# WU-CVGL/SIU3R

Measured on AMD Instinct MI355X. Metric: image-pairs/sec @2x512^2 (SIU3R network forward incl. panoptic post-process), higher is better.
Workload: dtype bf16x3 (fp32 activations, bf16 MFMA with hi/lo operand split; meets the 1e-3 parity bar)

## Files before the change

### include/siu3r_hip.h

```cpp
#ifndef SIU3R_HIP_H
#define SIU3R_HIP_H
#include <stdint.h>
#ifdef __cplusplus
extern "C" {
#endif

#define SIU3R_BF16 0
#define SIU3R_F32 1
#define SIU3R_F16 2
#define SIU3R_F64 3

const char* siu3r_last_error(void);
#define SIU3R_ABI_VERSION 12
int siu3r_abi_version(void);

int siu3r_rope2d(void* tokens, int dtype, int B, int N, int H, int D, int64_t stride_b,
                 int64_t stride_n, int64_t stride_h, const int64_t* positions, float base, float fwd,
                 void* stream);

typedef struct {
  const void* a;
  const void* w_hi;
  const void* w_lo;
  void* c;
  const float* bias;
  const void* residual;
  int32_t m, n, k, kpad;
  int64_t lda, ldc, ldr;
  int32_t a_dtype, c_dtype, r_dtype;
  int32_t act;
  int32_t relu_in;
  int32_t batch;
  int64_t sa, sw, sc, sr;
  int32_t a_mode;
  int32_t ih, iw, cin, kh, kw, stride, pad, oh, ow;
  int32_t out_mode, up, cout;
  const void* up_src;
  int32_t up_dtype;
  const float* rope_cos;
  const float* rope_sin;
  const int64_t* rope_pos;
  int32_t rope_ncols;
  int32_t map_gx, map_rm, map_rn;
  uint64_t* trace;
  const void* w_x3;
  int32_t bmod;
  int64_t sa_i, sc_i, sr_i, sbias;
  const float* ln_stats;
  const float* ln_c1;
  const float* ln_c2;
  int32_t ln_tiles;
  float ln_eps;
  int64_t ln_ldm, ln_sz, ln_sz_i;
  float* stats_out;
  int64_t st_ldm, st_sz, st_sz_i;
  void* c_aux;
  int32_t splitk;
  float* sk_ws;
  int32_t* sk_cnt;
  int64_t sk_ws_floats;
  int32_t sk_cnt_n;
  int32_t tile_cfg;
  int32_t m_main;
  int32_t sk_gx;
  void* c_x3;
  int32_t a_x3;
  int32_t c_x3_col0;
} siu3r_gemm_params;
#define SIU3R_TILE_AUTO 0
#define SIU3R_TILE_128x64 -1
#define SIU3R_TILE_PP_256x256 1
#define SIU3R_TILE_PP_256x128 2
#define SIU3R_TILE_PP_128x128 3
int siu3r_gemm(const siu3r_gemm_params* p, void* stream);
typedef struct {
  int32_t tile_cfg, bm, bn, splitk, skinny_rows, counters;
  int64_t ws_floats;
  char kernel[160];
  int32_t a_x3_ok, c_x3_ok;
  int32_t skinny_path;
} siu3r_gemm_plan_t;
int siu3r_gemm_plan(const siu3r_gemm_params* p, siu3r_gemm_plan_t* out);
int siu3r_gemm_tune(int key, int value);

int siu3r_layernorm(const float* x, void* y, int y_dtype, const float* gamma, const float* beta,
                    int64_t rows, int C, int64_t ldx, int64_t ldy, float eps, void* stream);
int siu3r_layernorm2(const float* x, void* y, int y_dtype, void* y2_bf16, const float* gamma, const float* beta, int64_t rows, int C,
                     int64_t ldx, int64_t ldy, int64_t ldy2, float eps, void* stream);

typedef struct {
  const void *q, *k, *v;
  void* out;
  int32_t dtype;
  int32_t B, H, Nq, Nk, D;
  int64_t q_sb, q_sn, q_sh, k_sb, k_sn, k_sh, v_sb, v_sn, v_sh;
  float scale;
  const float *rope_cos, *rope_sin;
  int32_t rope_max_pos;
  const int64_t *qpos, *kpos;
  const uint8_t* mask;
  int32_t split3;
  int64_t mask_ld;
  float* ws;
  int32_t splits;
  int32_t kv_bxor;
  int32_t kv_x3;
  int32_t out_x3;
} siu3r_attn_params;
int siu3r_attention(const siu3r_attn_params* p, void* stream);
int siu3r_attention_out_x3_ok(const siu3r_attn_params* p);
int siu3r_attention_kv_x3_ok(const siu3r_attn_params* p);
typedef struct {
  char kernel[160];
  int32_t queries_per_wg, key_ranges, combine, key_halves, side_path;
} siu3r_attn_plan_t;
int siu3r_attention_plan(const siu3r_attn_params* p, siu3r_attn_plan_t* out);

int siu3r_add(const float* a, const float* b, float* y, int64_t rows, int64_t b_rows, int C, void* stream);
int siu3r_pack_image_nhwc(const float* img, void* out, int out_dtype, int N, int H, int W, int cpad, void* stream);
int siu3r_resize_bilinear(const void* x, int x_dtype, void* y, int y_dtype, const void* addend, int add_dtype,
                          const float* ch_scale, const float* ch_shift, int N, int IH, int IW, int OH, int OW,
                          int C, int align_corners, void* stream);
int siu3r_resize_bilinear_strided(const void* x, int x_dtype, void* y, int y_dtype, const void* addend, int add_dtype,
                                  const float* ch_scale, const float* ch_shift, int N, int IH, int IW, int OH, int OW,
                                  int C, int align_corners, int64_t x_batch_stride, int64_t addend_batch_stride, void* stream);
int siu3r_resize_bilinear_planes(const void* x, int x_dtype, void* y_planes, int N, int IH, int IW, int OH, int OW, int C, int align_corners,
                                 int64_t x_batch_stride, void* stream);
int siu3r_affine_add(const void* x, int x_dtype, const void* addend, int add_dtype, void* y, int y_dtype,
                     const float* ch_scale, const float* ch_shift, int64_t rows, int C, void* stream);
int siu3r_affine_add_strided(const void* x, int x_dtype, const void* addend, int add_dtype, void* y, int y_dtype,
                             const float* ch_scale, const float* ch_shift, int64_t rows, int C, int64_t rows_per_batch,
                             int64_t x_batch_stride, int64_t addend_batch_stride, void* stream);
int siu3r_maxpool3x3s2(const void* x, void* y, int dtype, int N, int IH, int IW, int C, void* stream);
int siu3r_maxpool2x2s2(const void* x, void* y, int dtype, int N, int IH, int IW, int C, void* stream);
int siu3r_lpips_layer(const float* f0, const float* f1, const float* w, float* dist, int64_t npix, int C, float eps, void* stream);
int siu3r_stem7x7_x3(const float* img, const void* wfrag, const float* bias, const float* up_src, float* out, int B, int G, int H, int W,
                     int planes_out, void* stream);
int siu3r_proj_rows_x3(const float* x, const void* wfrag, const float* bias, float* out, int Z, int G, int64_t M, int K, int N, int ldc,
                       int64_t out_z_stride, void* stream);
int siu3r_rowchain_x3(const float* x, const float* res, const void* pack, float* out, int64_t M, int H, float eps1, float eps2, void* stream);
int siu3r_dwconv3x3_gelu(const void* x, void* y, int dtype, const float* w9c, const float* bias, int B, int H,
                         int W, int C, void* stream);
int siu3r_dwconv3x3_gelu_planes(const float* x, void* y_planes, const float* w9c, const float* bias, int B, int H, int W, int C, void* stream);
int siu3r_msdeform_sample(const void* value, int v_dtype, const float* offs_aw, const float* ref,
                          const int32_t* shapes_host, void* out, int out_dtype, int B, int S, int Q, int heads,
                          int d, int L, int P, void* stream);
int siu3r_msdeform_sample_planes(const void* value, int v_dtype, const float* offs_aw, const float* ref, const int32_t* shapes_host,
                                 void* out_planes, int B, int S, int Q, int heads, int d, int L, int P, void* stream);
int siu3r_groupnorm(const void* x, int x_dtype, void* y, int y_dtype, const float* gamma, const float* beta,
                    float* stats_ws, const void* addend, int add_dtype, int relu, int N, int HW, int C,
                    int groups, float eps, void* stream);
int siu3r_pts3d_exp(float* xyz, int64_t n, void* stream);
int siu3r_gaussian_adapter(const void* raw, int raw_dtype, float* opacities, float* scales, float* rotations,
                           float* harmonics, float* covariances, int64_t n, void* stream);
int siu3r_m2f_attn_mask(const float* mask_logits, uint8_t* out, int32_t* row_counts_ws, int B, int T, int IH,
                        int IW, int OH, int OW, int Q, int64_t out_ld, void* stream);

typedef struct {
  int32_t mode;
  int32_t width, height;
  float w2c[16];
  float proj[16];
  float tanfovx, tanfovy;
  float campos[3];
  float bg[3];
  int32_t sh_degree;
  int32_t sh_band4;
  float k2_znear_cull;
  float fx, fy, cx, cy;
  float near_plane, far_plane;
  float eps2d;
  float radius_clip;
  float extent_sigma;
  int32_t opacity_aware_extent;
  float alpha_min;
  float alpha_max;
  float t_min;
  float dilation;
  int32_t nt_post_blend;
  float k2_near, k2_far;
} siu3r_raster_cam;
int siu3r_raster_geometry(int width, int height, int64_t G, int32_t* out8);
int siu3r_raster_project(const siu3r_raster_cam* cams_host, int V, void* cams_dev, int64_t G, const float* means, const float* cov,
                         int cov_stride, const float* opacities, const float* colors, int channels, int sh_planar, float* rec,
                         int32_t* radii, int32_t* rect, int32_t* tiles_touched, uint32_t* keys, uint64_t* stats, void* stream);
int siu3r_raster_project_dp(const siu3r_raster_cam* cams_host, int V, void* cams_dev, const float* viewmats_dev, const float* Ks_dev, int64_t G,
                            const float* means, const float* cov, int cov_stride, const float* opacities, const float* colors, int channels,
                            int sh_planar, float* rec, int32_t* radii, int32_t* rect, int32_t* tiles_touched, uint32_t* keys, uint64_t* stats,
                            void* stream);
int siu3r_raster_project_c2w(const siu3r_raster_cam* cams_host, int V, void* cams_dev, const float* c2w_dev, const float* Kn_dev, float t_scale,
                             int64_t G, const float* means, const float* cov, int cov_stride, const float* opacities, const float* colors,
                             int channels, int sh_planar, float* rec, int32_t* radii, int32_t* rect, int32_t* tiles_touched, uint32_t* keys,
                             uint64_t* stats, void* stream);
int siu3r_raster_project_aa(const siu3r_raster_cam* cams_host, int V, void* cams_dev, int64_t G, const float* means, const float* cov,
                            int cov_stride, const float* opacities, const float* colors, int channels, int sh_planar, float* rec,
                            int32_t* radii, int32_t* rect, int32_t* tiles_touched, uint32_t* keys, uint64_t* stats, float* comp, void* stream);
int siu3r_raster_project_c2w_aa(const siu3r_raster_cam* cams_host, int V, void* cams_dev, const float* c2w_dev, const float* Kn_dev, float t_scale,
                                int64_t G, const float* means, const float* cov, int cov_stride, const float* opacities, const float* colors,
                                int channels, int sh_planar, float* rec, int32_t* radii, int32_t* rect, int32_t* tiles_touched, uint32_t* keys,
                                uint64_t* stats, float* comp, void* stream);
int siu3r_raster_sort(int V, int64_t G, uint32_t* keys_a, uint32_t* keys_b, int32_t* ids_a, int32_t* ids_b, int32_t* rs_hist,
                      int32_t* rs_tot, const uint64_t* stats, void* stream);
int siu3r_raster_bin(const siu3r_raster_cam* cams_host, int V, int64_t G, const uint32_t* keys, const int32_t* ids, const int32_t* rect,
                     int32_t* bin_hist, int32_t* bin_tot, int32_t* bin_start, void* entries, int64_t cap_e, uint64_t* stats, void* stream);
int siu3r_raster_composite_rgb(const siu3r_raster_cam* cams_host, int V, const void* cams_dev, int64_t G, const int32_t* bin_start,
                               const void* entries, int64_t cap_e, const float* rec, float* image, float* out_depth, float* out_alpha,
                               int32_t* n_touched, void* stream);
int siu3r_raster_tile_lists(const siu3r_raster_cam* cams_host, int V, const int32_t* bin_start, const void* entries, int64_t cap_e,
                            int32_t* tile_count, int32_t* tile_start, int32_t* ids, int64_t cap_d, uint64_t* stats, void* stream);
int siu3r_raster_composite_feat(const siu3r_raster_cam* cams_host, int V, const void* cams_dev, int64_t G, const int32_t* tile_start,
                                const int32_t* ids, int64_t cap_d, const float* rec, const float* feats, int channels, float* out,
                                float* out_alpha, void* stream);
int64_t siu3r_raster_composite_feat_ws_bytes(int width, int height, int V, int64_t cap_d);
int siu3r_raster_composite_feat_ws_lists(int width, int height, int V, int64_t G, const float* feats, int channels, const void* ws, int64_t ws_bytes,
                                         int64_t cap_d);
int siu3r_raster_composite_feat_ws(const siu3r_raster_cam* cams_host, int V, const void* cams_dev, int64_t G, const int32_t* tile_start,
                                   const int32_t* ids, int64_t cap_d, const float* rec, const float* feats, int channels, float* out,
                                   float* out_alpha, void* ws, int64_t ws_bytes, void* stream);
int siu3r_raster_tune(int key, int value);
int siu3r_raster_contrib(const siu3r_raster_cam* cams_host, int V, const void* cams_dev, int64_t G, const int32_t* bin_start, const void* entries,
                         int64_t cap_e, const float* rec, float* wmax, int32_t* count, uint64_t* wsum, void* stream);
int siu3r_raster_composite_rgb_bwd(const siu3r_raster_cam* cams_host, int V, const void* cams_dev, int64_t G, const int32_t* bin_start,
                                   const void* entries, int64_t cap_e, const float* rec, const float* image, const float* depth, const float* alpha,
                                   const float* g_image, const float* g_depth, const float* g_alpha, float* grad, void* stream);
int siu3r_raster_composite_rgb_bwd_abs(const siu3r_raster_cam* cams_host, int V, const void* cams_dev, int64_t G, const int32_t* bin_start,
                                       const void* entries, int64_t cap_e, const float* rec, const float* image, const float* depth,
                                       const float* alpha, const float* g_image, const float* g_depth, const float* g_alpha, float* grad,
                                       float* abs_mean2d, void* stream);
int siu3r_raster_project_bwd(const siu3r_raster_cam* cams_host, int V, const void* cams_dev, int64_t G, const float* means, const float* cov,
                             int cov_stride, const float* opacities, const float* colors, int channels, int sh_planar, const int32_t* rect,
                             const float* grad, float* g_means, float* g_cov, float* g_opacities, float* g_colors, float* g_mean2d,
                             float* pose_part, void* stream);
int siu3r_raster_project_bwd_aa(const siu3r_raster_cam* cams_host, int V, const void* cams_dev, int64_t G, const float* means, const float* cov,
                                int cov_stride, const float* opacities, const float* colors, int channels, int sh_planar, const int32_t* rect,
                                const float* grad, float* g_means, float* g_cov, float* g_opacities, float* g_colors, float* g_mean2d,
                                float* pose_part, void* stream);
int64_t siu3r_raster_pose_partial_rows(int64_t G);
int siu3r_raster_pose_reduce(int V, int64_t nrows, const float* pose_part, float* g_pose, void* stream);
int siu3r_raster_composite_rgb_bwd_k3(const siu3r_raster_cam* cams_host, int V, const void* cams_dev, int64_t G, const int32_t* bin_start,
                                      const void* entries, int64_t cap_e, const float* rec, const float* colors, const float* alphas,
                                      const float* g_colors, const float* g_alphas, float* grad, void* stream);
int siu3r_raster_quad_lists(const siu3r_raster_cam* cams_host, int V, const void* cams_dev, int64_t G, const int32_t* tile_start, const int32_t* ids,
                            int64_t cap_d, const float* rec, void* ws, int64_t ws_bytes, void* stream);
int siu3r_raster_composite_feat_bwd(const siu3r_raster_cam* cams_host, int V, const void* cams_dev, int64_t G, const int32_t* tile_start,
                                    const void* ws, int64_t cap_d, const float* rec, const float* feats, int channels, const float* out,
                                    const float* out_alpha, const float* g_out, const float* g_alpha, float* grad, float* g_feats, void* stream);
int siu3r_raster_project_bwd_k3(const siu3r_raster_cam* cams_host, int V, const void* cams_dev, int64_t G, const float* means, const float* cov,
                                int cov_stride, const int32_t* rect, const float* grad, float* g_means, float* g_cov, float* g_opacities,
                                float* g_colors, float* pose_part, void* stream);
int siu3r_raster_viewmat_reduce(int V, int64_t nrows, const float* pose_part, float* g_viewmats, void* stream);
int siu3r_scale_inplace(float* x, int64_t n, float s, void* stream);
int siu3r_lift_ids(const float* qc, int V, int H, int W, int q, int C, float sem_threshold, int num_queries,
                   uint32_t stuff_mask, int64_t* sem_id, int64_t* ins_id, int32_t* first_pix, int32_t* q_label,
                   void* stream);

int siu3r_split_bf16(const float* x, void* hi, void* lo, void* x3, int64_t rows, int k, int kpad, int64_t ldx, void* stream);

int siu3r_panoptic_stage1(const float* class_logits, const float* mask_logits_cl, float* probs, float* scores,
                          int32_t* labels, int32_t* kept_idx, int32_t* n_keep, float* p256, int32_t* lab_map,
                          int32_t* area, int32_t* orig, int32_t* seg_id, int32_t* seg_label, int32_t* seg_fused,
                          float* seg_score, int32_t* acc_list, int32_t* n_acc, int32_t* seg, int32_t* sem, int32_t* ins,
                          int B, int T, int Q, int C, int IH, int IW, int H, int W, int mask_size, float threshold,
                          float mask_threshold, float overlap, uint32_t fuse_mask, void* stream);
int siu3r_panoptic_qcl(const float* p256, const float* probs, const int32_t* kept_idx, const int32_t* acc_list, int nq,
                       float* out, int b, int T, int H, int W, int mask_size, int Q, int C, void* stream);

int siu3r_quat_scale_to_cov6(const float* quats_wxyz, const float* scales, float* cov6, int64_t G, void* stream);
int siu3r_sh_eval(const float* means, const float* campos3_host, const float* sh, int ncoef, int degree, float* rgb, int64_t G, void* stream);
int siu3r_blend_background(float* colors, const float* alpha, const float* bg_host, int channels, int64_t pixels, void* stream);
int siu3r_sh_eval_dp(const float* means, const float* campos3_dev, const float* sh, int ncoef, int degree, float* rgb, int64_t G, void* stream);
int siu3r_blend_background_dp(float* colors, const float* alpha, const float* bg_dev, int channels, int64_t pixels, void* stream);
int siu3r_quat_scale_to_cov6_bwd(const float* quats_wxyz, const float* scales, const float* g_cov6, float* g_quats, float* g_scales, int64_t G, void* stream);
int siu3r_sh_eval_bwd(const float* means, const float* campos3_dev, const float* sh, int ncoef, int degree, const float* g_rgb, float* g_sh, float* g_means,
                      float* g_campos3, int64_t G, void* stream);

int64_t siu3r_photo_loss_partials(int V, int C, int H, int W);
int siu3r_photo_loss(const float* pred, const float* target, int V, int C, int H, int W, const int64_t* pred_strides,
                     const int64_t* target_strides, float lambda, float data_range, float* grad_pred, float* partials, float* out,
                     void* stream);

int64_t siu3r_depth_loss_ws(int V, int H, int W);
int siu3r_depth_loss(const float* depth, const float* opacity, const float* target, const float* weight, int V, int H, int W, int mode, int space,
                     float min_opacity, float* g_depth, float* g_opacity, void* ws, float* out, float* per_view, int32_t* valid, void* stream);

int64_t siu3r_depth_smooth_ws(int V, int H, int W);
int siu3r_depth_smooth(const float* depth, const float* opacity, const int32_t* segments, int V, int H, int W, int order, int space,
                       float min_opacity, float* g_depth, float* g_opacity, void* ws, float* out, float* per_view, int32_t* active, void* stream);

int siu3r_density_accumulate(const float* g_mean2d, const int32_t* radii, int V, int64_t G, float sx, float sy, float* grad_accum,
                             int32_t* seen, int32_t* max_radius, void* stream);
int64_t siu3r_density_plan_ws(int64_t G);
int siu3r_density_plan(const float* grad_accum, const int32_t* seen, const int32_t* max_radius, const float* log_scales,
// ... 59 lines not shown
```

### siu3r_amd/_lib.py

```python
from __future__ import annotations

import ctypes as C
import os

_HERE = os.path.dirname(os.path.abspath(__file__))
LIB_PATH = os.environ.get("SIU3R_LIB_OVERRIDE") or os.path.join(_HERE, "libsiu3r_hip.so")

BF16, F32 = 0, 1


class GemmParams(C.Structure):
    _fields_ = [
        ("a", C.c_void_p), ("w_hi", C.c_void_p), ("w_lo", C.c_void_p), ("c", C.c_void_p),
        ("bias", C.c_void_p), ("residual", C.c_void_p),
        ("m", C.c_int32), ("n", C.c_int32), ("k", C.c_int32), ("kpad", C.c_int32),
        ("lda", C.c_int64), ("ldc", C.c_int64), ("ldr", C.c_int64),
        ("a_dtype", C.c_int32), ("c_dtype", C.c_int32), ("r_dtype", C.c_int32),
        ("act", C.c_int32), ("relu_in", C.c_int32),
        ("batch", C.c_int32),
        ("sa", C.c_int64), ("sw", C.c_int64), ("sc", C.c_int64), ("sr", C.c_int64),
        ("a_mode", C.c_int32),
        ("ih", C.c_int32), ("iw", C.c_int32), ("cin", C.c_int32), ("kh", C.c_int32), ("kw", C.c_int32),
        ("stride", C.c_int32), ("pad", C.c_int32), ("oh", C.c_int32), ("ow", C.c_int32),
        ("out_mode", C.c_int32), ("up", C.c_int32), ("cout", C.c_int32),
        ("up_src", C.c_void_p), ("up_dtype", C.c_int32),
        ("rope_cos", C.c_void_p), ("rope_sin", C.c_void_p), ("rope_pos", C.c_void_p), ("rope_ncols", C.c_int32),
        ("map_gx", C.c_int32), ("map_rm", C.c_int32), ("map_rn", C.c_int32),
        ("trace", C.c_void_p), ("w_x3", C.c_void_p),
        ("bmod", C.c_int32), ("sa_i", C.c_int64), ("sc_i", C.c_int64), ("sr_i", C.c_int64), ("sbias", C.c_int64),
        ("ln_stats", C.c_void_p), ("ln_c1", C.c_void_p), ("ln_c2", C.c_void_p), ("ln_tiles", C.c_int32), ("ln_eps", C.c_float),
        ("ln_ldm", C.c_int64), ("ln_sz", C.c_int64), ("ln_sz_i", C.c_int64),
        ("stats_out", C.c_void_p), ("st_ldm", C.c_int64), ("st_sz", C.c_int64), ("st_sz_i", C.c_int64),
        ("c_aux", C.c_void_p),
        ("splitk", C.c_int32), ("sk_ws", C.c_void_p), ("sk_cnt", C.c_void_p),
        ("sk_ws_floats", C.c_int64), ("sk_cnt_n", C.c_int32), ("tile_cfg", C.c_int32), ("m_main", C.c_int32), ("sk_gx", C.c_int32),
        ("c_x3", C.c_void_p), ("a_x3", C.c_int32), ("c_x3_col0", C.c_int32),
    ]


class GemmPlan(C.Structure):
    _fields_ = [
        ("tile_cfg", C.c_int32), ("bm", C.c_int32), ("bn", C.c_int32), ("splitk", C.c_int32), ("skinny_rows", C.c_int32),
        ("counters", C.c_int32), ("ws_floats", C.c_int64), ("kernel", C.c_char * 160), ("a_x3_ok", C.c_int32), ("c_x3_ok", C.c_int32), ("skinny_path", C.c_int32),
    ]


class AttnParams(C.Structure):
    _fields_ = [
        ("q", C.c_void_p), ("k", C.c_void_p), ("v", C.c_void_p), ("out", C.c_void_p),
        ("dtype", C.c_int32),
        ("B", C.c_int32), ("H", C.c_int32), ("Nq", C.c_int32), ("Nk", C.c_int32), ("D", C.c_int32),
        ("q_sb", C.c_int64), ("q_sn", C.c_int64), ("q_sh", C.c_int64),
        ("k_sb", C.c_int64), ("k_sn", C.c_int64), ("k_sh", C.c_int64),
        ("v_sb", C.c_int64), ("v_sn", C.c_int64), ("v_sh", C.c_int64),
        ("scale", C.c_float),
        ("rope_cos", C.c_void_p), ("rope_sin", C.c_void_p), ("rope_max_pos", C.c_int32),
        ("qpos", C.c_void_p), ("kpos", C.c_void_p), ("mask", C.c_void_p),
        ("split3", C.c_int32), ("mask_ld", C.c_int64),
        ("ws", C.c_void_p), ("splits", C.c_int32), ("kv_bxor", C.c_int32), ("kv_x3", C.c_int32), ("out_x3", C.c_int32),
    ]


class AttnPlan(C.Structure):
    _fields_ = [
        ("kernel", C.c_char * 160), ("queries_per_wg", C.c_int32), ("key_ranges", C.c_int32), ("combine", C.c_int32),
        ("key_halves", C.c_int32), ("side_path", C.c_int32),
    ]


class RasterCam(C.Structure):
    _fields_ = [
        ("mode", C.c_int32), ("width", C.c_int32), ("height", C.c_int32),
        ("w2c", C.c_float * 16), ("proj", C.c_float * 16),
        ("tanfovx", C.c_float), ("tanfovy", C.c_float), ("campos", C.c_float * 3), ("bg", C.c_float * 3),
        ("sh_degree", C.c_int32), ("sh_band4", C.c_int32), ("k2_znear_cull", C.c_float),
        ("fx", C.c_float), ("fy", C.c_float), ("cx", C.c_float), ("cy", C.c_float),
        ("near_plane", C.c_float), ("far_plane", C.c_float), ("eps2d", C.c_float), ("radius_clip", C.c_float),
        ("extent_sigma", C.c_float), ("opacity_aware_extent", C.c_int32),
        ("alpha_min", C.c_float), ("alpha_max", C.c_float), ("t_min", C.c_float), ("dilation", C.c_float),
        ("nt_post_blend", C.c_int32), ("k2_near", C.c_float), ("k2_far", C.c_float),
    ]


class AdamField(C.Structure):
    _fields_ = [
        ("param", C.c_void_p), ("grad", C.c_void_p), ("exp_avg", C.c_void_p), ("exp_avg_sq", C.c_void_p),
        ("width", C.c_int32), ("head_period", C.c_int32), ("lr", C.c_float), ("lr_tail", C.c_float),
    ]


_P, _I, _L, _F = C.c_void_p, C.c_int, C.c_int64, C.c_float
ABI_VERSION = 12

SIGNATURES = {
    "siu3r_last_error": [],
    "siu3r_abi_version": [],
    "siu3r_rope2d": [_P, _I, _I, _I, _I, _I, _L, _L, _L, _P, _F, _F, _P],
    "siu3r_gemm": [C.POINTER(GemmParams), _P],
    "siu3r_gemm_plan": [C.POINTER(GemmParams), C.POINTER(GemmPlan)],
    "siu3r_gemm_tune": [_I, _I],
    "siu3r_layernorm": [_P, _P, _I, _P, _P, _L, _I, _L, _L, _F, _P],
    "siu3r_layernorm2": [_P, _P, _I, _P, _P, _P, _L, _I, _L, _L, _L, _F, _P],
    "siu3r_attention": [C.POINTER(AttnParams), _P],
    "siu3r_attention_kv_x3_ok": [C.POINTER(AttnParams)],
    "siu3r_attention_out_x3_ok": [C.POINTER(AttnParams)],
    "siu3r_attention_plan": [C.POINTER(AttnParams), C.POINTER(AttnPlan)],
    "siu3r_add": [_P, _P, _P, _L, _L, _I, _P],
    "siu3r_pack_image_nhwc": [_P, _P, _I, _I, _I, _I, _I, _P],
    "siu3r_resize_bilinear": [_P, _I, _P, _I, _P, _I, _P, _P, _I, _I, _I, _I, _I, _I, _I, _P],
    "siu3r_affine_add": [_P, _I, _P, _I, _P, _I, _P, _P, _L, _I, _P],
    "siu3r_resize_bilinear_strided": [_P, _I, _P, _I, _P, _I, _P, _P, _I, _I, _I, _I, _I, _I, _I, _L, _L, _P],
    "siu3r_resize_bilinear_planes": [_P, _I, _P, _I, _I, _I, _I, _I, _I, _I, _L, _P],
    "siu3r_affine_add_strided": [_P, _I, _P, _I, _P, _I, _P, _P, _L, _I, _L, _L, _L, _P],
    "siu3r_maxpool3x3s2": [_P, _P, _I, _I, _I, _I, _I, _P],
    "siu3r_maxpool2x2s2": [_P, _P, _I, _I, _I, _I, _I, _P],
    "siu3r_lpips_layer": [_P, _P, _P, _P, _L, _I, _F, _P],
    "siu3r_stem7x7_x3": [_P, _P, _P, _P, _P, _I, _I, _I, _I, _I, _P],
    "siu3r_proj_rows_x3": [_P, _P, _P, _P, _I, _I, _L, _I, _I, _I, _L, _P],
    "siu3r_rowchain_x3": [_P, _P, _P, _P, _L, _I, _F, _F, _P],
    "siu3r_dwconv3x3_gelu": [_P, _P, _I, _P, _P, _I, _I, _I, _I, _P],
    "siu3r_dwconv3x3_gelu_planes": [_P, _P, _P, _P, _I, _I, _I, _I, _P],
    "siu3r_msdeform_sample_planes": [_P, _I, _P, _P, C.POINTER(C.c_int32), _P, _I, _I, _I, _I, _I, _I, _I, _P],
    "siu3r_msdeform_sample": [_P, _I, _P, _P, C.POINTER(C.c_int32), _P, _I, _I, _I, _I, _I, _I, _I, _I, _P],
    "siu3r_groupnorm": [_P, _I, _P, _I, _P, _P, _P, _P, _I, _I, _I, _I, _I, _I, _F, _P],
    "siu3r_pts3d_exp": [_P, _L, _P],
    "siu3r_gaussian_adapter": [_P, _I, _P, _P, _P, _P, _P, _L, _P],
    "siu3r_m2f_attn_mask": [_P, _P, _P, _I, _I, _I, _I, _I, _I, _I, _L, _P],
    "siu3r_split_bf16": [_P, _P, _P, _P, _L, _I, _I, _L, _P],
    "siu3r_raster_geometry": [_I, _I, _L, C.POINTER(C.c_int32)],
    "siu3r_raster_project": [C.POINTER(RasterCam), _I, _P, _L, _P, _P, _I, _P, _P, _I, _I, _P, _P, _P, _P, _P, _P, _P],
    "siu3r_raster_sort": [_I, _L, _P, _P, _P, _P, _P, _P, _P, _P],
    "siu3r_raster_bin": [C.POINTER(RasterCam), _I, _L, _P, _P, _P, _P, _P, _P, _P, _L, _P, _P],
    "siu3r_raster_composite_rgb": [C.POINTER(RasterCam), _I, _P, _L, _P, _P, _L, _P, _P, _P, _P, _P, _P],
    "siu3r_raster_tile_lists": [C.POINTER(RasterCam), _I, _P, _P, _L, _P, _P, _P, _L, _P, _P],
    "siu3r_raster_composite_feat": [C.POINTER(RasterCam), _I, _P, _L, _P, _P, _L, _P, _P, _I, _P, _P, _P],
    "siu3r_raster_composite_feat_ws_bytes": [_I, _I, _I, _L],
    "siu3r_raster_tune": [_I, _I],
    "siu3r_raster_composite_feat_ws": [C.POINTER(RasterCam), _I, _P, _L, _P, _P, _L, _P, _P, _I, _P, _P, _P, _L, _P],
    "siu3r_scale_inplace": [_P, _L, _F, _P],
    "siu3r_quat_scale_to_cov6": [_P, _P, _P, _L, _P],
    "siu3r_sh_eval": [_P, _P, _P, _I, _I, _P, _L, _P],
    "siu3r_blend_background": [_P, _P, _P, _I, _L, _P],
    "siu3r_sh_eval_dp": [_P, _P, _P, _I, _I, _P, _L, _P],
    "siu3r_blend_background_dp": [_P, _P, _P, _I, _L, _P],
    "siu3r_raster_project_dp": [C.POINTER(RasterCam), _I, _P, _P, _P, _L, _P, _P, _I, _P, _P, _I, _I, _P, _P, _P, _P, _P, _P, _P],
    "siu3r_raster_project_c2w": [C.POINTER(RasterCam), _I, _P, _P, _P, _F, _L, _P, _P, _I, _P, _P, _I, _I, _P, _P, _P, _P, _P, _P, _P],
    "siu3r_raster_project_aa": [C.POINTER(RasterCam), _I, _P, _L, _P, _P, _I, _P, _P, _I, _I, _P, _P, _P, _P, _P, _P, _P, _P],
    "siu3r_raster_project_c2w_aa": [C.POINTER(RasterCam), _I, _P, _P, _P, _F, _L, _P, _P, _I, _P, _P, _I, _I, _P, _P, _P, _P, _P, _P, _P, _P],
    "siu3r_raster_project_bwd_aa": [C.POINTER(RasterCam), _I, _P, _L, _P, _P, _I, _P, _P, _I, _I, _P, _P, _P, _P, _P, _P, _P, _P, _P],
    "siu3r_mip_filter3d_ws": [_I],
    "siu3r_mip_filter3d": [_P, _P, _I, _I, _I, _P, _L, _F, _F, _F, _P, _P, _P],
    "siu3r_mip_apply": [_P, _P, _P, _L, _P, _P, _P],
    "siu3r_mip_apply_bwd": [_P, _P, _P, _P, _P, _L, _P, _P, _P],
    "siu3r_raster_composite_rgb_bwd": [C.POINTER(RasterCam), _I, _P, _L, _P, _P, _L, _P, _P, _P, _P, _P, _P, _P, _P, _P],
    "siu3r_raster_composite_rgb_bwd_abs": [C.POINTER(RasterCam), _I, _P, _L, _P, _P, _L, _P, _P, _P, _P, _P, _P, _P, _P, _P, _P],
    "siu3r_raster_contrib": [C.POINTER(RasterCam), _I, _P, _L, _P, _P, _L, _P, _P, _P, _P, _P],
    "siu3r_raster_project_bwd": [C.POINTER(RasterCam), _I, _P, _L, _P, _P, _I, _P, _P, _I, _I, _P, _P, _P, _P, _P, _P, _P, _P, _P],
    "siu3r_raster_pose_partial_rows": [_L],
    "siu3r_raster_pose_reduce": [_I, _L, _P, _P, _P],
    "siu3r_raster_composite_rgb_bwd_k3": [C.POINTER(RasterCam), _I, _P, _L, _P, _P, _L, _P, _P, _P, _P, _P, _P, _P],
    "siu3r_raster_composite_feat_ws_lists": [_I, _I, _I, _L, _P, _I, _P, _L, _L],
    "siu3r_raster_quad_lists": [C.POINTER(RasterCam), _I, _P, _L, _P, _P, _L, _P, _P, _L, _P],
    "siu3r_raster_composite_feat_bwd": [C.POINTER(RasterCam), _I, _P, _L, _P, _P, _L, _P, _P, _I, _P, _P, _P, _P, _P, _P, _P],
    "siu3r_raster_project_bwd_k3": [C.POINTER(RasterCam), _I, _P, _L, _P, _P, _I, _P, _P, _P, _P, _P, _P, _P, _P],
    "siu3r_raster_viewmat_reduce": [_I, _L, _P, _P, _P],
    "siu3r_quat_scale_to_cov6_bwd": [_P, _P, _P, _P, _P, _L, _P],
    "siu3r_sh_eval_bwd": [_P, _P, _P, _I, _I, _P, _P, _P, _P, _L, _P],
    "siu3r_photo_loss_partials": [_I, _I, _I, _I],
    "siu3r_photo_loss": [_P, _P, _I, _I, _I, _I, C.POINTER(C.c_int64), C.POINTER(C.c_int64), _F, _F, _P, _P, _P, _P],
    "siu3r_depth_loss_ws": [_I, _I, _I],
    "siu3r_depth_loss": [_P, _P, _P, _P, _I, _I, _I, _I, _I, _F, _P, _P, _P, _P, _P, _P, _P],
    "siu3r_depth_smooth_ws": [_I, _I, _I],
    "siu3r_depth_smooth": [_P, _P, _P, _I, _I, _I, _I, _I, _F, _P, _P, _P, _P, _P, _P, _P],
    "siu3r_gaussian_adam_ws": [_L],
    "siu3r_gaussian_adam": [C.POINTER(AdamField), _I, _L, C.c_double, C.c_double, _F, _F, _F, _P, _I, _I, _P, _P, _P],
    "siu3r_density_accumulate": [_P, _P, _I, _L, _F, _F, _P, _P, _P, _P],
    "siu3r_density_plan_ws": [_L],
    "siu3r_density_plan": [_P, _P, _P, _P, _P, _L, _F, _F, _F, _I, _F, _I, _P, _P, _P, _P, _P],
    "siu3r_density_apply": [_I, _P, _P, _P, _I, _L, _P, _P, _P, _P, _P, _P, _P, _P, _P],
    "siu3r_mcmc_ws": [_L],
    "siu3r_mcmc_weights": [_P, _L, _F, _I, _P, _P, _P],
    "siu3r_mcmc_scan": [_P, _P, _L, _P, _P, _P, _P, _P],
    "siu3r_mcmc_sample": [_P, _L, _P, _L, _P, _P, _P],
    "siu3r_mcmc_relocate": [_P, _P, _P, _L, C.c_double, _P],
    "siu3r_mcmc_copy_rows": [_P, _P, _P, _I, _L, _P, _P, _L, _L, _P],
    "siu3r_mcmc_noise": [_P, _P, _P, _P, _P, _L, _F, _F, _P],
    "siu3r_mcmc_regularize": [_P, _P, _L, _F, _F, _P, _P, _P, _P, _P],
    "siu3r_exposure_ws": [_I, _I, _I],
    "siu3r_exposure_apply": [_P, C.POINTER(C.c_int64), _P, _I, _I, _I, _P, _P],
    "siu3r_exposure_apply_bwd": [_P, C.POINTER(C.c_int64), _P, _P, _I, _I, _I, _P, _P, _P, _P],
    "siu3r_camera_step": [_P, _P, _P, _P, _P, _P, _P, _I, _L] + [C.c_double] * 6 + [_P],
    "siu3r_bilagrid_apply": [_P, C.POINTER(C.c_int64), _P, _I, _I, _I, _I, _I, _I, _P, _P],
    "siu3r_bilagrid_apply_bwd": [_P, C.POINTER(C.c_int64), _P, _P, _I, _I, _I, _I, _I, _I, _P, _P, _P],
    "siu3r_bilagrid_tv_ws": [_I, _I, _I, _I],
    "siu3r_bilagrid_tv": [_P, _I, _I, _I, _I, _F, _P, _P, _P, _P],
    "siu3r_lift_ids":[_P, _I, _I, _I, _I, _I, _F, _I, C.c_uint32, _P, _P, _P, _P, _P],
    "siu3r_panoptic_stage1": [_P] * 20 + [_I] * 9 + [_F, _F, _F, C.c_uint32, _P],
    "siu3r_panoptic_qcl": [_P, _P, _P, _P, _I, _P, _I, _I, _I, _I, _I, _I, _I, _P],
}
_RESTYPES = {"siu3r_last_error": C.c_char_p, "siu3r_raster_composite_feat_ws_bytes": C.c_int64, "siu3r_raster_pose_partial_rows": C.c_int64}
_RESTYPES["siu3r_photo_loss_partials"] = C.c_int64
_RESTYPES["siu3r_density_plan_ws"] = C.c_int64
_RESTYPES["siu3r_depth_loss_ws"] = C.c_int64
_RESTYPES["siu3r_depth_smooth_ws"] = C.c_int64
_RESTYPES["siu3r_gaussian_adam_ws"] = C.c_int64
_RESTYPES["siu3r_mcmc_ws"] = C.c_int64
_RESTYPES["siu3r_exposure_ws"] = C.c_int64
_RESTYPES["siu3r_bilagrid_tv_ws"] = C.c_int64
_RESTYPES["siu3r_mip_filter3d_ws"] = C.c_int64

_lib = None


def lib():
    global _lib
    if _lib is not None:
        return _lib
    import torch
    if not os.path.exists(LIB_PATH):
        raise RuntimeError(
            f"{LIB_PATH} is missing: build it with `python -m siu3r_amd.build` "
            "(hipcc --offload-arch=gfx950).  There is no CPU fallback for the SIU3R hot path."
        )
    l = C.CDLL(LIB_PATH)
    for name, argtypes in SIGNATURES.items():
        fn = getattr(l, name)
        fn.argtypes = argtypes
        fn.restype = _RESTYPES.get(name, C.c_int)
    if l.siu3r_abi_version() != ABI_VERSION:
        raise RuntimeError(f"{LIB_PATH} has ABI version {l.siu3r_abi_version()}, these bindings expect {ABI_VERSION}: rebuild it "
                           f"(python -m siu3r_amd.build)")
    _lib = l
    return l


def check(rc: int, what: str = ""):
    if rc != 0:
        msg = lib().siu3r_last_error()
        raise RuntimeError((msg.decode() if msg else f"{what} failed") + f" [rc={rc}]")
```

### siu3r_amd/csrc/elementwise.hip

```cpp
#include "common.h"

namespace {

struct f32x4v {
  float v[4];
};
__device__ __forceinline__ f32x4v load4(const void* p, int dtype, int64_t i) {
  f32x4v r;
  if (dtype == SIU3R_F32) {
    float4 a = *(const float4*)((const float*)p + i);
    r.v[0] = a.x; r.v[1] = a.y; r.v[2] = a.z; r.v[3] = a.w;
  } else {
    uint2 a = *(const uint2*)((const u16*)p + i);
    r.v[0] = bf16_bits_to_f32((u16)(a.x & 0xffff));
    r.v[1] = bf16_bits_to_f32((u16)(a.x >> 16));
    r.v[2] = bf16_bits_to_f32((u16)(a.y & 0xffff));
    r.v[3] = bf16_bits_to_f32((u16)(a.y >> 16));
  }
  return r;
}
__device__ __forceinline__ void store4(void* p, int dtype, int64_t i, const f32x4v& r) {
  if (dtype == SIU3R_F32) {
    *(float4*)((float*)p + i) = make_float4(r.v[0], r.v[1], r.v[2], r.v[3]);
  } else {
    uint2 w;
    w.x = (uint32_t)f32_to_bf16_bits(r.v[0]) | ((uint32_t)f32_to_bf16_bits(r.v[1]) << 16);
    w.y = (uint32_t)f32_to_bf16_bits(r.v[2]) | ((uint32_t)f32_to_bf16_bits(r.v[3]) << 16);
    *(uint2*)((u16*)p + i) = w;
  }
}

__device__ __forceinline__ float wave_sum(float v) {
#pragma unroll
  for (int o = 32; o > 0; o >>= 1) v += __shfl_xor(v, o);
  return v;
}

template <int DT>
__global__ void rope2d_kernel(void* tokens, const int64_t* pos, int B, int N, int H, int D, int64_t sb, int64_t sn,
                              int64_t sh, float base, float fwd) {
  const int Q = D / 4, half = D / 2;
  const int64_t idx = (int64_t)blockIdx.x * blockDim.x + threadIdx.x;
  const int64_t total = (int64_t)B * N * half;
  if (idx >= total) return;
  const int pr = (int)(idx % half);
  const int64_t tok = idx / half;
  const int n = (int)(tok % N), b = (int)(tok / N);
  const int axis = pr / Q, q = pr - axis * Q;
  const float inv_freq = fwd / powf(base, q / float(Q));
  const float freq = pos[tok * 2 + axis] * inv_freq;
  const float c = cosf(freq), s = sinf(freq);
  const int64_t e0 = b * sb + n * sn + axis * 2 * Q + q;
  for (int h = 0; h < H; ++h) {
    const int64_t e = e0 + h * sh;
    if (DT == SIU3R_F32) {
      float* p = (float*)tokens + e;
      const float u = p[0], v = p[Q];
      p[0] = u * c - v * s;
      p[Q] = v * c + u * s;
    } else if (DT == SIU3R_F64) {
      double* p = (double*)tokens + e;
      const double u = p[0], v = p[Q];
      p[0] = u * (double)c - v * (double)s;
      p[Q] = v * (double)c + u * (double)s;
    } else if (DT == SIU3R_F16) {
      _Float16* p = (_Float16*)tokens + e;
      const float u = (float)p[0], v = (float)p[Q];
      p[0] = (_Float16)(u * c - v * s);
      p[Q] = (_Float16)(v * c + u * s);
    } else {
      u16* p = (u16*)tokens + e;
      const float u = bf16_bits_to_f32(p[0]), v = bf16_bits_to_f32(p[Q]);
      p[0] = f32_to_bf16_bits(u * c - v * s);
      p[Q] = f32_to_bf16_bits(v * c + u * s);
    }
  }
}

__global__ __launch_bounds__(256) void layernorm_kernel(const float* x, void* y, int y_dtype, void* y2, const float* gamma,
                                                        const float* beta, int64_t rows, int C, int64_t ldx,
                                                        int64_t ldy, int64_t ldy2, float eps) {
  const int lane = threadIdx.x & 63;
  const int64_t row = (int64_t)blockIdx.x * 4 + (threadIdx.x >> 6);
  if (row >= rows) return;
  const float* xr = x + row * ldx;
  float4 v[8];
  float sum = 0.f;
#pragma unroll
  for (int i = 0; i < 8; ++i) {
    const int c = lane * 4 + i * 256;
    if (c < C) {
      v[i] = *(const float4*)(xr + c);
      sum += v[i].x + v[i].y + v[i].z + v[i].w;
    }
  }
  const float mean = wave_sum(sum) / (float)C;
  float sq = 0.f;
#pragma unroll
  for (int i = 0; i < 8; ++i) {
    const int c = lane * 4 + i * 256;
    if (c < C) {
      const float a = v[i].x - mean, b = v[i].y - mean, cc = v[i].z - mean, d = v[i].w - mean;
      sq += a * a + b * b + cc * cc + d * d;
    }
  }
  const float rstd = rsqrtf(wave_sum(sq) / (float)C + eps);
#pragma unroll
  for (int i = 0; i < 8; ++i) {
    const int c = lane * 4 + i * 256;
    if (c < C) {
      const float4 g = *(const float4*)(gamma + c), bb = *(const float4*)(beta + c);
      f32x4v o;
      o.v[0] = (v[i].x - mean) * rstd * g.x + bb.x;
      o.v[1] = (v[i].y - mean) * rstd * g.y + bb.y;
      o.v[2] = (v[i].z - mean) * rstd * g.z + bb.z;
      o.v[3] = (v[i].w - mean) * rstd * g.w + bb.w;
      store4(y, y_dtype, row * ldy + c, o);
      if (y2) store4(y2, SIU3R_BF16, row * ldy2 + c, o);
    }
  }
}

__global__ void add_kernel(const float* a, const float* b, float* y, int64_t rows, int64_t b_rows, int C4) {
  const int64_t idx = (int64_t)blockIdx.x * blockDim.x + threadIdx.x;
  if (idx >= rows * C4) return;
  const int64_t r = idx / C4;
  const int c = (int)(idx - r * C4);
  const float4 x = ((const float4*)a)[idx];
  const float4 z = ((const float4*)b)[(r % b_rows) * C4 + c];
  ((float4*)y)[idx] = make_float4(x.x + z.x, x.y + z.y, x.z + z.z, x.w + z.w);
}

__global__ void pack_image_kernel(const float* img, void* out, int out_dtype, int N, int H, int W, int cpad) {
  const int64_t idx = (int64_t)blockIdx.x * blockDim.x + threadIdx.x;
  const int64_t hw = (int64_t)H * W;
  if (idx >= (int64_t)N * hw) return;
  const int64_t n = idx / hw, r = idx - n * hw;
  if (cpad == 4) {
    float4 o = {img[(n * 3 + 0) * hw + r], img[(n * 3 + 1) * hw + r], img[(n * 3 + 2) * hw + r], 0.f};
    ((float4*)out)[idx] = o;
    return;
  }
  f32x8 v;
#pragma unroll
  for (int j = 0; j < 8; ++j) v.v[j] = 0.f;
  for (int c = 0; c < 3; ++c) v.v[c] = img[(n * 3 + c) * hw + r];
  store8_from_f32(out, out_dtype, idx * 8, v);
}

__device__ __forceinline__ void src_index(int o, int in, int out, int align, int& i0, int& i1, float& l1) {
  float src;
  if (align) {
    const float scale = out > 1 ? (float)(in - 1) / (float)(out - 1) : 0.f;
// ... 263 lines not shown
        const float aw = expf(e4[pt] - mx) / den;
        const float locx = rx + o8[pt * 2 + 0] / (float)ww;
        const float locy = ry + o8[pt * 2 + 1] / (float)hh;
        const float gx = 2.f * locx - 1.f, gy = 2.f * locy - 1.f;
        const float fx = ((gx + 1.f) * ww - 1.f) * 0.5f, fy = ((gy + 1.f) * hh - 1.f) * 0.5f;
        const float x0f = floorf(fx), y0f = floorf(fy);
        const int x0 = (int)x0f, y0 = (int)y0f;
        const float lx = fx - x0f, ly = fy - y0f;
        const float wgt[4] = {(1.f - lx) * (1.f - ly), lx * (1.f - ly), (1.f - lx) * ly, lx * ly};
#pragma unroll
        for (int k = 0; k < 4; ++k) {
          const int xx = x0 + (k & 1), yy = y0 + (k >> 1);
          const bool ok = xx >= 0 && xx < ww && yy >= 0 && yy < hh;
          const int xc = min(max(xx, 0), ww - 1), yc = min(max(yy, 0), hh - 1);
          const int s_ = st0 + yc * ww + xc;
          v[pt][k] = load4(value, v_dtype, ((vb + s_) * heads + hd) * d + dc);
#pragma unroll
          for (int j = 0; j < 4; ++j) v[pt][k].v[j] = ok ? v[pt][k].v[j] : 0.f;
          wk[pt][k] = wgt[k] * aw;
        }
      }
#pragma unroll
      for (int pt = 0; pt < 4; ++pt)
#pragma unroll
        for (int k = 0; k < 4; ++k)
#pragma unroll
          for (int j = 0; j < 4; ++j) acc.v[j] += v[pt][k].v[j] * wk[pt][k];
    }
    if (out_x3) {
      store_planes4_pair((unsigned char*)out + ((int64_t)b * Q + q) * heads * d * 4, hd * d + dc, acc.v);
      return;
    }
    store4(out, out_dtype, (((int64_t)b * Q + q) * heads + hd) * d + dc, acc);
  } else {
    const int LP = L * P;
    const float* row = offs_aw + ((int64_t)b * Q + q) * (heads * LP * 3);
    const float* offs = row + hd * LP * 2;
    const float* logit = row + heads * LP * 2 + hd * LP;
    float mx = -INFINITY;
    for (int i = 0; i < LP; ++i) mx = fmaxf(mx, logit[i]);
    float den = 0.f;
    for (int i = 0; i < LP; ++i) den += expf(logit[i] - mx);
    f32x4v acc;
#pragma unroll
    for (int j = 0; j < 4; ++j) acc.v[j] = 0.f;
    for (int l = 0; l < L; ++l) {
      const int hh = sh.h[l], ww = sh.w[l];
      const float rx = ref[((int64_t)q * L + l) * 2 + 0], ry = ref[((int64_t)q * L + l) * 2 + 1];
      for (int pt = 0; pt < P; ++pt) {
        const int i = l * P + pt;
        const float aw = expf(logit[i] - mx) / den;
        const float locx = rx + offs[i * 2 + 0] / (float)ww;
        const float locy = ry + offs[i * 2 + 1] / (float)hh;
        const float gx = 2.f * locx - 1.f, gy = 2.f * locy - 1.f;
        const float fx = ((gx + 1.f) * ww - 1.f) * 0.5f, fy = ((gy + 1.f) * hh - 1.f) * 0.5f;
        const float x0f = floorf(fx), y0f = floorf(fy);
        const int x0 = (int)x0f, y0 = (int)y0f;
        const float lx = fx - x0f, ly = fy - y0f;
        const float wgt[4] = {(1.f - lx) * (1.f - ly), lx * (1.f - ly), (1.f - lx) * ly, lx * ly};
#pragma unroll
        for (int k = 0; k < 4; ++k) {
          const int xx = x0 + (k & 1), yy = y0 + (k >> 1);
          if (xx < 0 || xx >= ww || yy < 0 || yy >= hh) continue;
          const int64_t s = sh.start[l] + (int64_t)yy * ww + xx;
          const f32x4v v = load4(value, v_dtype, (((int64_t)b * S + s) * heads + hd) * d + dc);
          const float wk = wgt[k] * aw;
#pragma unroll
          for (int j = 0; j < 4; ++j) acc.v[j] += v.v[j] * wk;
        }
      }
    }
    store4(out, out_dtype, (((int64_t)b * Q + q) * heads + hd) * d + dc, acc);
  }
}

constexpr int GN_T = 1024;
__global__ __launch_bounds__(GN_T) void gn_stats_kernel(const void* x, int x_dtype, float* stats, int HW, int C,
                                                        int groups, float eps) {
  const int n = blockIdx.y, bx = blockIdx.x;
  const int g = groups % 8 == 0 ? (bx % 8) * (groups / 8) + bx / 8 : bx;
  const int cg = C / groups, cg4 = cg >> 2;
  const int64_t total = (int64_t)HW * cg4;
  double s = 0.0, ss = 0.0;
  auto acc = [&](const f32x4v& v) {
#pragma unroll
    for (int j = 0; j < 4; ++j) {
      s += v.v[j];
      ss += (double)v.v[j] * v.v[j];
    }
  };
  int64_t i = threadIdx.x;
  if (GN_T % cg4 == 0) {
    const int64_t step = (int64_t)(GN_T / cg4) * C;
    int64_t off = (int64_t)n * HW * C + g * cg + (int)(threadIdx.x % cg4) * 4 + (int64_t)(threadIdx.x / cg4) * C;
    for (; i + GN_T < total; i += 2 * GN_T, off += 2 * step) {
      const f32x4v v = load4(x, x_dtype, off), w = load4(x, x_dtype, off + step);
      acc(v);
      acc(w);
    }
    for (; i < total; i += GN_T, off += step) acc(load4(x, x_dtype, off));
  }
  for (; i < total; i += GN_T) {
    const int64_t px = i / cg4;
    acc(load4(x, x_dtype, ((int64_t)n * HW + px) * C + g * cg + (int)(i - px * cg4) * 4));
  }
  __shared__ double sh_s[GN_T], sh_ss[GN_T];
  sh_s[threadIdx.x] = s;
  sh_ss[threadIdx.x] = ss;
  __syncthreads();
  for (int o = GN_T / 2; o > 0; o >>= 1) {
    if (threadIdx.x < o) {
      sh_s[threadIdx.x] += sh_s[threadIdx.x + o];
      sh_ss[threadIdx.x] += sh_ss[threadIdx.x + o];
    }
    __syncthreads();
  }
  if (threadIdx.x == 0) {
    const double cnt = (double)HW * cg;
    const double mean = sh_s[0] / cnt;
    double var = sh_ss[0] / cnt - mean * mean;
    if (var < 0) var = 0;
    stats[((int64_t)n * groups + g) * 2 + 0] = (float)mean;
    stats[((int64_t)n * groups + g) * 2 + 1] = (float)(1.0 / sqrt(var + (double)eps));
  }
}
__global__ void gn_apply_kernel(const void* x, int x_dtype, void* y, int y_dtype, const float* gamma,
                                const float* beta, const float* stats, const void* addend, int add_dtype, int relu,
                                int N, int HW, int C, int groups) {
  const int C4 = C >> 2;
  const int64_t idx = (int64_t)blockIdx.x * blockDim.x + threadIdx.x;
  if (idx >= (int64_t)N * HW * C4) return;
  const int c = (int)(idx % C4) * 4;
  const int n = (int)(idx / ((int64_t)HW * C4));
  const int g = c / (C / groups);
  const float mean = stats[((int64_t)n * groups + g) * 2], rstd = stats[((int64_t)n * groups + g) * 2 + 1];
  f32x4v v = load4(x, x_dtype, idx * 4);
#pragma unroll
  for (int j = 0; j < 4; ++j) {
    float o = (v.v[j] - mean) * rstd * gamma[c + j] + beta[c + j];
    if (relu) o = fmaxf(o, 0.f);
    v.v[j] = o;
  }
  if (addend) {
    const f32x4v a = load4(addend, add_dtype, idx * 4);
#pragma unroll
    for (int j = 0; j < 4; ++j) v.v[j] += a.v[j];
  }
  store4(y, y_dtype, idx * 4, v);
}

__global__ void pts3d_kernel(float* xyz, int64_t n) {
  const int64_t i = (int64_t)blockIdx.x * blockDim.x + threadIdx.x;
  if (i >= n) return;
  const float x = xyz[i * 3], y = xyz[i * 3 + 1], z = xyz[i * 3 + 2];
  const float d = sqrtf(x * x + y * y + z * z);
  const float dc = fmaxf(d, 1e-8f);
  const float e = expm1f(d);
  xyz[i * 3] = x / dc * e;
  xyz[i * 3 + 1] = y / dc * e;
  xyz[i * 3 + 2] = z / dc * e;
}

constexpr int GA_ROWS = 128, GA_D = 83, GA_SH = 75;
__constant__ float c_sh_mask[25];
__global__ __launch_bounds__(256) void gaussian_adapter_kernel(const void* raw, int raw_dtype, float* opac,
                                                               float* scales, float* rots, float* sh, float* cov,
                                                               int64_t n) {
  __shared__ float s[GA_ROWS * GA_D];
  __shared__ float so[GA_ROWS * 17];
  const int64_t g0 = (int64_t)blockIdx.x * GA_ROWS;
  const int rows = (int)((n - g0) < GA_ROWS ? (n - g0) : GA_ROWS);
  const int nt = blockDim.x;
  if (raw_dtype == SIU3R_F32 && rows == GA_ROWS && ((uintptr_t)raw & 15) == 0) {
    const float4* src = (const float4*)((const float*)raw + g0 * GA_D);
    for (int i = threadIdx.x; i < GA_ROWS * GA_D / 4; i += nt) ((float4*)s)[i] = src[i];
  } else {
    for (int i = threadIdx.x; i < rows * GA_D; i += nt) s[i] = load_as_f32(raw, raw_dtype, g0 * GA_D + i);
  }
  __syncthreads();
  const int t = threadIdx.x;
  if (t < rows) {
    const float* r = s + t * GA_D;
    opac[g0 + t] = 1.f / (1.f + expf(-r[0]));
    float sc[3];
#pragma unroll
    for (int j = 0; j < 3; ++j) {
      const float x = r[1 + j];
      const float sp = x > 20.f ? x : log1pf(expf(x));
      sc[j] = fminf(0.001f * sp, 0.3f);
      so[t * 17 + j] = sc[j];
    }
    const float qi = r[4], qj = r[5], qk = r[6], qr = r[7];
    so[t * 17 + 3] = qi; so[t * 17 + 4] = qj; so[t * 17 + 5] = qk; so[t * 17 + 6] = qr;
    const float nrm = sqrtf(qi * qi + qj * qj + qk * qk + qr * qr) + 1e-8f;
    const float i_ = qi / nrm, j_ = qj / nrm, k_ = qk / nrm, r_ = qr / nrm;
    const float two_s = 2.f / ((i_ * i_ + j_ * j_ + k_ * k_ + r_ * r_) + 1e-8f);
    float R[9];
    R[0] = 1.f - two_s * (j_ * j_ + k_ * k_);
    R[1] = two_s * (i_ * j_ - k_ * r_);
    R[2] = two_s * (i_ * k_ + j_ * r_);
    R[3] = two_s * (i_ * j_ + k_ * r_);
    R[4] = 1.f - two_s * (i_ * i_ + k_ * k_);
    R[5] = two_s * (j_ * k_ - i_ * r_);
    R[6] = two_s * (i_ * k_ - j_ * r_);
    R[7] = two_s * (j_ * k_ + i_ * r_);
    R[8] = 1.f - two_s * (i_ * i_ + j_ * j_);
    float M[9];
#pragma unroll
    for (int a = 0; a < 3; ++a)
#pragma unroll
      for (int b = 0; b < 3; ++b) M[a * 3 + b] = R[a * 3 + b] * sc[b];
#pragma unroll
    for (int a = 0; a < 3; ++a)
#pragma unroll
      for (int b = 0; b < 3; ++b) {
        float v = 0.f;
#pragma unroll
        for (int k2 = 0; k2 < 3; ++k2) v += (M[a * 3 + k2] * sc[k2]) * R[b * 3 + k2];
        so[t * 17 + 7 + a * 3 + b] = v;
      }
  }
  __syncthreads();
  for (int i = threadIdx.x; i < rows * 3; i += nt) scales[g0 * 3 + i] = so[(i / 3) * 17 + i % 3];
  for (int i = threadIdx.x; i < rows * 4; i += nt) rots[g0 * 4 + i] = so[(i >> 2) * 17 + 3 + (i & 3)];
  for (int i = threadIdx.x; i < rows * 9; i += nt) cov[g0 * 9 + i] = so[(i / 9) * 17 + 7 + i % 9];
  if (rows == GA_ROWS && ((uintptr_t)sh & 15) == 0) {
    for (int i4 = threadIdx.x; i4 < GA_ROWS * GA_SH / 4; i4 += nt) {
      float v[4];
#pragma unroll
      for (int u = 0; u < 4; ++u) {
        const int i = i4 * 4 + u, rr = i / GA_SH, e = i - rr * GA_SH;
        v[u] = s[rr * GA_D + 8 + e] * c_sh_mask[e % 25];
      }
      ((float4*)(sh + g0 * GA_SH))[i4] = make_float4(v[0], v[1], v[2], v[3]);
    }
  } else {
    for (int i = threadIdx.x; i < rows * GA_SH; i += nt) {
      const int rr = i / GA_SH, e = i - rr * GA_SH;
      sh[g0 * GA_SH + i] = s[rr * GA_D + 8 + e] * c_sh_mask[e % 25];
    }
  }
}

__global__ void m2f_mask_kernel(const float* ml, uint8_t* out, int32_t* row_counts, int B, int T, int IH, int IW,
                                int OH, int OW, int Q, int64_t ld) {
  const int64_t idx = (int64_t)blockIdx.x * blockDim.x + threadIdx.x;
  const int64_t total = (int64_t)B * T * OH * OW * Q;
  if (idx >= total) return;
  const int q = (int)(idx % Q);
  int64_t r = idx / Q;
  const int ox = (int)(r % OW);
  r /= OW;
  const int oy = (int)(r % OH);
  r /= OH;
  const int t = (int)(r % T);
  const int b = (int)(r / T);
  int y0, y1, x0, x1;
  float ly, lx;
  src_index(oy, IH, OH, 0, y0, y1, ly);
  src_index(ox, IW, OW, 0, x0, x1, lx);
  const int64_t base = ((int64_t)b * T + t) * IH * IW;
  const float v00 = ml[(base + (int64_t)y0 * IW + x0) * Q + q], v01 = ml[(base + (int64_t)y0 * IW + x1) * Q + q];
  const float v10 = ml[(base + (int64_t)y1 * IW + x0) * Q + q], v11 = ml[(base + (int64_t)y1 * IW + x1) * Q + q];
  const float v = (1.f - ly) * ((1.f - lx) * v00 + lx * v01) + ly * ((1.f - lx) * v10 + lx * v11);
  const float sg = 1.f / (1.f + expf(-v));
  const uint8_t blocked = sg < 0.5f ? 1 : 0;
  const int64_t nk = (int64_t)T * OH * OW;
  out[((int64_t)b * Q + q) * ld + ((int64_t)t * OH + oy) * OW + ox] = blocked;
  if (!blocked) row_counts[b * Q + q] = 1;
}
__global__ void zero_i32_kernel(int32_t* p, int64_t n) {
  const int64_t idx = (int64_t)blockIdx.x * blockDim.x + threadIdx.x;
  if (idx < n) p[idx] = 0;
}
__global__ void m2f_mask_fix_kernel(uint8_t* out, const int32_t* row_counts, int64_t rows, int64_t nk, int64_t ld) {
  const int64_t idx = (int64_t)blockIdx.x * blockDim.x + threadIdx.x;
  if (idx >= rows * nk) return;
  const int64_t r = idx / nk;
  if (row_counts[r] == 0) out[r * ld + (idx - r * nk)] = 0;
}

__global__ void split_bf16_kernel(const float* x, u16* hi, u16* lo, u16* x3, int64_t rows, int k, int kpad, int64_t ldx) {
  const int64_t idx = (int64_t)blockIdx.x * blockDim.x + threadIdx.x;
  if (idx >= rows * kpad) return;
  const int64_t r = idx / kpad;
  const int c = (int)(idx - r * kpad);
  const float v = c < k ? x[r * ldx + c] : 0.f;
  const u16 h = f32_to_bf16_bits(v);
  const u16 l = f32_to_bf16_bits(v - bf16_bits_to_f32(h));
  if (hi) hi[idx] = h;
  if (lo) lo[idx] = l;
  if (x3) {
    const int64_t o = r * 2 * kpad + (c >> 5) * 64 + (c & 31);
    x3[o] = h;
    x3[o + 32] = l;
  }
}

inline dim3 grid1d(int64_t total, int block = 256) { return dim3((unsigned)cdiv64(total, block)); }

inline bool al4(const void* p, int dtype) { return ((uintptr_t)p & (dtype == SIU3R_F32 ? 15 : 7)) == 0; }
inline bool al16(const void* p) { return ((uintptr_t)p & 15) == 0; }

}

extern "C" int siu3r_rope2d(void* tokens, int dtype, int B, int N, int H, int D, int64_t sb, int64_t sn, int64_t sh,
                            const int64_t* positions, float base, float fwd, void* stream) {
  SIU3R_CHECK(D % 4 == 0, "token dim must be multiple of 4");
  SIU3R_CHECK(dtype == SIU3R_F32 || dtype == SIU3R_BF16 || dtype == SIU3R_F16 || dtype == SIU3R_F64, "rope_2d: unsupported dtype %d", dtype);
  SIU3R_CHECK(B >= 0 && N >= 0 && H >= 0, "rope_2d: negative size");
  const int64_t total = (int64_t)B * N * (D / 2);
  if (total == 0 || H == 0) return 0;
  SIU3R_CHECK(tokens && positions, "rope_2d: null pointer");
  hipStream_t s = (hipStream_t)stream;
  if (dtype == SIU3R_F32)
    hipLaunchKernelGGL(rope2d_kernel<SIU3R_F32>, grid1d(total), dim3(256), 0, s, tokens, positions, B, N, H, D, sb, sn, sh, base, fwd);
  else if (dtype == SIU3R_F64)
    hipLaunchKernelGGL(rope2d_kernel<SIU3R_F64>, grid1d(total), dim3(256), 0, s, tokens, positions, B, N, H, D, sb, sn, sh, base, fwd);
  else if (dtype == SIU3R_F16)
    hipLaunchKernelGGL(rope2d_kernel<SIU3R_F16>, grid1d(total), dim3(256), 0, s, tokens, positions, B, N, H, D, sb, sn, sh, base, fwd);
  else
    hipLaunchKernelGGL(rope2d_kernel<SIU3R_BF16>, grid1d(total), dim3(256), 0, s, tokens, positions, B, N, H, D, sb, sn, sh, base, fwd);
  SIU3R_LAUNCH_CHECK("siu3r_rope2d");
  return 0;
}

extern "C" int siu3r_layernorm(const float* x, void* y, int y_dtype, const float* gamma, const float* beta,
                               int64_t rows, int C, int64_t ldx, int64_t ldy, float eps, void* stream) {
  SIU3R_CHECK(C % 4 == 0 && C <= 2048 && ldx % 4 == 0 && ldy % 4 == 0, "layernorm: C=%d must be a multiple of 4 and <= 2048", C);
  if (rows == 0) return 0;
  SIU3R_CHECK(x && y && gamma && beta, "layernorm: null pointer");
  SIU3R_CHECK(al16(x) && al4(y, y_dtype) && al16(gamma) && al16(beta), "layernorm: x, gamma, beta must be 16-byte aligned, y 16 (fp32) / 8 (bf16)");
  hipLaunchKernelGGL(layernorm_kernel, dim3((unsigned)cdiv64(rows, 4)), dim3(256), 0, (hipStream_t)stream, x, y, y_dtype, (void*)nullptr, gamma, beta, rows, C, ldx, ldy, (int64_t)0, eps);
  SIU3R_LAUNCH_CHECK("siu3r_layernorm");
  return 0;
}

extern "C" int siu3r_layernorm2(const float* x, void* y, int y_dtype, void* y2_bf16, const float* gamma, const float* beta, int64_t rows,
                                int C, int64_t ldx, int64_t ldy, int64_t ldy2, float eps, void* stream) {
  SIU3R_CHECK(C % 4 == 0 && C <= 2048 && ldx % 4 == 0 && ldy % 4 == 0 && ldy2 % 4 == 0, "layernorm2: C=%d must be a multiple of 4 and <= 2048", C);
  if (rows == 0) return 0;
  SIU3R_CHECK(x && y && y2_bf16 && gamma && beta, "layernorm2: null pointer");
  SIU3R_CHECK(al16(x) && al4(y, y_dtype) && al4(y2_bf16, SIU3R_BF16) && al16(gamma) && al16(beta),
              "layernorm2: x, gamma, beta must be 16-byte aligned, y 16 (fp32) / 8 (bf16), y2 8");
  hipLaunchKernelGGL(layernorm_kernel, dim3((unsigned)cdiv64(rows, 4)), dim3(256), 0, (hipStream_t)stream, x, y, y_dtype, y2_bf16, gamma, beta, rows, C, ldx, ldy, ldy2, eps);
  SIU3R_LAUNCH_CHECK("siu3r_layernorm2");
  return 0;
}

extern "C" int siu3r_add(const float* a, const float* b, float* y, int64_t rows, int64_t b_rows, int C, void* stream) {
  SIU3R_CHECK(C % 4 == 0 && b_rows > 0, "add: bad arguments");
  if (rows == 0 || C == 0) return 0;
  SIU3R_CHECK(a && b && y, "add: null pointer");
  SIU3R_CHECK(al16(a) && al16(b) && al16(y), "add: a, b, y must be 16-byte aligned");
  hipLaunchKernelGGL(add_kernel, grid1d(rows * (C / 4)), dim3(256), 0, (hipStream_t)stream, a, b, y, rows, b_rows, C / 4);
  SIU3R_LAUNCH_CHECK("siu3r_add");
  return 0;
}

extern "C" int siu3r_pack_image_nhwc(const float* img, void* out, int out_dtype, int N, int H, int W, int cpad, void* stream) {
  SIU3R_CHECK(cpad == 8 || (cpad == 4 && out_dtype == SIU3R_F32), "pack_image: 8 channels (bf16 / fp32) or 4 channels (fp32) per pixel, got %d", cpad);
  if ((int64_t)N * H * W == 0) return 0;
  SIU3R_CHECK(img && out, "pack_image: null pointer");
  SIU3R_CHECK(al16(out), "pack_image: out must be 16-byte aligned");
  hipLaunchKernelGGL(pack_image_kernel, grid1d((int64_t)N * H * W), dim3(256), 0, (hipStream_t)stream, img, out, out_dtype, N, H, W, cpad);
  SIU3R_LAUNCH_CHECK("siu3r_pack_image_nhwc");
  return 0;
}

extern "C" int siu3r_resize_bilinear_strided(const void* x, int x_dtype, void* y, int y_dtype, const void* addend, int add_dtype,
                                             const float* ch_scale, const float* ch_shift, int N, int IH, int IW, int OH, int OW, int C,
                                             int align_corners, int64_t x_batch_stride, int64_t addend_batch_stride, void* stream) {
  SIU3R_CHECK(C % 4 == 0, "resize_bilinear: bad arguments (C=%d)", C);
  SIU3R_CHECK((ch_scale == nullptr) == (ch_shift == nullptr), "resize_bilinear: scale/shift must come together");
  if ((int64_t)N * OH * OW * C == 0) return 0;
  SIU3R_CHECK(x && y && IH > 0 && IW > 0, "resize_bilinear: null pointer or empty source");
  SIU3R_CHECK(al4(x, x_dtype) && al4(y, y_dtype) && al4(addend, add_dtype), "resize_bilinear: x, y, addend must be 16-byte (fp32) / 8-byte (bf16) aligned");
  SIU3R_CHECK(x_batch_stride >= (int64_t)IH * IW * C && x_batch_stride % 4 == 0 && (!addend || (addend_batch_stride >= (int64_t)OH * OW * C && addend_batch_stride % 4 == 0)),
              "resize_bilinear: batch strides must cover one map and keep 4-element alignment");
  hipLaunchKernelGGL(resize_kernel, grid1d((int64_t)N * OH * OW * (C / 4)), dim3(256), 0, (hipStream_t)stream, x, x_dtype, y, y_dtype, addend, add_dtype, ch_scale, ch_shift, N, IH, IW, OH, OW, C, align_corners, x_batch_stride, addend_batch_stride, 0);
  SIU3R_LAUNCH_CHECK("siu3r_resize_bilinear");
  return 0;
}

extern "C" int siu3r_resize_bilinear_planes(const void* x, int x_dtype, void* y_planes, int N, int IH, int IW, int OH, int OW, int C, int align_corners,
                                            int64_t x_batch_stride, void* stream) {
  SIU3R_CHECK(C % 32 == 0, "resize_bilinear_planes: planes need whole 32-column segments (C=%d)", C);
  if ((int64_t)N * OH * OW * C == 0) return 0;
  SIU3R_CHECK(x && y_planes && IH > 0 && IW > 0, "resize_bilinear_planes: null pointer or empty source");
  SIU3R_CHECK(al4(x, x_dtype) && ((uintptr_t)y_planes & 127) == 0, "resize_bilinear_planes: x must be 16-byte (fp32) / 8-byte (bf16) aligned, the planes 128-byte aligned");
  SIU3R_CHECK(x_batch_stride >= (int64_t)IH * IW * C && x_batch_stride % 4 == 0, "resize_bilinear_planes: the batch stride must cover one map and keep 4-element alignment");
  hipLaunchKernelGGL(resize_kernel, grid1d((int64_t)N * OH * OW * (C / 4)), dim3(256), 0, (hipStream_t)stream, x, x_dtype, y_planes, SIU3R_F32, nullptr, SIU3R_F32, nullptr, nullptr, N, IH, IW, OH, OW, C, align_corners, x_batch_stride, (int64_t)OH * OW * C, 1);
// ... 5 lines not shown
                                     int add_dtype, const float* ch_scale, const float* ch_shift, int N, int IH,
                                     int IW, int OH, int OW, int C, int align_corners, void* stream) {
  return siu3r_resize_bilinear_strided(x, x_dtype, y, y_dtype, addend, add_dtype, ch_scale, ch_shift, N, IH, IW, OH, OW, C, align_corners,
                                       (int64_t)IH * IW * C, (int64_t)OH * OW * C, stream);
}

extern "C" int siu3r_affine_add_strided(const void* x, int x_dtype, const void* addend, int add_dtype, void* y, int y_dtype, const float* ch_scale,
                                        const float* ch_shift, int64_t rows, int C, int64_t rows_per_batch, int64_t x_batch_stride,
                                        int64_t addend_batch_stride, void* stream) {
  SIU3R_CHECK(C % 4 == 0, "affine_add: bad arguments");
  if (rows == 0 || C == 0) return 0;
  SIU3R_CHECK(x && y && rows_per_batch > 0 && rows % rows_per_batch == 0, "affine_add: bad arguments");
  SIU3R_CHECK(al4(x, x_dtype) && al4(y, y_dtype) && al4(addend, add_dtype), "affine_add: x, y, addend must be 16-byte (fp32) / 8-byte (bf16) aligned");
  SIU3R_CHECK(x_batch_stride >= rows_per_batch * C && x_batch_stride % 4 == 0 && (!addend || (addend_batch_stride >= rows_per_batch * C && addend_batch_stride % 4 == 0)),
              "affine_add: batch strides must cover one batch item and keep 4-element alignment");
  hipLaunchKernelGGL(affine_add_kernel, grid1d(rows * (C / 4)), dim3(256), 0, (hipStream_t)stream, x, x_dtype, addend, add_dtype, y, y_dtype, ch_scale, ch_shift, rows, C,
                     rows_per_batch, x_batch_stride, addend_batch_stride);
  SIU3R_LAUNCH_CHECK("siu3r_affine_add");
  return 0;
}

extern "C" int siu3r_affine_add(const void* x, int x_dtype, const void* addend, int add_dtype, void* y, int y_dtype,
                                const float* ch_scale, const float* ch_shift, int64_t rows, int C, void* stream) {
  return siu3r_affine_add_strided(x, x_dtype, addend, add_dtype, y, y_dtype, ch_scale, ch_shift, rows, C, rows, rows * C, rows * C, stream);
}

extern "C" int siu3r_maxpool3x3s2(const void* x, void* y, int dtype, int N, int IH, int IW, int C, void* stream) {
  SIU3R_CHECK(C % 4 == 0, "maxpool: bad arguments");
  if ((int64_t)N * IH * IW * C == 0) return 0;
  SIU3R_CHECK(x && y, "maxpool: null pointer");
  SIU3R_CHECK(al4(x, dtype) && al4(y, dtype), "maxpool: x, y must be 16-byte (fp32) / 8-byte (bf16) aligned");
  const int OH = (IH + 2 - 3) / 2 + 1, OW = (IW + 2 - 3) / 2 + 1;
  hipLaunchKernelGGL(maxpool_kernel, grid1d((int64_t)N * OH * OW * (C / 4)), dim3(256), 0, (hipStream_t)stream, x, y, dtype, N, IH, IW, OH, OW, C);
  SIU3R_LAUNCH_CHECK("siu3r_maxpool3x3s2");
  return 0;
}

extern "C" int siu3r_maxpool2x2s2(const void* x, void* y, int dtype, int N, int IH, int IW, int C, void* stream) {
  SIU3R_CHECK(C % 4 == 0 && IH >= 2 && IW >= 2, "maxpool2x2s2: bad arguments");
  if ((int64_t)N * C == 0) return 0;
  SIU3R_CHECK(x && y, "maxpool2x2s2: null pointer");
  SIU3R_CHECK(al4(x, dtype) && al4(y, dtype), "maxpool2x2s2: x, y must be 16-byte (fp32) / 8-byte (bf16) aligned");
  const int OH = IH / 2, OW = IW / 2;
  hipLaunchKernelGGL(maxpool2x2_kernel, grid1d((int64_t)N * OH * OW * (C / 4)), dim3(256), 0, (hipStream_t)stream, x, y, dtype, N, IH, IW, OH, OW, C);
  SIU3R_LAUNCH_CHECK("siu3r_maxpool2x2s2");
  return 0;
}

extern "C" int siu3r_lpips_layer(const float* f0, const float* f1, const float* w, float* dist, int64_t npix, int C, float eps, void* stream) {
  SIU3R_CHECK(npix == 0 || (f0 && f1 && w && dist), "lpips_layer: null pointer");
  SIU3R_CHECK(C > 0 && C % 4 == 0 && (((uintptr_t)f0 | (uintptr_t)f1 | (uintptr_t)w) & 15) == 0, "lpips_layer: C = %d must be a multiple of 4, pointers 16-byte aligned", C);
  if (npix > 0) hipLaunchKernelGGL(lpips_layer_kernel, dim3((unsigned)cdiv64(npix, 4)), dim3(256), 0, (hipStream_t)stream, f0, f1, w, dist, npix, C, eps);
  SIU3R_LAUNCH_CHECK("siu3r_lpips_layer");
  return 0;
}

extern "C" int siu3r_dwconv3x3_gelu(const void* x, void* y, int dtype, const float* w9c, const float* bias, int B,
                                    int H, int W, int C, void* stream) {
  SIU3R_CHECK(C % 4 == 0 && H % 2 == 0 && W % 2 == 0, "dwconv3x3_gelu: bad arguments");
  const int64_t ntok = 21 * (int64_t)(H * W / 4);
  if ((int64_t)B * ntok * C == 0) return 0;
  SIU3R_CHECK(x && y && w9c && bias, "dwconv3x3_gelu: null pointer");
  SIU3R_CHECK(al4(x, dtype) && al4(y, dtype) && al16(w9c), "dwconv3x3_gelu: x, y must be 16-byte (fp32) / 8-byte (bf16) aligned, w9c 16");
  hipLaunchKernelGGL(dwconv_gelu_kernel, grid1d((int64_t)B * ntok * (C / 4)), dim3(256), 0, (hipStream_t)stream, x, y, dtype, w9c, bias, B, H, W, C, 0);
  SIU3R_LAUNCH_CHECK("siu3r_dwconv3x3_gelu");
  return 0;
}

extern "C" int siu3r_dwconv3x3_gelu_planes(const float* x, void* y_planes, const float* w9c, const float* bias, int B, int H, int W, int C, void* stream) {
  SIU3R_CHECK(C % 32 == 0 && H % 2 == 0 && W % 2 == 0, "dwconv3x3_gelu_planes: planes need whole 32-column segments (C=%d) and even H, W", C);
  const int64_t ntok = 21 * (int64_t)(H * W / 4);
  if ((int64_t)B * ntok * C == 0) return 0;
  SIU3R_CHECK(x && y_planes && w9c && bias, "dwconv3x3_gelu_planes: null pointer");
  SIU3R_CHECK(al16(x) && al16(w9c) && ((uintptr_t)y_planes & 127) == 0, "dwconv3x3_gelu_planes: x, w9c must be 16-byte aligned, the planes 128-byte aligned");
  hipLaunchKernelGGL(dwconv_gelu_kernel, grid1d((int64_t)B * ntok * (C / 4)), dim3(256), 0, (hipStream_t)stream, x, y_planes, SIU3R_F32, w9c, bias, B, H, W, C, 1);
  SIU3R_LAUNCH_CHECK("siu3r_dwconv3x3_gelu_planes");
  return 0;
}

static int msdeform_sample(const void* value, int v_dtype, const float* offs_aw, const float* ref, const int32_t* shapes_host, void* out, int out_dtype,
                           int B, int S, int Q, int heads, int d, int L, int P, int out_x3, void* stream) {
  SIU3R_CHECK(shapes_host, "msdeform_sample: null pointer");
  SIU3R_CHECK(L >= 1 && L <= 4 && d % 4 == 0, "msdeform_sample: L=%d (1..4), d=%d (%%4)", L, d);
  MsdShapes sh;
  int start = 0;
  for (int l = 0; l < L; ++l) {
    sh.h[l] = shapes_host[2 * l];
    sh.w[l] = shapes_host[2 * l + 1];
    sh.start[l] = start;
    start += sh.h[l] * sh.w[l];
  }
  SIU3R_CHECK(start == S, "msdeform_sample: spatial shapes sum %d != S=%d", start, S);
  if ((int64_t)B * Q * heads * d == 0) return 0;
  SIU3R_CHECK(value && offs_aw && ref && out, "msdeform_sample: null pointer");
  SIU3R_CHECK(al4(value, v_dtype) && al4(out, out_dtype), "msdeform_sample: value, out must be 16-byte (fp32) / 8-byte (bf16) aligned");
  const int D4 = d / 4;
  const int qb = (256 % D4 == 0 && !(out_x3 && d % 8 != 0)) ? 256 / D4 : 0;
  const dim3 grid = qb ? dim3((unsigned)((int64_t)B * ((Q + qb - 1) / qb) * heads)) : grid1d((int64_t)B * Q * heads * D4);
  const bool al = (((uintptr_t)offs_aw) & 15) == 0 && P == 4;
#define SIU3R_MSD(LT_, PT_) hipLaunchKernelGGL((msdeform_kernel<LT_, PT_>), grid, dim3(256), 0, (hipStream_t)stream, value, v_dtype, offs_aw, ref, sh, out, out_dtype, B, S, Q, heads, d, L, P, qb, out_x3)
  SIU3R_CHECK(!out_x3 || (al && (L == 1 || L == 3 || L == 4) && ((uintptr_t)out & 127) == 0),
              "msdeform_sample_planes: planes come from the <L, 4> kernels only (L = 1, 3, 4; P = 4; 16-byte aligned offs_aw) and need a 128-byte aligned destination");
  if (al && L == 1) SIU3R_MSD(1, 4);
  else if (al && L == 3) SIU3R_MSD(3, 4);
  else if (al && L == 4) SIU3R_MSD(4, 4);
  else SIU3R_MSD(0, 0);
#undef SIU3R_MSD
  SIU3R_LAUNCH_CHECK("siu3r_msdeform_sample");
  return 0;
}

extern "C" int siu3r_msdeform_sample(const void* value, int v_dtype, const float* offs_aw, const float* ref,
                                     const int32_t* shapes_host, void* out, int out_dtype, int B, int S, int Q,
                                     int heads, int d, int L, int P, void* stream) {
  return msdeform_sample(value, v_dtype, offs_aw, ref, shapes_host, out, out_dtype, B, S, Q, heads, d, L, P, 0, stream);
}

extern "C" int siu3r_msdeform_sample_planes(const void* value, int v_dtype, const float* offs_aw, const float* ref, const int32_t* shapes_host,
                                            void* out_planes, int B, int S, int Q, int heads, int d, int L, int P, void* stream) {
  SIU3R_CHECK(d % 4 == 0 && ((int64_t)heads * d) % 32 == 0, "msdeform_sample_planes: planes need rows of whole 32-column segments (heads=%d, d=%d)", heads, d);
  return msdeform_sample(value, v_dtype, offs_aw, ref, shapes_host, out_planes, SIU3R_F32, B, S, Q, heads, d, L, P, 1, stream);
}

extern "C" int siu3r_groupnorm(const void* x, int x_dtype, void* y, int y_dtype, const float* gamma,
                               const float* beta, float* stats_ws, const void* addend, int add_dtype, int relu, int N,
                               int HW, int C, int groups, float eps, void* stream) {
  SIU3R_CHECK(groups > 0 && C % groups == 0 && (C / groups) % 4 == 0, "groupnorm: C/groups must be a multiple of 4");
  if ((int64_t)N * HW * C == 0) return 0;
  SIU3R_CHECK(x && y && gamma && beta && stats_ws, "groupnorm: null pointer");
  SIU3R_CHECK(al4(x, x_dtype) && al4(y, y_dtype) && al4(addend, add_dtype), "groupnorm: x, y, addend must be 16-byte (fp32) / 8-byte (bf16) aligned");
  hipStream_t s = (hipStream_t)stream;
  hipLaunchKernelGGL(gn_stats_kernel, dim3(groups, N), dim3(GN_T), 0, s, x, x_dtype, stats_ws, HW, C, groups, eps);
  hipLaunchKernelGGL(gn_apply_kernel, grid1d((int64_t)N * HW * (C / 4)), dim3(256), 0, s, x, x_dtype, y, y_dtype, gamma, beta, stats_ws, addend, add_dtype, relu, N, HW, C, groups);
  SIU3R_LAUNCH_CHECK("siu3r_groupnorm");
  return 0;
}

extern "C" int siu3r_pts3d_exp(float* xyz, int64_t n, void* stream) {
  if (n == 0) return 0;
  SIU3R_CHECK(xyz, "pts3d_exp: null pointer");
  hipLaunchKernelGGL(pts3d_kernel, grid1d(n), dim3(256), 0, (hipStream_t)stream, xyz, n);
  SIU3R_LAUNCH_CHECK("siu3r_pts3d_exp");
  return 0;
}

extern "C" int siu3r_gaussian_adapter(const void* raw, int raw_dtype, float* opacities, float* scales,
                                      float* rotations, float* harmonics, float* covariances, int64_t n,
                                      void* stream) {
  if (n == 0) return 0;
  SIU3R_CHECK(raw && opacities && scales && rotations && harmonics && covariances, "gaussian_adapter: null pointer");
  static bool mask_set = false;
  if (!mask_set) {
    float m[25];
    m[0] = 1.f;
    for (int deg = 1; deg <= 4; ++deg) {
      float v = 0.1f;
      for (int i = 0; i < deg; ++i) v *= 0.25f;
      for (int i = deg * deg; i < (deg + 1) * (deg + 1); ++i) m[i] = v;
    }
    if (hipMemcpyToSymbol(HIP_SYMBOL(c_sh_mask), m, sizeof(m)) != hipSuccess) {
      siu3r_set_error("gaussian_adapter: cannot upload SH mask");
      return 2;
    }
    mask_set = true;
  }
  hipLaunchKernelGGL(gaussian_adapter_kernel, dim3((unsigned)cdiv64(n, GA_ROWS)), dim3(256), 0, (hipStream_t)stream, raw, raw_dtype, opacities, scales, rotations, harmonics, covariances, n);
  SIU3R_LAUNCH_CHECK("siu3r_gaussian_adapter");
  return 0;
}

extern "C" int siu3r_m2f_attn_mask(const float* mask_logits, uint8_t* out, int32_t* row_counts_ws, int B, int T,
                                   int IH, int IW, int OH, int OW, int Q, int64_t out_ld, void* stream) {
  SIU3R_CHECK(out_ld >= (int64_t)T * OH * OW, "m2f_attn_mask: out_ld too small");
  if ((int64_t)B * Q * T * OH * OW == 0) return 0;
  SIU3R_CHECK(mask_logits && out && row_counts_ws && IH > 0 && IW > 0, "m2f_attn_mask: null pointer or empty source");
  hipStream_t s = (hipStream_t)stream;
  hipLaunchKernelGGL(zero_i32_kernel, grid1d((int64_t)B * Q), dim3(256), 0, s, row_counts_ws, (int64_t)B * Q);
  const int64_t nk = (int64_t)T * OH * OW;
  hipLaunchKernelGGL(m2f_mask_kernel, grid1d((int64_t)B * nk * Q), dim3(256), 0, s, mask_logits, out, row_counts_ws, B, T, IH, IW, OH, OW, Q, out_ld);
  hipLaunchKernelGGL(m2f_mask_fix_kernel, grid1d((int64_t)B * Q * nk), dim3(256), 0, s, out, row_counts_ws, (int64_t)B * Q, nk, out_ld);
  SIU3R_LAUNCH_CHECK("siu3r_m2f_attn_mask");
  return 0;
}

extern "C" int siu3r_split_bf16(const float* x, void* hi, void* lo, void* x3, int64_t rows, int k, int kpad, int64_t ldx,
                                void* stream) {
  SIU3R_CHECK(kpad >= k && (!x3 || kpad % 32 == 0), "split_bf16: bad arguments");
  if (rows == 0 || kpad == 0) return 0;
  SIU3R_CHECK(x && (hi || x3), "split_bf16: null pointer");
  hipLaunchKernelGGL(split_bf16_kernel, grid1d(rows * kpad), dim3(256), 0, (hipStream_t)stream, x, (u16*)hi, (u16*)lo, (u16*)x3, rows, k, kpad, ldx);
  SIU3R_LAUNCH_CHECK("siu3r_split_bf16");
  return 0;
}
```

### siu3r_amd/csrc/proj.hip

```cpp
#include "common.h"

namespace {

struct ProjParams {
  const float* x;
  const uint4* wfrag;
  const float* bias;
  float* out;
  int64_t M, out_zs;
  int Z, G, N, ldc;
};

__device__ __forceinline__ void lds_barrier() { asm volatile("s_waitcnt lgkmcnt(0)\n\ts_barrier" ::: "memory"); }

template <int K, int NB, int RG>
__global__ __launch_bounds__(64 * NB * RG) void proj_rows_x3_kernel(const ProjParams p) {
#if __HIP_DEVICE_COMPILE__
  constexpr int NT = 64 * NB * RG, ROWS = 32 * RG, KS = K / 16;
  constexpr int LD = K + 8;
  constexpr int PIECES = ROWS * K / 4;
  constexpr int PPT = (PIECES + NT - 1) / NT;
  __shared__ __attribute__((aligned(16))) unsigned short s_hi[ROWS * LD], s_lo[ROWS * LD];
  const int t = threadIdx.x, lane = t & 63, wave = t >> 6;
  const int nb = wave % NB, rg = wave / NB;
  const int z = blockIdx.y, g = z % p.G;
  const int l31 = lane & 31, lh = lane >> 5;

  bf16x8 bh[KS], bl[KS];
  {
    const uint4* wf = p.wfrag + ((size_t)(g * NB + nb) * KS * 2) * 64 + lane;
#pragma unroll
    for (int s = 0; s < KS; ++s) {
      bh[s] = as_bf16x8(wf[(2 * s) * 64]);
      bl[s] = as_bf16x8(wf[(2 * s + 1) * 64]);
    }
  }
  const int col = nb * 32 + l31;
  const float bv = (p.bias && col < p.N) ? p.bias[g * NB * 32 + col] : 0.f;

  const int64_t ntiles = (p.M + ROWS - 1) / ROWS;
  const float* xz = p.x + (int64_t)z * p.M * K;
  float* oz = p.out + (int64_t)z * p.out_zs;
  float4 nx[PPT];
  auto fetch = [&](int64_t tile) {
#pragma unroll
    for (int i = 0; i < PPT; ++i) {
      const int pc = i * NT + t;
      const int64_t row = tile * ROWS + pc / (K / 4);
      nx[i] = (pc < PIECES && row < p.M) ? *(const float4*)(xz + row * K + 4 * (pc % (K / 4))) : make_float4(0.f, 0.f, 0.f, 0.f);
    }
  };
  int64_t tile = blockIdx.x;
  if (tile < ntiles) fetch(tile);
  for (; tile < ntiles; tile += gridDim.x) {
    lds_barrier();
#pragma unroll
    for (int i = 0; i < PPT; ++i) {
      const int pc = i * NT + t, r = pc / (K / 4), c = 4 * (pc % (K / 4));
      if (pc >= PIECES) break;
      const float4 v = nx[i];
      const uint32_t u0 = __float_as_uint(v.x), u1 = __float_as_uint(v.y), u2 = __float_as_uint(v.z), u3 = __float_as_uint(v.w);
      uint2 h, l;
      h.x = __builtin_amdgcn_perm(u1, u0, 0x07060302u);
      h.y = __builtin_amdgcn_perm(u3, u2, 0x07060302u);
      l.x = pack_bf16x2(v.x - __uint_as_float(u0 & 0xffff0000u), v.y - __uint_as_float(u1 & 0xffff0000u));
      l.y = pack_bf16x2(v.z - __uint_as_float(u2 & 0xffff0000u), v.w - __uint_as_float(u3 & 0xffff0000u));
      *(uint2*)(s_hi + r * LD + c) = h;
      *(uint2*)(s_lo + r * LD + c) = l;
    }
    lds_barrier();
    if (tile + gridDim.x < ntiles) fetch(tile + gridDim.x);

    f32x16 acc;
#pragma unroll
    for (int r = 0; r < 16; ++r) acc[r] = 0.f;
    const unsigned short *ah_p = s_hi + (rg * 32 + l31) * LD + 8 * lh, *al_p = s_lo + (rg * 32 + l31) * LD + 8 * lh;
#pragma unroll
    for (int s = 0; s < KS; ++s) {
      const bf16x8 ah = as_bf16x8(*(const uint4*)(ah_p + 16 * s)), al = as_bf16x8(*(const uint4*)(al_p + 16 * s));
      acc = __builtin_amdgcn_mfma_f32_32x32x16_bf16(ah, bh[s], acc, 0, 0, 0);
      acc = __builtin_amdgcn_mfma_f32_32x32x16_bf16(al, bh[s], acc, 0, 0, 0);
      acc = __builtin_amdgcn_mfma_f32_32x32x16_bf16(ah, bl[s], acc, 0, 0, 0);
    }
    if (col < p.N) {
      const int64_t row0 = tile * ROWS + rg * 32 + 4 * lh;
#pragma unroll
      for (int r = 0; r < 16; ++r) {
        const int64_t row = row0 + (r & 3) + 8 * (r >> 2);
        if (row < p.M) oz[row * p.ldc + col] = acc[r] + bv;
      }
    }
  }
#endif
}

}

extern "C" int siu3r_proj_rows_x3(const float* x, const void* wfrag, const float* bias, float* out, int Z, int G, int64_t M, int K, int N, int ldc,
                                  int64_t out_z_stride, void* stream) {
  SIU3R_CHECK(x && wfrag && out, "proj_rows_x3: null pointer");
  SIU3R_CHECK(Z > 0 && G > 0 && Z % G == 0 && M > 0 && N > 0 && ldc >= N, "proj_rows_x3: bad shape (Z=%d G=%d N=%d ldc=%d)", Z, G, N, ldc);
  ProjParams p{x, (const uint4*)wfrag, bias, out, M, out_z_stride > 0 ? out_z_stride : M * ldc, Z, G, N, ldc};
  const int nb = (N + 31) / 32;
  auto grid = [&](int rows) {
    const int64_t nt = (M + rows - 1) / rows;
    int64_t per = 256 / Z;
    if (per < 1) per = 1;
    return dim3((unsigned)(nt < per ? nt : per), Z);
  };
  hipStream_t s = (hipStream_t)stream;
  if (K == 256 && nb == 3)
    hipLaunchKernelGGL((proj_rows_x3_kernel<256, 3, 2>), grid(64), dim3(384), 0, s, p);
  else if (K == 128 && nb == 1)
    hipLaunchKernelGGL((proj_rows_x3_kernel<128, 1, 4>), grid(128), dim3(256), 0, s, p);
  else {
    siu3r_set_error("proj_rows_x3: no instantiation for K=%d N=%d (K 256 with N 65..96, K 128 with N <= 32)", K, N);
    return 1;
  }
  SIU3R_LAUNCH_CHECK("siu3r_proj_rows_x3");
  return 0;
}
```

### siu3r_amd/model.py

```python
from __future__ import annotations

import functools
import math
from typing import Dict, List, Optional, Sequence

import os

import torch
import torch.nn.functional as F

from . import ops
from .ops import ACT_GELU, ACT_NONE, ACT_RELU
from .gaussians_types import Gaussians
from . import postprocess as pp

ENC_HEADS, DEC_HEADS = 16, 12
ADAPTER_IDX = (5, 11, 17, 23)
DPT_HOOKS = (0, 6, 9, 12)


class _Weights:

    def __init__(self, sd: Dict[str, torch.Tensor], device, split: bool):
        self.sd, self.dev, self.split = sd, device, split
# ... 333 lines not shown
            other = {sides[0]: sides[1], sides[1]: sides[0]}
            build = lambda q: ops.cat_packed([W_.linear_ln_rows(q + ".attn.qkv", (0, 2 * Cc), q + ".norm1"),
                                              W_.linear_ln(other[q] + ".cross_attn.projk", other[q] + ".norm_y"),
                                              W_.linear_ln_rows(q + ".attn.qkv", (2 * Cc, 3 * Cc), q + ".norm1"),
                                              W_.linear_ln(other[q] + ".cross_attn.projv", other[q] + ".norm_y")])
            pj_buf = torch.empty((B, V, N + 1, 5 * Cc), dtype=ctx.act, device=x.device)
            pj = pj_buf.view(B * V, N + 1, 5, DEC_HEADS, hd)
            att = dict(heads=DEC_HEADS, head_dim=hd, scale=hd ** -0.5, split3=ctx.split)
            kvp = ops.Planes(pj_buf, storage=pj_buf) if (ctx.split and _KV_PLANES and ops.attention(pj[:, :, 0], pj[:, :, 1], pj[:, :, 3], dry_run=True, **att)) else None
            ops.linear_grouped(A(x, xb), grp("qkvx", build), ln=xs, rope=(rope[0], rope[1], pos, 3 * Cc), out=pj_buf, planes_out=kvp, planes_from_col=Cc)
            kvp = kvp is not None and kvp.valid
            self_qkv = (pj[:, :, 0], pj[:, :, 1], pj[:, :, 3])
        else:
            pj, kvp = None, False
            att = dict(heads=DEC_HEADS, head_dim=hd, scale=hd ** -0.5, split3=ctx.split)
            qkv = ops.linear_grouped(A(x, xb), grp("qkv", lambda q: W_.linear_ln(q + ".attn.qkv", q + ".norm1")), out_dtype=ctx.act, ln=xs,
                                     rope=(rope[0], rope[1], pos, 2 * Cc)).view(B * V, N + 1, 3, DEC_HEADS, hd)
            self_qkv = (qkv[:, :, 0], qkv[:, :, 1], qkv[:, :, 2])

        def attend(tag, wname, qkv_, res, S_out, **kw):
            xo, so, bo = S_out
            wp = grp(tag, lambda q: W_.linear(q + wname))
            a4 = torch.empty((B, V, N + 1, Cc), dtype=ctx.act, device=x.device)
            ap = _feeds_planes("dec_attn", ctx, a4, lambda t: ops.linear_grouped(t, wp, residual=res, out=xo, stats_out=so, aux_out=bo, dry_run=True))
            ops.attention(*qkv_, out=a4.view(B * V, N + 1, Cc), planes_out=ap, planes_only=True, **att, **kw)
            ops.linear_grouped(a4, wp, residual=res, out=xo, stats_out=so, aux_out=bo, a_planes=ap)

        S1 = x1, s1, b1 = self._new_stream(x)
        attend("proj", ".attn.proj", self_qkv, x, S1, kv_planes=kvp)
        qq = ops.linear_grouped(A(x1, b1), grp("projq", lambda q: W_.linear_ln(q + ".cross_attn.projq", q + ".norm2")), out_dtype=ctx.act, ln=s1,
                                rope=(rope[0], rope[1], pos, Cc)).view(B * V, N + 1, DEC_HEADS, hd)
        S2 = x2, s2, b2 = self._new_stream(x)
        if pj is not None:
            attend("xproj", ".cross_attn.proj", (qq, pj[:, :, 2], pj[:, :, 4]), x1, S2, kv_bxor=1, kv_planes=kvp)
        else:
            kv = ops.linear_grouped(A(x, xb), grp("projkv", lambda q: W_.linear_ln([q + ".cross_attn.projk", q + ".cross_attn.projv"], q + ".norm_y")),
                                    out_dtype=ctx.act, ln=xs, flip=True, rope=(rope[0], rope[1], pos, Cc)).view(B * V, N + 1, 2, DEC_HEADS, hd)
            attend("xproj", ".cross_attn.proj", (qq, kv[:, :, 0], kv[:, :, 1]), x1, S2)
        w1, w2 = grp("fc1", lambda q: W_.linear_ln(q + ".mlp.fc1", q + ".norm3")), grp("fc2", lambda q: W_.linear(q + ".mlp.fc2"))
        out2 = dict(residual=x2, out=d["g"][i + 1], stats_out=d["gstat"][i + 1], aux_out=d["gb16"][i + 1])
        h = torch.empty((B, V, N + 1, w1.n), dtype=ctx.act, device=x.device)
        hp = _feeds_planes("dec_fc", ctx, h, lambda t: ops.linear_grouped(t, w2, dry_run=True, **out2))
        ops.linear_grouped(A(x2, b2), w1, act=ACT_GELU, ln=s2, out=h, planes_out=hp, planes_only=True)
        ops.linear_grouped(h, w2, a_planes=hp, **out2)

    def decode_side(self, d, i, side):
        B, V, H, W, N = d["enc"]["dims"]
        g, g_next, rope = d["g"][i], d["g"][i + 1], d["rope"]
        if side == 0:
            mem0 = g[:, 1] if V == 2 else g[:, 1:].reshape(B, (V - 1) * (N + 1), -1)
            self._dec_block(f"backbone.dec_blocks.{i}", g[:, 0], mem0, d["pos0"], d["mem0_pos"], rope, out=g_next[:, 0])
            return
        if V == 2:
            xr, memr, outr = g[:, 1], g[:, 0], g_next[:, 1]
        else:
            xr = g[:, 1:].reshape(B * (V - 1), N + 1, -1)
            memr = torch.stack([torch.cat([g[:, j] for j in range(V) if j != v], dim=1) for v in range(1, V)], dim=1).flatten(0, 1)
            outr = g_next[0, 1:] if B == 1 else None
        r = self._dec_block(f"backbone.dec_blocks2.{i}", xr, memr, d["pos_rest"], d["memr_pos"], rope, out=outr)
        if outr is None:
            g_next[:, 1:].copy_(r.view(B, V - 1, N + 1, -1))

    def decode_end(self, d):
        B, V, H, W, N = d["enc"]["dims"]
        layers = [d["fv"]] + d["g"][1:]
        last = self.ctx.ln("backbone.dec_norm", layers[-1].reshape(B * V, N + 1, -1), 1e-6, out_dtype=torch.float32)
        layers[-1] = last.view(B, V, N + 1, -1)
        return dict(layers=layers, fv=d["fv"])

    def decode(self, enc):
        ctx = self.ctx
        d = self.decode_begin(enc)
        if d["merged"]:
            for i in range(self.dec_depth):
                self.decode_layer_merged(d, i)
            return self.decode_end(d)
        main = torch.cuda.current_stream()
        side = ctx.side_stream(0) if ctx.concurrent else main
        for i in range(self.dec_depth):
            if side is not main:
                side.wait_stream(main)
            self.decode_side(d, i, 0)
            with torch.cuda.stream(side):
                self.decode_side(d, i, 1)
            if side is not main:
                main.wait_stream(side)
        return self.decode_end(d)

    def _assemble(self, enc, dec):
        strip = lambda t: t[..., :-1, :]
        B, V, H, W, N = enc["dims"]
        feats = [strip(dec["fv"][:, v]) for v in range(V)]
        all_feats = [[strip(t[:, v]) for t in enc["av"]] for v in range(V)]
        decs = [[strip(t[:, v]) for t in dec["layers"]] for v in range(V)]
        return feats, all_feats, decs

    def forward(self, context: dict, symmetrize_batch=False, return_views=False):
        assert not symmetrize_batch, "symmetrize_batch is a training-time option"
        images, K = context["image"], context["intrinsics"]
        B, V, _, H, W = images.shape
        assert V == 2, "AsymmetricCroCo is the two-view backbone; use AsymmetricCroCoMulti for more views"
        enc = self.encode(images, K)
        dec = self.decode(enc)
        feats, all_feats, decs = self._assemble(enc, dec)
        shape = torch.tensor([[H, W]] * B)
        res = (feats[0], feats[1], all_feats[0], all_feats[1], decs[0], decs[1], shape, shape.clone())
        if return_views:
            res = res + ({"img": images[:, 0]}, {"img": images[:, 1]})
        return res

    __call__ = forward

    @property
    def patch_size(self):
        return 16

    @property
    def d_out(self):
        return 1024


class AsymmetricCroCoMulti(AsymmetricCroCo):

    def forward(self, context: dict, symmetrize_batch=False, return_views=False):
        assert not symmetrize_batch, "symmetrize_batch is a training-time option"
        images, K = context["image"], context["intrinsics"]
        B, V, _, H, W = images.shape
        enc = self.encode(images, K)
        dec = self.decode(enc)
        feats, all_feats, decs = self._assemble(enc, dec)
        shapes = [torch.tensor([[H, W]] * B) for _ in range(V)]
        res = (feats, all_feats, decs, shapes)
        if return_views:
            res = res + ([{"img": images[:, v]} for v in range(V)],)
        return res

    __call__ = forward


_PROJ_KERNEL = os.environ.get("SIU3R_NO_PROJ_KERNEL", "0") != "1"


def _head4(ctx, names, x, out=None):
    B, G, M, K = x.shape
    n = ctx.w.sd[names[0] + ".weight"].shape[0]
    if not (_PROJ_KERNEL and ctx.split and x.dtype == torch.float32 and x.is_contiguous() and ops.proj_rows_ok(K, n)):
        return None
    wf, wb, n = ctx.w.proj(tuple(names))
    if out is None:
        out = torch.empty((B, G, M, n), dtype=torch.float32, device=x.device)
    return ops.proj_rows_x3(x, wf, wb, n, out)


_STEM_KERNEL = os.environ.get("SIU3R_NO_STEM_KERNEL", "0") != "1"


def _stem_kernel_ok(ctx, img, path1, H, W) -> bool:
    return (_STEM_KERNEL and ctx.split and img.dtype == torch.float32 and img.shape[-1] == 4 and img.is_contiguous() and path1.dtype == torch.float32
            and path1.shape[-1] == 256 and path1.is_contiguous() and H % 16 == 0 and W % 16 == 0)


class _DPTHeads:

    def __init__(self, ctx: _Ctx, prefixes: Sequence[str], gs: bool):
        self.ctx, self.ps, self.gs = ctx, tuple(prefixes), gs
        self.grouped = len(self.ps) > 1

    def _w(self, kind: str, name: str):
        w = self.ctx.w
        if not self.grouped:
            return getattr(w, kind)(self.ps[0] + name)
        return w.group("pair:" + "|".join(self.ps) + ":" + name, lambda q: getattr(w, kind)(q + name), self.ps)

    def _rcu_planes(self) -> bool:
        return self.grouped and self.ctx.split and _CONV_PLANES

    def _stem_kernel_planes(self) -> bool:
        return _CONV_PLANES and not ops._NO_PRESPLIT

    def _stem_gemm_planes(self) -> bool:
        return self.grouped and self.ctx.split and _CONV_PLANES

    def _rcu(self, q, x, extra=None):
        ctx = self.ctx
        W = lambda name: self._w("conv", q + name)
        skip = lambda: x if extra is None else ops.affine_add(x.flatten(0, -4), extra.flatten(0, -4), None, None).view(x.shape)
        if self.grouped:
            W(".conv1"), W(".conv2")
            res = skip()
        if self._rcu_planes():
            o = torch.empty(x.shape[:-1] + (W(".conv1").n,), dtype=torch.float32, device=x.device)
            op = ops.Planes(o, storage=o)
            reads = bool(ops.conv2d(o, W(".conv2"), pad=1, residual=res, dry_run=True).a_x3_ok)
            ops.conv2d(x, W(".conv1"), pad=1, act=ACT_RELU, relu_in=True, out=o, planes_out=op if reads else None, planes_only=True)
            return ops.conv2d(o, W(".conv2"), pad=1, residual=res, a_planes=op if reads else None)
        o = ops.conv2d(x, W(".conv1"), pad=1, out_dtype=ctx.act, act=ACT_RELU, relu_in=True)
        if not self.grouped:
            res = skip()
        return ops.conv2d(o, W(".conv2"), pad=1, out_dtype=ctx.act, residual=res)

    def _fusion(self, q, x0, x1, reader=None):
        out = x0 if x1 is None else self._rcu(q + ".resConfUnit1", x1, extra=x0)
        out = self._rcu(q + ".resConfUnit2", out)
        lead, (hh, ww) = out.shape[:-3], out.shape[-3:-1]
        out = ops.linear(out.flatten(-3, -2), self._w("linear", q + ".out_conv"), out_dtype=self.ctx.act)
        up = torch.empty((*lead, 2 * hh, 2 * ww, out.shape[-1]), dtype=out.dtype, device=out.device)
        upp = _feeds_planes(reader[0], self.ctx, up, reader[1]) if reader is not None and _CONV_PLANES else None
        ops.resize_bilinear(out.view(-1, hh, ww, out.shape[-1]), (2 * hh, 2 * ww), True, out=up.view(-1, 2 * hh, 2 * ww, up.shape[-1]), planes_out=upp, planes_only=True)
        return up if reader is None else (up, upp)

    def trunk(self, tokens: Sequence[torch.Tensor], H, W, reader=None):
        ctx = self.ctx
        nh, nw = H // 16, W // 16
        layers = []
        for i, hk in enumerate(DPT_HOOKS):
            t = tokens[hk]
            a = f".dpt.act_postprocess.{i}"
            l = ops.linear(t, self._w("linear", a + ".0"), out_dtype=ctx.act).view(*t.shape[:-2], nh, nw, -1)
            if i in (0, 1):
                l = ops.conv_transpose2d(l, self._w("convT", a + ".1"), out_dtype=ctx.act)
            elif i == 3:
                l = ops.conv2d(l, self._w("conv", a + ".1"), stride=2, pad=1, out_dtype=ctx.act)
            layers.append(ops.conv2d(l, self._w("conv", f".dpt.scratch.layer_rn.{i}"), pad=1, out_dtype=ctx.act))
        s = ".dpt.scratch"
        path4 = self._fusion(s + ".refinenet4", layers[3], None)
        path3 = self._fusion(s + ".refinenet3", path4, layers[2])
        path2 = self._fusion(s + ".refinenet2", path3, layers[1])
        return self._fusion(s + ".refinenet1", path2, layers[0], reader)

    def _head4_names(self):
        return tuple(q + ".dpt.head.4" for q in self.ps)

    def forward_pts3d(self, tokens, H, W):
        ctx = self.ctx
        w0, w2 = self._w("conv", ".dpt.head.0"), self._w("conv", ".dpt.head.2")
        x, xp = self.trunk(tokens, H, W, reader=("pts_fusion", lambda t: ops.conv2d(t, w0, pad=1, dry_run=True)))
        x = ops.conv2d(x, w0, pad=1, out_dtype=ctx.act, a_planes=xp)
        lead = x.shape[:-3]
        up = torch.empty((*lead, H, W, x.shape[-1]), dtype=x.dtype, device=x.device)
        upp = _feeds_planes("pts_resize", ctx, up, lambda t: ops.conv2d(t, w2, pad=1, act=ACT_RELU, dry_run=True)) if _CONV_PLANES else None
        ops.resize_bilinear(x.flatten(0, -4), (H, W), True, out=up.view(-1, H, W, up.shape[-1]), planes_out=upp, planes_only=True)
        x = ops.conv2d(up, w2, pad=1, out_dtype=ctx.act, act=ACT_RELU, a_planes=upp)
        xyz = _head4(ctx, self._head4_names(), x.view(lead[0], len(self.ps), H * W, -1))
        if xyz is None:
            xyz = ops.linear(x.flatten(-3, -2), self._w("linear", ".dpt.head.4"), out_dtype=torch.float32)
        return ops.pts3d_exp_(xyz).view(*lead, H, W, 3)

    def forward_gs(self, tokens, img, H, W, out=None):
        ctx = self.ctx
        path1 = self.trunk(tokens, H, W)
        lead, G = path1.shape[:-3], len(self.ps)
        B = lead[0]
        assert B == 1 or G == 1
        x = torch.empty((*lead, H, W, path1.shape[-1]), dtype=ctx.act, device=ctx.dev)
        img5, up5, x5 = img.view(B, G, H, W, -1), path1.view(B, G, H // 2, W // 2, -1), x.view(B, G, H, W, -1)
        head0 = lambda: self._w("conv", ".dpt.head.0")
        stem = _stem_kernel_ok(ctx, img, path1, H, W)
        if self.grouped or stem:
            head0()
        xp = ops.Planes(x, storage=x) if (self._stem_gemm_planes() or (stem and self._stem_kernel_planes())) else None
        reads = xp is not None and bool(ops.conv2d(x, head0(), pad=1, act=ACT_RELU, dry_run=True).a_x3_ok)
        if stem:
            wf, wb = ctx.w.stem7(tuple(q + ".dpt.input_merger.0" for q in self.ps))
            reads = reads and self._stem_kernel_planes()
            ops.stem7x7_x3(img5, wf, wb, up5, x5, planes=reads)
        else:
            wrote = []
            for g, q in enumerate(self.ps):
                xg = ops.Planes(x5[:, g], storage=x5[:, g]) if reads else None
                ops.conv2d(img5[:, g], ctx.w.conv(q + ".dpt.input_merger.0", cin_pad=ops.image_channels(ctx.split)), pad=3, act=ACT_RELU,
                           up_src=up5[:, g], out=x5[:, g], planes_out=xg, planes_only=True)
                wrote.append(xg is not None and xg.valid)
            assert all(wrote) or not any(wrote), "the stems of a group run the same plan"
            reads = reads and all(wrote)
        if reads:
            xp.valid = xp.only = True
        x = ops.conv2d(x, head0(), pad=1, out_dtype=ctx.act, act=ACT_RELU, a_planes=xp if reads else None)
        if out is None:
            out = torch.empty((*lead, H * W, ctx.w.sd[self.ps[0] + ".dpt.head.4.weight"].shape[0]), dtype=torch.float32, device=ctx.dev)
        if _head4(ctx, self._head4_names(), x.view(B, G, H * W, -1), out=out if self.grouped else out.unsqueeze(1)) is None:
            ops.linear(x.flatten(-3, -2), self._w("linear", ".dpt.head.4"), out=out)
        return out


class UnifiedGaussianAdapter:

    def __init__(self, gaussian_scale_min=0.5, gaussian_scale_max=15.0, sh_degree=4):
        assert sh_degree == 4, "the HIP adapter kernel is specialised for sh_degree 4 (83 raw channels)"
        self.sh_degree = sh_degree

    @property
    def d_sh(self):
        return (self.sh_degree + 1) ** 2

    @property
    def d_in(self):
        return 7 + 3 * self.d_sh

    def forward(self, means, raw_gaussians, eps: float = 1e-8) -> Gaussians:
        g = ops.gaussian_adapter(raw_gaussians.contiguous())
        return Gaussians(means=means, **g)


class CroCoViTAdapter:
    def __init__(self, ctx: _Ctx, size):
        self.ctx = ctx
        self.H, self.W = size[0] // 16, size[1] // 16

    def _ref(self, Hi, Wi):
        key = ("adapter_ref", Hi, Wi)
        c = self.ctx.cache
        if key not in c:
            pts = []
            for (hh, ww) in ((Hi // 8, Wi // 8), (Hi // 16, Wi // 16), (Hi // 32, Wi // 32)):
                ry, rx = torch.meshgrid(torch.linspace(0.5, hh - 0.5, hh), torch.linspace(0.5, ww - 0.5, ww), indexing="ij")
                pts.append(torch.stack((rx.reshape(-1) / ww, ry.reshape(-1) / hh), -1))
            c[key] = torch.cat(pts, 0)[:, None, :].contiguous().to(self.ctx.dev)
        return c[key]

    def _extractor(self, p, c, ref, feat, h, w):
        ctx = self.ctx
        qn = ctx.ln(p + ".query_norm", c, 1e-6)
        fn = ctx.ln(p + ".feat_norm", feat, 1e-6)
        offs_aw = ops.linear(qn, ctx.w.merged(p + ".attn.offs_aw", [p + ".attn.sampling_offsets", p + ".attn.attention_weights"]), out_dtype=torch.float32)
        value = ops.linear(fn, ctx.w.linear(p + ".attn.value_proj"), out_dtype=ctx.act)
        wo = ctx.w.linear(p + ".attn.output_proj")
        samp = torch.empty((value.shape[0], offs_aw.shape[1], value.shape[2]), dtype=ctx.act, device=value.device)
        sp = _feeds_planes("ext_msd", ctx, samp, lambda t: ops.linear(t, wo, residual=c, dry_run=True))
        ops.msdeform_sample(value, offs_aw, ref, [(h, w)], 16, 4, ctx.act, out=samp, planes_out=sp, planes_only=True)
        c = ops.linear(samp, wo, out_dtype=torch.float32, residual=c, a_planes=sp)
        f1 = ops.linear(ctx.ln(p + ".ffn_norm", c, 1e-6), ctx.w.linear(p + ".ffn.fc1"), out_dtype=ctx.act)
        wk = p + ".ffn.dwconv.dwconv"
        if wk + "#w9c" not in ctx.w.vec:
            ctx.w.vec[wk + "#w9c"] = ctx.w.t(wk + ".weight").reshape(-1, 9).t().contiguous()
        w2 = ctx.w.linear(p + ".ffn.fc2")
        f2 = torch.empty_like(f1)
        fp = _feeds_planes("ext_dw", ctx, f2, lambda t: ops.linear(t, w2, residual=c, dry_run=True))
        ops.dwconv3x3_gelu(f1, ctx.w.vec[wk + "#w9c"], ctx.w.v(wk + ".bias"), h, w, out=f2, planes_out=fp, planes_only=True)
        return ops.linear(f2, w2, out_dtype=torch.float32, residual=c, a_planes=fp)

    def spm(self, img8: torch.Tensor):
        ctx = self.ctx
        Z, Hi, Wi, _ = img8.shape
        h, w = Hi // 16, Wi // 16
        sp = "adapter.spm"
        c = ops.conv2d(img8, ctx.w.conv(sp + ".stem.0", cin_pad=ops.image_channels(ctx.split), bn=sp + ".stem.1"), stride=2, pad=1, out_dtype=ctx.act, act=ACT_RELU)
        c = ops.conv2d(c, ctx.w.conv(sp + ".stem.3", bn=sp + ".stem.4"), pad=1, out_dtype=ctx.act, act=ACT_RELU)
        c = ops.conv2d(c, ctx.w.conv(sp + ".stem.6", bn=sp + ".stem.7"), pad=1, out_dtype=ctx.act, act=ACT_RELU)
        c1 = ops.maxpool3x3s2(c)
        c2 = ops.conv2d(c1, ctx.w.conv(sp + ".conv2.0", bn=sp + ".conv2.1"), stride=2, pad=1, out_dtype=ctx.act, act=ACT_RELU)
        c3 = ops.conv2d(c2, ctx.w.conv(sp + ".conv3.0", bn=sp + ".conv3.1"), stride=2, pad=1, out_dtype=ctx.act, act=ACT_RELU)
        c4 = ops.conv2d(c3, ctx.w.conv(sp + ".conv4.0", bn=sp + ".conv4.1"), stride=2, pad=1, out_dtype=ctx.act, act=ACT_RELU)
        le = ctx.w.v("adapter.level_embed")
        n2, n3, n4 = 4 * h * w, h * w, h * w // 4
        cc = torch.empty((Z, n2 + n3 + n4, 1024), dtype=torch.float32, device=ctx.dev)
        ops.linear(c2.view(Z, n2, -1), ctx.w.linear(sp + ".fc2", key=sp + ".fc2+le", extra_bias=le[0]), out=cc[:, :n2])
        ops.linear(c3.view(Z, n3, -1), ctx.w.linear(sp + ".fc3", key=sp + ".fc3+le", extra_bias=le[1]), out=cc[:, n2:n2 + n3])
        ops.linear(c4.view(Z, n4, -1), ctx.w.linear(sp + ".fc4", key=sp + ".fc4+le", extra_bias=le[2]), out=cc[:, n2 + n3:])
        return dict(c1_feat=c1, cc=cc, outs=[], dims=(Z, Hi, Wi, h, w, n2, n3, n4), ref=self._ref(Hi, Wi))

    def interact(self, a, i, x):
        Z, Hi, Wi, h, w, n2, n3, n4 = a["dims"]
        a["cc"] = self._extractor(f"adapter.interactions.{i}.extractor", a["cc"], a["ref"], x, h, w)
        if i == 3:
            for j in range(2):
                a["cc"] = self._extractor(f"adapter.interactions.3.extra_extractors.{j}", a["cc"], a["ref"], x, h, w)
        a["outs"].append(x.view(Z, h, w, -1))

    LATERAL = "mask2former.model.pixel_decoder.adapter_1.0"

    def _lateral_weights(self):
        W_ = self.ctx.w
        key = "adapter.lateral_fused"
        if key + ".y1" not in W_.lin:
            d = torch.float64
            w_lat = W_.t(self.LATERAL + ".weight").reshape(256, -1).to(d)
            b_lat = W_.t(self.LATERAL + ".bias").to(d) if (self.LATERAL + ".bias") in W_.sd else torch.zeros(256, dtype=d, device=W_.dev)
            s1, b1 = (t.to(d) for t in W_.bn_affine("adapter.norm1"))
            w_up, b_up = W_.t("adapter.up.weight").to(d), W_.t("adapter.up.bias").to(d)
            w_fc1 = W_.t("adapter.spm.fc1.weight").reshape(w_up.shape[1], -1).to(d)
            b_fc1 = W_.t("adapter.spm.fc1.bias").to(d)
            wa = w_lat * s1[None, :]
            W_.lin[key + ".y1"] = ops.pack_matrix(wa.float(), None, W_.split)
            W_.lin[key + ".up"] = ops.pack_conv_transpose(torch.einsum("pc,icyx->ipyx", wa, w_up).float(), None, W_.split)
            W_.lin[key + ".c1"] = ops.pack_matrix((wa @ w_fc1).float(), (w_lat @ b1 + wa @ (b_up + b_fc1) + b_lat).float(), W_.split)
        return W_.lin[key + ".y1"], W_.lin[key + ".up"], W_.lin[key + ".c1"]

    def finish(self, a, with_f1: bool = False):
        ctx = self.ctx
        Z, Hi, Wi, h, w, n2, n3, n4 = a["dims"]
        cc = a["cc"]
        c2 = (cc[:, :n2] if ctx.split else cc[:, :n2].to(ctx.act)).view(Z, 2 * h, 2 * w, -1)
        c3 = cc[:, n2:n2 + n3].view(Z, h, w, -1)
        c4 = cc[:, n2 + n3:].view(Z, h // 2, w // 2, -1)
        x1, x2, x3, x4 = a["outs"]
        pw_y1, pw_up, pw_c1 = self._lateral_weights()
        y1 = ops.linear(x1.view(Z, h * w, -1), pw_y1, out_dtype=torch.float32).view(Z, h, w, 256)
        t1 = ops.linear(a["c1_feat"].view(Z, 16 * h * w, -1), pw_c1, out_dtype=torch.float32).view(Z, 4 * h, 4 * w, 256)
        u1 = ops.resize_bilinear(y1, (4 * h, 4 * w), False, addend=t1, out_dtype=torch.float32)
        a["lat1"] = ops.conv_transpose2d(c2, pw_up, out_dtype=torch.float32, residual=u1)
        s2, b2 = ctx.w.bn_affine("adapter.norm2")
        s3, b3 = ctx.w.bn_affine("adapter.norm3")
        s4, b4 = ctx.w.bn_affine("adapter.norm4")
        f1 = None
        if with_f1:
            s1, b1 = ctx.w.bn_affine("adapter.norm1")
            c1 = ops.linear(a["c1_feat"], ctx.w.linear("adapter.spm.fc1"), out_dtype=torch.float32)
            c1 = ops.conv_transpose2d(c2, ctx.w.convT("adapter.up"), out_dtype=torch.float32, residual=c1)
            f1 = ops.resize_bilinear(x1, (4 * h, 4 * w), False, addend=c1, ch_scale=s1, ch_shift=b1, out_dtype=ctx.act)
        f2 = ops.resize_bilinear(x2, (2 * h, 2 * w), False, addend=c2, ch_scale=s2, ch_shift=b2, out_dtype=ctx.act)
        f3 = ops.affine_add(x3, c3, s3, b3, out_dtype=ctx.act)
        f4 = ops.resize_bilinear(x4, (h // 2, w // 2), False, addend=c4, ch_scale=s4, ch_shift=b4, out_dtype=ctx.act)
        return [f1, f2, f3, f4]

    def forward_nhwc(self, img: torch.Tensor, img8: torch.Tensor, all_feat: Sequence[torch.Tensor]):
        a = self.spm(img8)
        for i, idx in enumerate(ADAPTER_IDX):
            self.interact(a, i, all_feat[idx])
        return self.finish(a, with_f1=True)

    def forward(self, x, all_feat):
        img8 = ops.pack_image_nhwc(x.contiguous().float(), self.ctx.act, ops.image_channels(self.ctx.split))
        return [f.permute(0, 3, 1, 2) for f in self.forward_nhwc(x, img8, all_feat)]

    __call__ = forward


def _sine_pos_2d(h, w, npf=128):
    y = torch.arange(1, h + 1, dtype=torch.float32)[:, None].expand(h, w)
    x = torch.arange(1, w + 1, dtype=torch.float32)[None, :].expand(h, w)
    eps, scale = 1e-6, 2 * math.pi
    y = y / (y[-1:, :] + eps) * scale
    x = x / (x[:, -1:] + eps) * scale
# ... 146 lines not shown
            wkey, key = ("m2f_kvw", lvl), ("m2f_kv", T, sizes[lvl])
            if wkey not in ctx.cache:
                wk, wv, bk, bv = [], [], [], []
                for idx in (lvl, lvl + 3, lvl + 6):
                    wi, bi = ctx.w.t(f"{dp}.layers.{idx}.cross_attn.in_proj_weight"), ctx.w.t(f"{dp}.layers.{idx}.cross_attn.in_proj_bias")
                    wk.append(wi[256:512]); wv.append(wi[512:]); bk.append(bi[256:512]); bv.append(bi[512:])
                wkk = torch.cat(wk, 0)
                ctx.cache[wkey] = (ops.pack_matrix(torch.cat((wkk, torch.cat(wv, 0)), 0), None, ctx.split), wkk, torch.cat(bk, 0), torch.cat(bv, 0))
            pw, wkk, bkk, bvv = ctx.cache[wkey]
            if key not in ctx.cache:
                posk = pos3[lvl] @ wkk.t() + bkk
                ctx.cache[key] = torch.cat((posk, bvv[None].expand(posk.shape[0], -1)), 1).contiguous()
            res = ctx.cache[key]
            kv = ops.linear(feats[lvl], pw, out_dtype=ctx.act, residual=res if B == 1 else res[None].expand(B, -1, -1))
            kvs.append(kv.view(B, -1, 6, 8, 32))
        Q = self.num_queries
        qf = ctx.w.v(tm + ".queries_features.weight")
        qe = ctx.w.v(tm + ".queries_embedder.weight")
        hs = qf.unsqueeze(0).expand(B, -1, -1).contiguous()
        hsb = hs if ctx.split else hs.to(ctx.act)
        d = 32
        inter, interb = ctx.ln2(dp + ".layernorm", hs, 1e-5)
        masks, inters = [], [inter]
        m, am = self._mask_predictor(interb, mf_bt, sizes[0])
        masks.append(m)
        for idx in range(9):
            p = f"{dp}.layers.{idx}"
            lvl = idx % 3
            if p + ".cross_attn.q" not in ctx.w.lin:
                wi, bi = ctx.w.t(p + ".cross_attn.in_proj_weight"), ctx.w.t(p + ".cross_attn.in_proj_bias")
                ctx.w.lin[p + ".cross_attn.q"] = ops.pack_matrix(wi[:256], None, ctx.split)
                ctx.cache[p + ".cross_attn.qres"] = (qe @ wi[:256].t() + bi[:256]).contiguous()
                wq, wk_ = ctx.w.t(p + ".self_attn.q_proj.weight"), ctx.w.t(p + ".self_attn.k_proj.weight")
                bq, bk_ = ctx.w.t(p + ".self_attn.q_proj.bias"), ctx.w.t(p + ".self_attn.k_proj.bias")
                wqk = torch.cat((wq, wk_), 0)
                ctx.w.lin[p + ".self_attn.qk0"] = ops.pack_matrix(wqk, None, ctx.split)
                ctx.cache[p + ".self_attn.qkres"] = (qe @ wqk.t() + torch.cat((bq, bk_), 0)).contiguous()
            bres = (lambda r: r if B == 1 else r[None].expand(B, -1, -1))
            q = ops.linear(hsb, ctx.w.lin[p + ".cross_attn.q"], out_dtype=ctx.act, residual=bres(ctx.cache[p + ".cross_attn.qres"])).view(B, Q, 8, d)
            j = idx // 3
            k, v = kvs[lvl][:, :, j], kvs[lvl][:, :, 3 + j]
            if self.forced_attn_masks is not None:
                fm = self.forced_attn_masks[idx].to(ctx.dev, torch.uint8)
                am = torch.zeros((B, Q, ((fm.shape[-1] + 63) // 64) * 64), dtype=torch.uint8, device=ctx.dev)
                am[..., :fm.shape[-1]] = fm
            if self.record_attn_masks is not None:
                self.record_attn_masks.append(am.clone())
            a = ops.attention(q, k, v, heads=8, head_dim=d, scale=d ** -0.5, mask=am, split3=ctx.split)
            a = ops.linear(a, ctx.w.linear(p + ".cross_attn.out_proj"), out_dtype=torch.float32, residual=hs)
            hs, hsb = ctx.ln2(p + ".cross_attn_layer_norm", a, 1e-5)
            qk = ops.linear(hsb, ctx.w.lin[p + ".self_attn.qk0"], out_dtype=ctx.act, residual=bres(ctx.cache[p + ".self_attn.qkres"])).view(B, Q, 2, 8, d)
            v = ops.linear(hsb, ctx.w.linear(p + ".self_attn.v_proj"), out_dtype=ctx.act).view(B, Q, 8, d)
            a = ops.attention(qk[:, :, 0], qk[:, :, 1], v, heads=8, head_dim=d, scale=d ** -0.5, split3=ctx.split)
            a = ops.linear(a, ctx.w.linear(p + ".self_attn.out_proj"), out_dtype=torch.float32, residual=hs)
            hs, hsb = ctx.ln2(p + ".self_attn_layer_norm", a, 1e-5)
            f_ = ops.linear(hsb, ctx.w.linear(p + ".fc1"), out_dtype=ctx.act, act=ACT_RELU)
            f_ = ops.linear(f_, ctx.w.linear(p + ".fc2"), out_dtype=torch.float32, residual=hs)
            hs, hsb = ctx.ln2(p + ".final_layer_norm", f_, 1e-5)
            inter, interb = ctx.ln2(dp + ".layernorm", hs, 1e-5)
            m, am = self._mask_predictor(interb, mf_bt, sizes[(idx + 1) % 3])
            masks.append(m)
            inters.append(inter)
        class_logits = ops.linear(interb, ctx.w.linear("mask2former.class_predictor"), out_dtype=torch.float32)
        return class_logits, masks[-1], masks, inters

    def forward_nhwc(self, feats_nhwc: Sequence[torch.Tensor], B: int, T: int, lat1=None):
        mask_features, ms = self._pixel_decoder(feats_nhwc, lat1)
        class_logits, mask_cl, all_masks, inters = self._decoder(ms, mask_features, B, T)
        out = VideoMask2FormerForVideoSegmentationOutput(
            loss=None, class_queries_logits=class_logits,
            masks_queries_logits=mask_cl.permute(0, 4, 1, 2, 3),
            auxiliary_logits=None, attentions=None, word_embeddings=None,
        )
        out["_masks_channel_last"] = mask_cl
        out["_mask_features"], out["_ms"] = mask_features, ms
        return out

    def forward(self, multi_scale_feat: List[torch.Tensor], word_embeddings=None, mask_labels=None, class_labels=None, **kw):
        assert word_embeddings is None and mask_labels is None and class_labels is None, "inference path only"
        B, T = multi_scale_feat[0].shape[:2]
        feats = [f.flatten(0, 1).permute(0, 2, 3, 1).contiguous() for f in multi_scale_feat]
        return self.forward_nhwc(feats, B, T)

    __call__ = forward


_KV_PLANES = not os.environ.get("SIU3R_NO_KV_PLANES")
_CONV_PLANES = not os.environ.get("SIU3R_NO_CONV_PLANES")
_PRODUCER_PLANES_SITES = ("enc_attn", "dec_attn", "dec_fc", "pts_resize", "pts_fusion", "ext_msd", "ext_dw")
_PRODUCER_PLANES_DEFAULT = ("enc_attn", "pts_resize", "pts_fusion")
_PRODUCER_PLANES = frozenset(s_ for s_ in os.environ.get("SIU3R_PRODUCER_PLANES", ",".join(_PRODUCER_PLANES_DEFAULT)).split(",") if s_)
assert _PRODUCER_PLANES <= set(_PRODUCER_PLANES_SITES), _PRODUCER_PLANES


def _feeds_planes(site: str, ctx, like: torch.Tensor, plan) -> Optional[ops.Planes]:
    if site not in _PRODUCER_PLANES or ops._NO_PRESPLIT or not ctx.split or like.dtype != torch.float32:
        return None
    return ops.Planes(like, storage=like) if plan(like).a_x3_ok else None


_DEC_QKVX = not os.environ.get("SIU3R_NO_DEC_QKVX")
_HEAD_PAIRS = os.environ.get("SIU3R_NO_HEAD_PAIRS", "0") != "1"
_DEC_PER_LAYER = os.environ.get("SIU3R_DEC_PER_LAYER", "0") == "1"

_MAIN, _SEG, _DEC, _H0, _H1 = range(5)


@functools.lru_cache(maxsize=None)
def _schedule(paired: bool, merged: bool, dec_depth: int, pipelined: bool):
    steps = [("run", _MAIN, "enc_begin"), ("wait", _SEG, _MAIN), ("run", _SEG, "spm")]
    for k in range(len(ADAPTER_IDX)):
        steps += [("run", _MAIN, f"enc{k}"), ("wait", _SEG, _MAIN), ("run", _SEG, f"int{k}")]
    steps += [("run", _SEG, "seg"), ("after_seg", _SEG, None), ("run", _MAIN, "dec_pre")]
    if merged:
        steps += [("run", _MAIN, f"dec{i}") for i in range(dec_depth)] if _DEC_PER_LAYER else [("run", _MAIN, "dec_all")]
    for i in range(0 if merged else dec_depth):
        steps += [("wait", _DEC, _MAIN), ("run", _MAIN, f"decA{i}"), ("run", _DEC, f"decB{i}"), ("wait", _MAIN, _DEC)]
    steps += [("run", _MAIN, "dec_post"), ("wait", _H0, _MAIN), ("wait", _H1, _MAIN), ("wait", _SEG, _MAIN)]
    if paired:
        steps += [("run", _H0, "gs"), ("run", _H1 if pipelined else _MAIN, "pts")]
    else:
        steps += [("run", _H0, "gs0"), ("run", _H1, "gsr"), ("run", _H0 if pipelined else _MAIN, "ptsr"), ("run", _SEG, "pts0")]
    tail = _H1 if pipelined else _MAIN
    steps += [("wait", tail, _H0), ("wait", tail, _H1), ("wait", tail, _SEG), ("wait", tail, _SEG), ("run", tail, "tail")]
    return tuple(steps), tail


_PANOPTIC_TABLES = ("tab", "probs", "kept_idx", "acc_list", "p256", "seg", "sem", "ins")


class _PendingForward:

    def __init__(self, model, st, caller, host_slot, eager, replayed, lift, return_intermediates):
        self._model, self._out, self.done = model, None, False
        self.st, self.caller, self.host_slot, self.eager, self.replayed = st, caller, host_slot, eager, replayed
        self.lift, self.return_intermediates = lift, return_intermediates
        self.seg_out = self.pend = self.gaussians = None
        self.tail_stream = caller

    def result(self):
        if not self.done:
            self._out, self.done = self._model._finish(self), True
            self._model = self.st = self.seg_out = self.pend = self.gaussians = None
        return self._out


class _Run:

    def __init__(self, images, K):
        self.images, self.K = images, K
        self.img_bv = self.img8 = self.enc = self.adapter = self.dstate = self.dec = self.ms = self.seg = self.gaussians = None
        self.gs, self.pts, self.raw = [None, None], [None, None], None
        self.want_f1 = False


class SIU3RModel:
    def __init__(self, state_dict: Dict[str, torch.Tensor], image_size=(512, 512), precision="bf16", device="cuda",
                 num_queries=100, seg_threshold=0.5, label_ids_to_fuse=(0, 1), sh_degree=4):
        if not torch.cuda.is_available():
            raise RuntimeError("SIU3RModel (siu3r_amd) needs an MI355X GPU: there is no CPU fallback")
        self.image_size = tuple(image_size)
        self.precision = precision
        self.seg_threshold, self.label_ids_to_fuse = seg_threshold, set(label_ids_to_fuse)
        sd = {k[len("model."):] if k.startswith("model.") else k: v for k, v in state_dict.items()}
        self._w = _Weights(sd, torch.device(device), precision == "bf16x3")
        self._ctx = _Ctx(self._w, precision)
        self.backbone = AsymmetricCroCo(self._ctx)
        self.adapter = CroCoViTAdapter(self._ctx, image_size)
        self.mask2former = VideoMask2FormerForVideoSegmentation(self._ctx, num_queries)
        pts, gs = ("downstream_head1", "downstream_head2"), ("gaussian_param_head1", "gaussian_param_head2")
        self.downstream_head1, self.downstream_head2 = (_DPTHeads(self._ctx, (q,), gs=False) for q in pts)
        self.gaussian_param_head1, self.gaussian_param_head2 = (_DPTHeads(self._ctx, (q,), gs=True) for q in gs)
        self.gs_pair, self.pts_pair = _DPTHeads(self._ctx, gs, gs=True), _DPTHeads(self._ctx, pts, gs=False)
        self.gaussian_adapter = UnifiedGaussianAdapter(sh_degree=sh_degree)
        self.processor = pp.VideoMask2FormerImageProcessor()
        self.raw_gs_dim = (sh_degree + 1) ** 2 * 3 + 3 + 4 + 1
        self.use_graph = os.environ.get("SIU3R_NO_GRAPH", "0") != "1"
        self._graphs: Dict = {}
        self.pipeline_depth = max(1, int(os.environ.get("SIU3R_PIPELINE_DEPTH", "2")))
        self._next_slot = 0
        self._inflight: Dict = {}
        self._timeline = None

    def eval(self):
        return self

    def release_source_weights(self):
        self._w.sd = {k: v for k, v in self._w.sd.items() if v.numel() <= 65536}

    def forward(self, context_views_images, context_views_intrinsics, mask_labels=None, class_labels=None,
                enable_query_class_logit_lift=False, return_intermediates=False):
        if self._inflight.get(0) is not None and not self._inflight[0].done:
            raise RuntimeError("SIU3RModel.forward: a forward_async() of slot 0 is still pending; call its result() first")
        return self._submit(context_views_images, context_views_intrinsics, mask_labels, class_labels, enable_query_class_logit_lift,
                            return_intermediates, slot=None).result()

    def forward_async(self, context_views_images, context_views_intrinsics, mask_labels=None, class_labels=None,
                      enable_query_class_logit_lift=False):
        slot = self._next_slot
        prev = self._inflight.get(slot)
        if prev is not None and not prev.done:
            raise RuntimeError(f"SIU3RModel.forward_async: {self.pipeline_depth} steps are already pending; call result() on the oldest first")
        self._next_slot = (slot + 1) % self.pipeline_depth
        h = self._submit(context_views_images, context_views_intrinsics, mask_labels, class_labels, enable_query_class_logit_lift, False, slot=slot)
        self._inflight[slot] = h
        return h

    def _submit(self, context_views_images, context_views_intrinsics, mask_labels, class_labels, enable_query_class_logit_lift,
                return_intermediates, slot):
        assert mask_labels is None and class_labels is None, "inference path only (training losses are out of scope)"
        ctx = self._ctx
        images = context_views_images.to(ctx.dev)
        K = context_views_intrinsics.to(ctx.dev)
        B, V, _, H, W = images.shape
        key = (B, V, H, W, images.dtype, K.dtype)
        eager = (not self.use_graph) or return_intermediates or ops.kernel_timer_active() or torch.cuda.is_current_stream_capturing()
        ent = None if eager else self._graphs.get(key)
        replayed = ent is not None
        caller = torch.cuda.current_stream()
        sidx = 0 if slot is None else slot
        pipelined = slot is not None and ctx.concurrent
        if replayed:
            sl = ent["slots"].get(sidx)
            if sl is None:
                sl = ent["slots"][sidx] = self._capture_slot(ent, key, images, K)
                if sidx == 0:
                    ent["graphs"], ent["st"] = sl["graphs"], sl["st"]
            st = sl["st"]
        else:
            st = _Run(images, K)
            st.want_f1 = bool(return_intermediates)
        h = _PendingForward(self, st, caller, sidx, eager, replayed, enable_query_class_logit_lift, return_intermediates)
        after_seg = functools.partial(self._after_seg, h)
        if replayed:
            if sl.get("done") is not None:
                caller.wait_event(sl["done"])
            st.images.copy_(images, non_blocking=True)
            st.K.copy_(K, non_blocking=True)
            h.tail_stream = self._run_stages(st, functools.partial(self._replay_stage, sl), after_seg, pipelined=pipelined)
            if pipelined:
                sl["done"] = torch.cuda.Event()
                sl["done"].record(h.tail_stream)
        elif eager:
            self._run_stages(st, lambda name, fn: fn(), after_seg)
        else:
            ent = self._graphs[key] = {"graphs": None, "st": None, "slots": {}, "need": {}}
            self._run_stages(st, functools.partial(self._meter_stage, ent["need"]), after_seg)
        h.gaussians = st.gaussians
        return h

    @staticmethod
    def _meter_stage(need, name, fn):
        with ops.splitk_meter() as m:
            fn()
        need[name] = m

    def _replay_stage(self, sl, name, fn):
        tl = self._timeline
        if tl is not None:
            e0, e1 = torch.cuda.Event(enable_timing=True), torch.cuda.Event(enable_timing=True)
            e0.record()
        fn() if name == "tail" else sl["graphs"][name].replay()
        if tl is not None:
            e1.record()
            tl.append((name, e0, e1))

    def _after_seg(self, h):
        st = h.st
        B, _, _, H, W = st.images.shape
        seg_o = st.seg
        if h.replayed:
            seg_o = VideoMask2FormerForVideoSegmentationOutput(st.seg)
            for k_ in ("class_queries_logits", "masks_queries_logits"):
                seg_o[k_] = seg_o[k_].clone()
                seg_o[k_].record_stream(h.caller)
        pend = self.processor.begin_panoptic(seg_o, threshold=self.seg_threshold, target_sizes=[(H, W)] * B,
                                             label_ids_to_fuse=self.label_ids_to_fuse, host_slot=h.host_slot)
        for k_ in _PANOPTIC_TABLES:
            pend[k_].record_stream(h.caller)
        h.seg_out, h.pend = seg_o, pend

    def _finish(self, h):
        st, seg_out, gaussians = h.st, h.seg_out, h.gaussians
        B, V, _, H, W = st.images.shape
        cur = torch.cuda.current_stream()
        if h.tail_stream is not cur:
            cur.wait_stream(h.tail_stream)
            for _, v_ in gaussians.items():
                if isinstance(v_, torch.Tensor):
                    v_.record_stream(cur)
        if cur is not h.caller:
            for k_ in _PANOPTIC_TABLES:
                h.pend[k_].record_stream(cur)
        results = self.processor.finish_panoptic(h.pend)
        if not h.eager:
            for k_ in ("_masks_channel_last", "_mask_features", "_ms"):
                seg_out.pop(k_, None)
        g_, masks, infos, qcl, qscores = pp.post_process_gaussians(gaussians, results, B, V, H, W, h.lift)
        if h.return_intermediates:
            _, _, decs = self.backbone._assemble(st.enc, st.dec)
            all1 = [t[:, 0, :-1] for t in st.enc["av"]]
            all2 = [t[:, 1, :-1] for t in st.enc["av"]]
            self._last = dict(dec1=decs[0], dec2=decs[1], decs=decs, all_feat1=all1, all_feat2=all2, ms=st.ms, lat1=st.adapter["lat1"], pts1=st.pts[0],
                              pts2=st.pts[1], gs_raw1=st.gs[0].reshape(B, H, W, -1), gs_raw2=st.gs[1].reshape(-1, H, W, st.gs[1].shape[-1]), seg_out=st.seg)
        if h.lift:
            return g_, seg_out, masks, infos, qscores
        return g_, seg_out, masks, infos

    def _capture_slot(self, ent, key, images, K):
        ctx = self._ctx
        sl = {"st": _Run(images.clone(), K.clone()), "graphs": {}, "ws": {}}
        st = sl["st"]
        torch.cuda.synchronize()
        conc, ctx.concurrent = ctx.concurrent, False
        try:
            for name, fn in self._stages(st):
                if name == "tail":
                    continue
                m = ent["need"].get(name)
                ws = sl["ws"][name] = m.workspace(ctx.dev) if m is not None else None
                g = torch.cuda.CUDAGraph()
                with ops.splitk_scope(ws):
                    with torch.cuda.graph(g, capture_error_mode="thread_local"):
                        fn()
                sl["graphs"][name] = g
        finally:
            ctx.concurrent = conc
        torch.cuda.synchronize()
        return sl

    def _stages(self, st):
        bb = self.backbone

        def dec_pre():
            st.dstate = bb.decode_begin(st.enc)
            B, V, _, H, W = st.images.shape
            st.raw = torch.empty((B, V, H * W, self.raw_gs_dim), dtype=torch.float32, device=self._ctx.dev)

        def dec_post():
            st.dec = bb.decode_end(st.dstate)

        dec = [("dec_pre", dec_pre)]
        if self._merged_decoder(st) and not _DEC_PER_LAYER:
            dec += [("dec_all", lambda: [bb.decode_layer_merged(st.dstate, i) for i in range(bb.dec_depth)])]
        for i in range(bb.dec_depth):
            if self._merged_decoder(st):
                if _DEC_PER_LAYER:
                    dec += [(f"dec{i}", lambda i=i: bb.decode_layer_merged(st.dstate, i))]
            else:
                dec += [(f"decA{i}", lambda i=i: bb.decode_side(st.dstate, i, 0)), (f"decB{i}", lambda i=i: bb.decode_side(st.dstate, i, 1))]
        dec += [("dec_post", dec_post)]
        ad = self.adapter
        bounds = [0] + [i + 1 for i in ADAPTER_IDX]

        def enc_seg(k):
            bb.encode_blocks(st.enc, bounds[k], bounds[k + 1])
            if k == len(ADAPTER_IDX) - 1:
                if bounds[-1] < bb.enc_depth:
                    bb.encode_blocks(st.enc, bounds[-1], bb.enc_depth)
                bb.encode_end(st.enc)

        def interact(k):
            B, V, _, H, W = st.images.shape
            t = st.enc["all_feat"][ADAPTER_IDX[k]].view(B * V, -1, bb.enc_embed_dim)[:, :-1]
            ad.interact(st.adapter, k, t)

        enc = [("enc_begin", lambda: self._s_encode_begin(st)), ("spm", lambda: setattr(st, "adapter", ad.spm(st.img8)))]
        for k in range(len(ADAPTER_IDX)):
            enc += [(f"enc{k}", lambda k=k: enc_seg(k)), (f"int{k}", lambda k=k: interact(k))]
        if self._paired_heads(st):
            heads = [("gs", lambda: self._s_head(st, True)), ("pts", lambda: self._s_head(st, False))]
        else:
            heads = [("gs0", lambda: self._s_head(st, True, 0)), ("gsr", lambda: self._s_head(st, True, 1)), ("pts0", lambda: self._s_head(st, False, 0)),
                     ("ptsr", lambda: self._s_head(st, False, 1))]
        return enc + [("seg", lambda: self._s_seg(st))] + dec + heads + [("tail", lambda: self._s_tail(st))]

    def _paired_heads(self, st) -> bool:
        B, V = st.images.shape[:2]
        return _HEAD_PAIRS and V == 2 and B == 1

    def _merged_decoder(self, st) -> bool:
        return self._ctx.fold and st.images.shape[1] == 2

    def _run_stages(self, st, run, after_seg=None, pipelined=False):
        ctx = self._ctx
        stages = dict(self._stages(st))
        main = torch.cuda.current_stream()
        streams = (main, ctx.side_stream(1), ctx.side_stream(0), ctx.side_stream(2), ctx.side_stream(3)) if ctx.concurrent else (main,) * 5
        steps, tail = _schedule(self._paired_heads(st), self._merged_decoder(st), self.backbone.dec_depth, bool(pipelined))
        for op, x, arg in steps:
            x = streams[x]
            if op == "wait":
                if x is not streams[arg]:
                    x.wait_stream(streams[arg])
            elif op == "after_seg" and after_seg is None:
                pass
            elif x is main:
                run(arg, stages[arg]) if op == "run" else after_seg()
            else:
                with torch.cuda.stream(x):
                    run(arg, stages[arg]) if op == "run" else after_seg()
        return streams[tail]

    def _s_encode_begin(self, st):
        ctx = self._ctx
        B, V, _, H, W = st.images.shape
        st.img_bv = st.images.reshape(B * V, 3, H, W).contiguous().float()
        st.img8 = ops.pack_image_nhwc(st.img_bv, ctx.act, ops.image_channels(ctx.split))
        st.enc = self.backbone.encode_begin(st.images, st.K)

    def _s_seg(self, st):
        B, V, _, H, W = st.images.shape
        st.ms = self.adapter.finish(st.adapter, with_f1=st.want_f1)
        st.seg = self.mask2former.forward_nhwc(st.ms, B, V, lat1=st.adapter["lat1"])

    @staticmethod
    def _rest_views(t):
        r = t[:, 1:]
        return r[0] if t.shape[0] == 1 else (r[:, 0] if t.shape[1] == 2 else r.reshape(-1, *t.shape[2:]))

    def _s_head(self, st, gs: bool, side=None):
        B, V, _, H, W = st.images.shape
        views = (lambda t: t) if side is None else (lambda t: t[:, 0]) if side == 0 else self._rest_views
        toks = [views(t)[..., :-1, :] for t in st.dec["layers"]]
        heads = (self.gs_pair, self.gaussian_param_head1, self.gaussian_param_head2) if gs else (self.pts_pair, self.downstream_head1, self.downstream_head2)
        head = heads[0 if side is None else 1 + side]
        if gs:
            dst = st.raw if side is None else st.raw[:, side] if (side == 0 or V == 2) else (st.raw[0, 1:] if B == 1 else None)
            r = head.forward_gs(toks, views(st.img8.view(B, V, H, W, -1)).contiguous(), H, W, out=dst)
        else:
            r = head.forward_pts3d(toks, H, W)
        res = st.gs if gs else st.pts
        if side is None:
            res[:] = [r[:, 0], r[:, 1]]
        else:
            res[side] = r

    def _s_tail(self, st):
        B, V, _, H, W = st.images.shape
        cat = lambda a, b_: torch.cat((a.reshape(B, 1, H * W, -1), b_.reshape(B, V - 1, H * W, -1)), dim=1)
        raw = st.raw if (V == 2 or B == 1) else cat(st.gs[0], st.gs[1])
        st.gaussians = self.gaussian_adapter.forward(cat(st.pts[0], st.pts[1]), raw)

    __call__ = forward


class SIU3RMultiViewModel(SIU3RModel):

    def __init__(self, *args, **kw):
        super().__init__(*args, **kw)
        self.backbone = AsymmetricCroCoMulti(self._ctx)
```

### siu3r_amd/ops.py

```python
from __future__ import annotations

import ctypes as C
import math
import os
from dataclasses import dataclass
from typing import Optional, Sequence

import torch

from . import _lib
from ._lib import BF16, F32, AttnParams, GemmParams, check

ACT_NONE, ACT_GELU, ACT_RELU = 0, 1, 2


def _dt(t: torch.Tensor) -> int:
    if t.dtype == torch.float32:
        return F32
    if t.dtype == torch.bfloat16:
        return BF16
    raise RuntimeError(f"unsupported dtype {t.dtype} (float32 or bfloat16 expected)")


def torch_dtype(code: int):
# ... 612 lines not shown
        if splits > 1:
            p.splits = splits
            ws = torch.empty((B, heads, splits, qt * 128, head_dim + 4), dtype=torch.float32, device=q.device)
            p.ws = _p(ws)
    if dry_run:
        return bool(_lib.lib().siu3r_attention_kv_x3_ok(C.byref(p))) and not _NO_PRESPLIT
    if plan:
        pl = _lib.AttnPlan()
        check(_lib.lib().siu3r_attention_plan(C.byref(p), C.byref(pl)))
        return pl

    def planes_ok():
        p.out = _p(planes_out.t)
        ok = bool(_lib.lib().siu3r_attention_out_x3_ok(C.byref(p)))
        p.out = _p(out)
        return ok

    if _producer_planes(planes_out, planes_only, out, planes_ok):
        p.out, p.out_x3 = _p(planes_out.t), 1
    check(_lib.lib().siu3r_attention(C.byref(p), _stream()))
    return out


def attention_plan(q, k, v, **kw):
    return attention(q, k, v, plan=True, **kw)


def layernorm2(x: torch.Tensor, gamma, beta, eps: float):
    _gpu(x)
    assert x.dtype == torch.float32 and x.is_contiguous()
    Cc = x.shape[-1]
    rows = x.numel() // Cc
    out = torch.empty(x.shape, dtype=torch.float32, device=x.device)
    out2 = torch.empty(x.shape, dtype=torch.bfloat16, device=x.device)
    check(_lib.lib().siu3r_layernorm2(_p(x), _p(out), F32, _p(out2), _p(gamma), _p(beta), rows, Cc, Cc, Cc, Cc, eps, _stream()))
    return out, out2


def layernorm(x: torch.Tensor, gamma, beta, eps: float, out_dtype=torch.float32):
    _gpu(x)
    assert x.dtype == torch.float32 and x.stride(-1) == 1
    Cc = x.shape[-1]
    rows = x.numel() // Cc
    x2 = x.reshape(rows, Cc) if x.is_contiguous() else x
    out = torch.empty(x.shape, dtype=out_dtype, device=x.device)
    if x.is_contiguous():
        ldx = Cc
    else:
        assert x.dim() == 3
        for b in range(x.shape[0]):
            check(_lib.lib().siu3r_layernorm(_p(x[b]), _p(out[b]), _dt(out), _p(gamma), _p(beta), x.shape[1], Cc,
                                             x.stride(1), Cc, eps, _stream()))
        return out
    check(_lib.lib().siu3r_layernorm(_p(x2), _p(out), _dt(out), _p(gamma), _p(beta), rows, Cc, ldx, Cc, eps, _stream()))
    return out


def add(a: torch.Tensor, b: torch.Tensor):
    _gpu(a, b)
    assert a.is_contiguous() and b.is_contiguous() and a.dtype == torch.float32 and b.dtype == torch.float32
    Cc = a.shape[-1]
    y = torch.empty_like(a)
    check(_lib.lib().siu3r_add(_p(a), _p(b), _p(y), a.numel() // Cc, b.numel() // Cc, Cc, _stream()))
    return y


def pack_image_nhwc(img: torch.Tensor, out_dtype, cpad: int = 8):
    _gpu(img)
    assert img.dtype == torch.float32 and img.is_contiguous() and img.shape[1] == 3
    N, _, H, W = img.shape
    out = torch.empty((N, H, W, cpad), dtype=out_dtype, device=img.device)
    check(_lib.lib().siu3r_pack_image_nhwc(_p(img), _p(out), _dt(out), N, H, W, cpad, _stream()))
    return out


def pack_image_nhwc8(img: torch.Tensor, out_dtype):
    return pack_image_nhwc(img, out_dtype, 8)


def pack_stem7(weights: Sequence[torch.Tensor], biases: Sequence[Optional[torch.Tensor]]):
    frs = []
    for w in weights:
        _gpu(w)
        assert tuple(w.shape) == (256, 3, 7, 7), w.shape
        wk = torch.zeros((256, 7, 8, 4), dtype=torch.float32, device=w.device)
        wk[:, :, :7, :3] = w.detach().float().permute(0, 2, 3, 1)
        wk = wk.reshape(256, 14, 2, 8)
        fr = wk.reshape(8, 32, 14, 2, 8).permute(0, 2, 3, 1, 4)
        fr = fr.reshape(8, 14, 64, 8)
        hi = fr.to(torch.bfloat16)
        lo = (fr - hi.float()).to(torch.bfloat16)
        frs.append(torch.stack([hi, lo], dim=2))
    b = None
    if any(x is not None for x in biases):
        b = torch.stack([torch.zeros(256, device=weights[0].device) if x is None else x.detach().float() for x in biases]).contiguous()
    return torch.stack(frs).contiguous(), b


def stem7x7_x3(img: torch.Tensor, wfrag: torch.Tensor, bias: Optional[torch.Tensor], up_src: Optional[torch.Tensor], out: torch.Tensor, planes: bool = False):
    _gpu(img, wfrag, bias, up_src, out)
    B, G, H, W, c = img.shape
    assert c == 4 and img.dtype == torch.float32 and img.is_contiguous() and tuple(wfrag.shape) == (G, 8, 14, 2, 64, 8) and wfrag.dtype == torch.bfloat16
    assert out.shape == (B, G, H, W, 256) and out.dtype == torch.float32 and out.is_contiguous()
    assert bias is None or (tuple(bias.shape) == (G, 256) and bias.is_contiguous())
    assert up_src is None or (up_src.shape == (B, G, H // 2, W // 2, 256) and up_src.dtype == torch.float32 and up_src.is_contiguous())
    check(_lib.lib().siu3r_stem7x7_x3(_p(img), _p(wfrag), _p(bias), _p(up_src), _p(out), B, G, H, W, 1 if planes else 0, _stream()))
    return out


def _proj_fragments(w: torch.Tensor) -> torch.Tensor:
    w = w.detach().float().reshape(w.shape[0], -1)
    N, K = w.shape
    NB = (N + 31) // 32
    assert K % 16 == 0
    wp = torch.zeros((NB * 32, K), dtype=torch.float32, device=w.device)
    wp[:N] = w
    fr = wp.reshape(NB, 32, K // 16, 2, 8).permute(0, 2, 3, 1, 4).reshape(NB, K // 16, 64, 8)
    hi = fr.to(torch.bfloat16)
    lo = (fr - hi.float()).to(torch.bfloat16)
    return torch.stack([hi, lo], dim=2)


def pack_proj(weights: Sequence[torch.Tensor], biases: Sequence[Optional[torch.Tensor]]):
    frs, N = [], None
    for w in weights:
        _gpu(w)
        N = w.shape[0]
        frs.append(_proj_fragments(w))
    b = None
    if any(x is not None for x in biases):
        NB = frs[0].shape[0]
        b = torch.zeros((len(weights), NB * 32), dtype=torch.float32, device=frs[0].device)
        for i, x in enumerate(biases):
            if x is not None:
                b[i, :N] = x.detach().float()
    return torch.stack(frs).contiguous(), b, N


def proj_rows_x3(x: torch.Tensor, wfrag: torch.Tensor, bias: Optional[torch.Tensor], n: int, out: torch.Tensor):
    _gpu(x, wfrag, bias, out)
    B, G, M, K = x.shape
    assert x.dtype == torch.float32 and x.is_contiguous() and wfrag.shape[0] == G and wfrag.dtype == torch.bfloat16
    assert out.shape == (B, G, M, n) and out.dtype == torch.float32 and out.stride(3) == 1 and out.stride(2) >= n
    zs = out.stride(1) if G > 1 else out.stride(0)
    assert zs >= M * out.stride(2) and (B == 1 or G == 1 or out.stride(0) == G * zs), (out.shape, out.stride())
    check(_lib.lib().siu3r_proj_rows_x3(_p(x), _p(wfrag), _p(bias), _p(out), B * G, G, M, K, n, out.stride(2), zs, _stream()))
    return out


def proj_rows_ok(K: int, n: int) -> bool:
    return (K == 256 and 65 <= n <= 96) or (K == 128 and n <= 32)


def pack_rowchain(wo, bo, g1, b1, w1, c1, w2, c2, g2, b2) -> torch.Tensor:
    H = w1.shape[0]
    assert tuple(wo.shape) == (256, 256) and tuple(w1.shape) == (H, 256) and tuple(w2.shape) == (256, H) and H > 0 and H % 256 == 0
    vec = [bo, g1, b1, c2, g2, b2, c1]
    assert all(v.numel() == (H if v is c1 else 256) for v in vec)
    parts = [_proj_fragments(w).contiguous().view(torch.uint8).reshape(-1) for w in (wo, w1, w2)]
    parts.append(torch.cat([v.detach().float().reshape(-1) for v in vec]).contiguous().view(torch.uint8))
    return torch.cat(parts).contiguous()


def unpack_rowchain(pack: torch.Tensor, H: int) -> dict:
    def mat(buf, N, K):
        fr = buf.view(torch.bfloat16).reshape(N // 32, K // 16, 2, 2, 32, 8).double()
        return (fr[:, :, 0] + fr[:, :, 1]).permute(0, 3, 1, 2, 4).reshape(N, K)
    pack = pack.cpu()
    o1, o2, o3 = 256 * 256 * 4, 256 * 256 * 4 + H * 256 * 4, 256 * 256 * 4 + 2 * H * 256 * 4
    assert pack.dtype == torch.uint8 and pack.numel() == o3 + (6 * 256 + H) * 4
    vec = pack[o3:].view(torch.float32)
    out = {"wo": mat(pack[:o1], 256, 256), "w1": mat(pack[o1:o2], H, 256), "w2": mat(pack[o2:o3], 256, H)}
    for i, k in enumerate(("bo", "g1", "b1", "c2", "g2", "b2")):
        out[k] = vec[256 * i:256 * (i + 1)].clone()
    out["c1"] = vec[6 * 256:].clone()
    return out


def rowchain_ok(x: torch.Tensor, res: torch.Tensor, split: bool) -> bool:
    return bool(split) and all(t.dtype == torch.float32 and t.is_contiguous() and t.dim() >= 2 and t.shape[-1] == 256 for t in (x, res)) \
        and x.shape == res.shape


def rowchain_x3(x: torch.Tensor, res: torch.Tensor, pack: torch.Tensor, H: int, eps1: float, eps2: float, out: Optional[torch.Tensor] = None):
    _gpu(x, res, pack, out)
    assert rowchain_ok(x, res, True), (x.shape, x.dtype, res.shape, res.dtype)
    assert pack.dtype == torch.uint8 and pack.numel() == (256 * 256 + 2 * H * 256) * 4 + (6 * 256 + H) * 4
    if out is None:
        out = torch.empty_like(x)
    assert out.shape == x.shape and out.dtype == torch.float32 and out.is_contiguous()
    M = x.numel() // 256
    if M:
        check(_lib.lib().siu3r_rowchain_x3(_p(x), _p(res), _p(pack), _p(out), M, H, eps1, eps2, _stream()))
    return out


def image_channels(split: bool) -> int:
    return 4 if split else 8


def _batch_strided(t: torch.Tensor, inner: int) -> int:
    dense = list(torch.empty(t.shape[1:], device="meta").stride())
    assert list(t.stride()[1:]) == dense and (t.shape[0] == 1 or t.stride(0) >= inner), (t.shape, t.stride())
    return t.stride(0) if t.shape[0] > 1 else inner


def resize_bilinear(x: torch.Tensor, size, align_corners: bool, *, addend=None, ch_scale=None, ch_shift=None,
                    out_dtype=None, out: Optional[torch.Tensor] = None, planes_out: Optional[Planes] = None, planes_only: bool = False):
    _gpu(x, addend, out)
    N, IH, IW, Cc = x.shape
    OH, OW = size
    if out is None:
        out = torch.empty((N, OH, OW, Cc), dtype=out_dtype or x.dtype, device=x.device)
    assert out.shape == (N, OH, OW, Cc) and out.is_contiguous()
    x_bs = _batch_strided(x, IH * IW * Cc)
    if _producer_planes(planes_out, planes_only, out, lambda: addend is None and ch_scale is None and Cc % 32 == 0 and planes_out.t.data_ptr() % 128 == 0):
        check(_lib.lib().siu3r_resize_bilinear_planes(_p(x), _dt(x), _p(planes_out.t), N, IH, IW, OH, OW, Cc, int(align_corners), x_bs, _stream()))
        return out
    a_bs = OH * OW * Cc
    if addend is not None:
        assert addend.shape == out.shape
        a_bs = _batch_strided(addend, OH * OW * Cc)
    check(_lib.lib().siu3r_resize_bilinear_strided(_p(x), _dt(x), _p(out), _dt(out), _p(addend), _dt(addend) if addend is not None else F32,
                                                   _p(ch_scale), _p(ch_shift), N, IH, IW, OH, OW, Cc, int(align_corners), x_bs, a_bs, _stream()))
    return out


def affine_add(x: torch.Tensor, addend, ch_scale, ch_shift, out_dtype=None):
    _gpu(x, addend)
    Cc = x.shape[-1]
    rows_pb = math.prod(x.shape[1:-1])
    x_bs = _batch_strided(x, rows_pb * Cc)
    a_bs = rows_pb * Cc
    if addend is not None:
        assert addend.numel() == x.numel()
        a_bs = _batch_strided(addend.view(x.shape) if addend.is_contiguous() else addend, rows_pb * Cc)
    out = torch.empty(x.shape, dtype=out_dtype or x.dtype, device=x.device)
    check(_lib.lib().siu3r_affine_add_strided(_p(x), _dt(x), _p(addend), _dt(addend) if addend is not None else F32, _p(out), _dt(out), _p(ch_scale),
                                              _p(ch_shift), x.shape[0] * rows_pb, Cc, rows_pb, x_bs, a_bs, _stream()))
    return out


def maxpool3x3s2(x: torch.Tensor):
    _gpu(x)
    assert x.is_contiguous()
    N, IH, IW, Cc = x.shape
    out = torch.empty((N, (IH - 1) // 2 + 1, (IW - 1) // 2 + 1, Cc), dtype=x.dtype, device=x.device)
    check(_lib.lib().siu3r_maxpool3x3s2(_p(x), _p(out), _dt(x), N, IH, IW, Cc, _stream()))
    return out


def maxpool2x2s2(x: torch.Tensor):
    _gpu(x)
    assert x.is_contiguous()
    N, IH, IW, Cc = x.shape
    out = torch.empty((N, IH // 2, IW // 2, Cc), dtype=x.dtype, device=x.device)
    check(_lib.lib().siu3r_maxpool2x2s2(_p(x), _p(out), _dt(x), N, IH, IW, Cc, _stream()))
    return out


def lpips_layer(f0: torch.Tensor, f1: torch.Tensor, w: torch.Tensor, eps: float) -> torch.Tensor:
    _gpu(f0, f1, w)
    assert f0.shape == f1.shape and f0.is_contiguous() and f1.is_contiguous() and w.is_contiguous()
    assert f0.dtype == f1.dtype == w.dtype == torch.float32 and w.numel() == f0.shape[-1]
    dist = torch.empty(f0.shape[:-1], dtype=torch.float32, device=f0.device)
    check(_lib.lib().siu3r_lpips_layer(_p(f0), _p(f1), _p(w), _p(dist), dist.numel(), f0.shape[-1], float(eps), _stream()))
    return dist


def dwconv3x3_gelu(x: torch.Tensor, w9c: torch.Tensor, bias: torch.Tensor, H: int, W: int, *, out: Optional[torch.Tensor] = None,
                   planes_out: Optional[Planes] = None, planes_only: bool = False):
    _gpu(x, out)
    assert x.is_contiguous()
    B, N, Cc = x.shape
    assert N == 21 * (H * W // 4)
    if out is None:
        out = torch.empty_like(x)
    assert out.shape == x.shape and out.dtype == x.dtype and out.is_contiguous()
    if _producer_planes(planes_out, planes_only, out, lambda: x.dtype == torch.float32 and Cc % 32 == 0 and planes_out.t.data_ptr() % 128 == 0):
        check(_lib.lib().siu3r_dwconv3x3_gelu_planes(_p(x), _p(planes_out.t), _p(w9c), _p(bias), B, H, W, Cc, _stream()))
        return out
    check(_lib.lib().siu3r_dwconv3x3_gelu(_p(x), _p(out), _dt(x), _p(w9c), _p(bias), B, H, W, Cc, _stream()))
    return out


def msdeform_sample(value: torch.Tensor, offs_aw: torch.Tensor, ref: torch.Tensor, shapes: Sequence[Sequence[int]],
                    heads: int, points: int, out_dtype, *, out: Optional[torch.Tensor] = None, planes_out: Optional[Planes] = None,
                    planes_only: bool = False):
    _gpu(value, offs_aw, ref, out)
    assert value.is_contiguous() and offs_aw.is_contiguous() and ref.is_contiguous() and offs_aw.dtype == torch.float32
    B, S, Cc = value.shape
    Q = offs_aw.shape[1]
    L = len(shapes)
    d = Cc // heads
    assert offs_aw.shape[2] == heads * L * points * 3 and ref.shape == (Q, L, 2)
    if out is None:
        out = torch.empty((B, Q, Cc), dtype=out_dtype, device=value.device)
    assert out.shape == (B, Q, Cc) and out.is_contiguous()
    arr = (C.c_int32 * (2 * L))(*[int(v) for s in shapes for v in s])
    if _producer_planes(planes_out, planes_only, out, lambda: L in (1, 3, 4) and points == 4 and Cc % 32 == 0 and offs_aw.data_ptr() % 16 == 0
                        and planes_out.t.data_ptr() % 128 == 0):
        check(_lib.lib().siu3r_msdeform_sample_planes(_p(value), _dt(value), _p(offs_aw), _p(ref), arr, _p(planes_out.t), B, S, Q, heads, d, L, points, _stream()))
        return out
    check(_lib.lib().siu3r_msdeform_sample(_p(value), _dt(value), _p(offs_aw), _p(ref), arr, _p(out), _dt(out), B, S, Q,
                                           heads, d, L, points, _stream()))
    return out
# ... 72 lines not shown
```

Baseline: 57.55.

## Fuse gaussian adapter and pts3d exp into head projection epilogues

After: 57.69, median of 6. Within noise of the previous version (+0.2%).

```diff
diff --git a/include/siu3r_hip.h b/include/siu3r_hip.h
--- a/include/siu3r_hip.h
+++ b/include/siu3r_hip.h
@@ -138,6 +138,10 @@
                      int planes_out, void* stream);
 int siu3r_proj_rows_x3(const float* x, const void* wfrag, const float* bias, float* out, int Z, int G, int64_t M, int K, int N, int ldc,
                        int64_t out_z_stride, void* stream);
+int siu3r_proj_rows_x3_gaussians(const float* x, const void* wfrag, const float* bias, float* raw_or_null, float* opacities, float* scales,
+                                 float* rotations, float* harmonics, float* covariances, int Z, int G, int64_t M, int K, int N, void* stream);
+int siu3r_proj_rows_x3_pts3d(const float* x, const void* wfrag, const float* bias, float* out, int Z, int G, int64_t M, int K, int N, int ldc,
+                             int64_t out_z_stride, void* stream);
 int siu3r_rowchain_x3(const float* x, const float* res, const void* pack, float* out, int64_t M, int H, float eps1, float eps2, void* stream);
 int siu3r_dwconv3x3_gelu(const void* x, void* y, int dtype, const float* w9c, const float* bias, int B, int H,
                          int W, int C, void* stream);
diff --git a/siu3r_amd/_lib.py b/siu3r_amd/_lib.py
--- a/siu3r_amd/_lib.py
+++ b/siu3r_amd/_lib.py
@@ -117,6 +117,8 @@
     "siu3r_lpips_layer": [_P, _P, _P, _P, _L, _I, _F, _P],
     "siu3r_stem7x7_x3": [_P, _P, _P, _P, _P, _I, _I, _I, _I, _I, _P],
     "siu3r_proj_rows_x3": [_P, _P, _P, _P, _I, _I, _L, _I, _I, _I, _L, _P],
+    "siu3r_proj_rows_x3_gaussians": [_P, _P, _P, _P, _P, _P, _P, _P, _P, _I, _I, _L, _I, _I, _P],
+    "siu3r_proj_rows_x3_pts3d": [_P, _P, _P, _P, _I, _I, _L, _I, _I, _I, _L, _P],
     "siu3r_rowchain_x3": [_P, _P, _P, _P, _L, _I, _F, _F, _P],
     "siu3r_dwconv3x3_gelu": [_P, _P, _I, _P, _P, _I, _I, _I, _I, _P],
     "siu3r_dwconv3x3_gelu_planes": [_P, _P, _P, _P, _I, _I, _I, _I, _P],
diff --git a/siu3r_amd/csrc/elementwise.hip b/siu3r_amd/csrc/elementwise.hip
--- a/siu3r_amd/csrc/elementwise.hip
+++ b/siu3r_amd/csrc/elementwise.hip
@@ -1,4 +1,5 @@
 #include "common.h"
+#include "gaussian_rows.h"
 
 namespace {
 
@@ -568,13 +569,11 @@
 __global__ void pts3d_kernel(float* xyz, int64_t n) {
   const int64_t i = (int64_t)blockIdx.x * blockDim.x + threadIdx.x;
   if (i >= n) return;
-  const float x = xyz[i * 3], y = xyz[i * 3 + 1], z = xyz[i * 3 + 2];
-  const float d = sqrtf(x * x + y * y + z * z);
-  const float dc = fmaxf(d, 1e-8f);
-  const float e = expm1f(d);
-  xyz[i * 3] = x / dc * e;
-  xyz[i * 3 + 1] = y / dc * e;
-  xyz[i * 3 + 2] = z / dc * e;
+  float x = xyz[i * 3], y = xyz[i * 3 + 1], z = xyz[i * 3 + 2];
+  pts3d_row(x, y, z);
+  xyz[i * 3] = x;
+  xyz[i * 3 + 1] = y;
+  xyz[i * 3 + 2] = z;
 }
 
 constexpr int GA_ROWS = 128, GA_D = 83, GA_SH = 75;
@@ -596,45 +595,7 @@
   __syncthreads();
   const int t = threadIdx.x;
   if (t < rows) {
-    const float* r = s + t * GA_D;
-    opac[g0 + t] = 1.f / (1.f + expf(-r[0]));
-    float sc[3];
-#pragma unroll
-    for (int j = 0; j < 3; ++j) {
-      const float x = r[1 + j];
-      const float sp = x > 20.f ? x : log1pf(expf(x));
-      sc[j] = fminf(0.001f * sp, 0.3f);
-      so[t * 17 + j] = sc[j];
-    }
-    const float qi = r[4], qj = r[5], qk = r[6], qr = r[7];
-    so[t * 17 + 3] = qi; so[t * 17 + 4] = qj; so[t * 17 + 5] = qk; so[t * 17 + 6] = qr;
-    const float nrm = sqrtf(qi * qi + qj * qj + qk * qk + qr * qr) + 1e-8f;
-    const float i_ = qi / nrm, j_ = qj / nrm, k_ = qk / nrm, r_ = qr / nrm;
-    const float two_s = 2.f / ((i_ * i_ + j_ * j_ + k_ * k_ + r_ * r_) + 1e-8f);
-    float R[9];
-    R[0] = 1.f - two_s * (j_ * j_ + k_ * k_);
-    R[1] = two_s * (i_ * j_ - k_ * r_);
-    R[2] = two_s * (i_ * k_ + j_ * r_);
-    R[3] = two_s * (i_ * j_ + k_ * r_);
-    R[4] = 1.f - two_s * (i_ * i_ + k_ * k_);
-    R[5] = two_s * (j_ * k_ - i_ * r_);
-    R[6] = two_s * (i_ * k_ - j_ * r_);
-    R[7] = two_s * (j_ * k_ + i_ * r_);
-    R[8] = 1.f - two_s * (i_ * i_ + j_ * j_);
-    float M[9];
-#pragma unroll
-    for (int a = 0; a < 3; ++a)
-#pragma unroll
-      for (int b = 0; b < 3; ++b) M[a * 3 + b] = R[a * 3 + b] * sc[b];
-#pragma unroll
-    for (int a = 0; a < 3; ++a)
-#pragma unroll
-      for (int b = 0; b < 3; ++b) {
-        float v = 0.f;
-#pragma unroll
-        for (int k2 = 0; k2 < 3; ++k2) v += (M[a * 3 + k2] * sc[k2]) * R[b * 3 + k2];
-        so[t * 17 + 7 + a * 3 + b] = v;
-      }
+    opac[g0 + t] = gaussian_row(s + t * GA_D, so + t * 17);
   }
   __syncthreads();
   for (int i = threadIdx.x; i < rows * 3; i += nt) scales[g0 * 3 + i] = so[(i / 3) * 17 + i % 3];
@@ -646,14 +607,14 @@
 #pragma unroll
       for (int u = 0; u < 4; ++u) {
         const int i = i4 * 4 + u, rr = i / GA_SH, e = i - rr * GA_SH;
-        v[u] = s[rr * GA_D + 8 + e] * c_sh_mask[e % 25];
+        v[u] = gaussian_sh(s[rr * GA_D + 8 + e], c_sh_mask[e % 25]);
       }
       ((float4*)(sh + g0 * GA_SH))[i4] = make_float4(v[0], v[1], v[2], v[3]);
     }
   } else {
     for (int i = threadIdx.x; i < rows * GA_SH; i += nt) {
       const int rr = i / GA_SH, e = i - rr * GA_SH;
-      sh[g0 * GA_SH + i] = s[rr * GA_D + 8 + e] * c_sh_mask[e % 25];
+      sh[g0 * GA_SH + i] = gaussian_sh(s[rr * GA_D + 8 + e], c_sh_mask[e % 25]);
     }
   }
 }
@@ -965,12 +926,7 @@
   static bool mask_set = false;
   if (!mask_set) {
     float m[25];
-    m[0] = 1.f;
-    for (int deg = 1; deg <= 4; ++deg) {
-      float v = 0.1f;
-      for (int i = 0; i < deg; ++i) v *= 0.25f;
-      for (int i = deg * deg; i < (deg + 1) * (deg + 1); ++i) m[i] = v;
-    }
+    gaussian_sh_mask(m);
     if (hipMemcpyToSymbol(HIP_SYMBOL(c_sh_mask), m, sizeof(m)) != hipSuccess) {
       siu3r_set_error("gaussian_adapter: cannot upload SH mask");
       return 2;
diff --git a/siu3r_amd/csrc/gaussian_rows.h b/siu3r_amd/csrc/gaussian_rows.h
--- /dev/null
+++ b/siu3r_amd/csrc/gaussian_rows.h
@@ -0,0 +1,64 @@
+#pragma once
+#include <hip/hip_runtime.h>
+
+static inline void gaussian_sh_mask(float m[25]) {
+  m[0] = 1.f;
+  for (int deg = 1; deg <= 4; ++deg) {
+    float v = 0.1f;
+    for (int i = 0; i < deg; ++i) v *= 0.25f;
+    for (int i = deg * deg; i < (deg + 1) * (deg + 1); ++i) m[i] = v;
+  }
+}
+
+__device__ __forceinline__ float gaussian_row(const float* r, float* so) {
+  const float opac = 1.f / (1.f + expf(-r[0]));
+  float sc[3];
+#pragma unroll
+  for (int j = 0; j < 3; ++j) {
+    const float x = r[1 + j];
+    const float sp = x > 20.f ? x : log1pf(expf(x));
+    sc[j] = fminf(0.001f * sp, 0.3f);
+    so[j] = sc[j];
+  }
+  const float qi = r[4], qj = r[5], qk = r[6], qr = r[7];
+  so[3] = qi; so[4] = qj; so[5] = qk; so[6] = qr;
+  const float nrm = sqrtf(qi * qi + qj * qj + qk * qk + qr * qr) + 1e-8f;
+  const float i_ = qi / nrm, j_ = qj / nrm, k_ = qk / nrm, r_ = qr / nrm;
+  const float two_s = 2.f / ((i_ * i_ + j_ * j_ + k_ * k_ + r_ * r_) + 1e-8f);
+  float R[9];
+  R[0] = 1.f - two_s * (j_ * j_ + k_ * k_);
+  R[1] = two_s * (i_ * j_ - k_ * r_);
+  R[2] = two_s * (i_ * k_ + j_ * r_);
+  R[3] = two_s * (i_ * j_ + k_ * r_);
+  R[4] = 1.f - two_s * (i_ * i_ + k_ * k_);
+  R[5] = two_s * (j_ * k_ - i_ * r_);
+  R[6] = two_s * (i_ * k_ - j_ * r_);
+  R[7] = two_s * (j_ * k_ + i_ * r_);
+  R[8] = 1.f - two_s * (i_ * i_ + j_ * j_);
+  float M[9];
+#pragma unroll
+  for (int a = 0; a < 3; ++a)
+#pragma unroll
+    for (int b = 0; b < 3; ++b) M[a * 3 + b] = R[a * 3 + b] * sc[b];
+#pragma unroll
+  for (int a = 0; a < 3; ++a)
+#pragma unroll
+    for (int b = 0; b < 3; ++b) {
+      float v = 0.f;
+#pragma unroll
+      for (int k2 = 0; k2 < 3; ++k2) v += (M[a * 3 + k2] * sc[k2]) * R[b * 3 + k2];
+      so[7 + a * 3 + b] = v;
+    }
+  return opac;
+}
+
+__device__ __forceinline__ float gaussian_sh(float raw, float mask) { return raw * mask; }
+
+__device__ __forceinline__ void pts3d_row(float& x, float& y, float& z) {
+  const float d = sqrtf(x * x + y * y + z * z);
+  const float dc = fmaxf(d, 1e-8f);
+  const float e = expm1f(d);
+  x = x / dc * e;
+  y = y / dc * e;
+  z = z / dc * e;
+}
diff --git a/siu3r_amd/csrc/proj.hip b/siu3r_amd/csrc/proj.hip
--- a/siu3r_amd/csrc/proj.hip
+++ b/siu3r_amd/csrc/proj.hip
@@ -1,4 +1,5 @@
 #include "common.h"
+#include "gaussian_rows.h"
 
 namespace {
 
@@ -9,18 +10,40 @@
   float* out;
   int64_t M, out_zs;
   int Z, G, N, ldc;
+  float *opac, *scales, *rots, *sh, *cov;
+  float sh_mask[25];
 };
 
 __device__ __forceinline__ void lds_barrier() { asm volatile("s_waitcnt lgkmcnt(0)\n\ts_barrier" ::: "memory"); }
 
-template <int K, int NB, int RG>
+template <class F>
+__device__ __forceinline__ void store_span(float* dst, int n, int tid, int nthreads, F get) {
+  int head = (int)((16u - ((uint32_t)(uintptr_t)dst & 15u)) >> 2) & 3;
+  if (head > n) head = n;
+  const int n4 = (n - head) >> 2, tail0 = head + 4 * n4;
+  for (int i = tid; i < n4; i += nthreads) {
+    const int b = head + 4 * i;
+    *(float4*)(dst + b) = make_float4(get(b), get(b + 1), get(b + 2), get(b + 3));
+  }
+  for (int i = tid; i < head + (n - tail0); i += nthreads) {
+    const int j = i < head ? i : tail0 + (i - head);
+    dst[j] = get(j);
+  }
+}
+
+constexpr int FIN_LD = 97;
+
+template <int K, int NB, int RG, int FIN>
 __global__ __launch_bounds__(64 * NB * RG) void proj_rows_x3_kernel(const ProjParams p) {
+  static_assert(FIN == 0 || (FIN == 1 && K == 256 && NB == 3 && RG == 2) || (FIN == 2 && K == 128 && NB == 1 && RG == 4), "no such finishing epilogue");
 #if __HIP_DEVICE_COMPILE__
   constexpr int NT = 64 * NB * RG, ROWS = 32 * RG, KS = K / 16;
   constexpr int LD = K + 8;
   constexpr int PIECES = ROWS * K / 4;
   constexpr int PPT = (PIECES + NT - 1) / NT;
   __shared__ __attribute__((aligned(16))) unsigned short s_hi[ROWS * LD], s_lo[ROWS * LD];
+  __shared__ float s_row[FIN == 1 ? ROWS * FIN_LD : 1], s_so[FIN == 1 ? ROWS * 17 : 1], s_mask[FIN == 1 ? 32 : 1];
+  __shared__ float s_xyz[FIN == 2 ? RG * 96 : 1];
   const int t = threadIdx.x, lane = t & 63, wave = t >> 6;
   const int nb = wave % NB, rg = wave / NB;
   const int z = blockIdx.y, g = z % p.G;
@@ -41,6 +64,11 @@
   const int64_t ntiles = (p.M + ROWS - 1) / ROWS;
   const float* xz = p.x + (int64_t)z * p.M * K;
   float* oz = p.out + (int64_t)z * p.out_zs;
+  if constexpr (FIN == 1) {
+#pragma unroll
+    for (int i = 0; i < 25; ++i)
+      if (t == i) s_mask[i] = p.sh_mask[i];
+  }
   float4 nx[PPT];
   auto fetch = [&](int64_t tile) {
 #pragma unroll
@@ -82,18 +110,64 @@
       acc = __builtin_amdgcn_mfma_f32_32x32x16_bf16(al, bh[s], acc, 0, 0, 0);
       acc = __builtin_amdgcn_mfma_f32_32x32x16_bf16(ah, bl[s], acc, 0, 0, 0);
     }
-    if (col < p.N) {
-      const int64_t row0 = tile * ROWS + rg * 32 + 4 * lh;
-#pragma unroll
-      for (int r = 0; r < 16; ++r) {
-        const int64_t row = row0 + (r & 3) + 8 * (r >> 2);
-        if (row < p.M) oz[row * p.ldc + col] = acc[r] + bv;
-      }
+    if constexpr (FIN == 2) {
+      float* sx = s_xyz + rg * 96;
+      if (l31 < 3) {
+#pragma unroll
+        for (int r = 0; r < 16; ++r) sx[(4 * lh + (r & 3) + 8 * (r >> 2)) * 3 + l31] = acc[r] + bv;
+      }
+      asm volatile("s_waitcnt lgkmcnt(0)" ::: "memory");
+      const int64_t row = tile * ROWS + rg * 32 + l31;
+      if (lh == 0 && row < p.M) {
+        float x = sx[l31 * 3], y = sx[l31 * 3 + 1], zc = sx[l31 * 3 + 2];
+        pts3d_row(x, y, zc);
+        float* o = oz + row * p.ldc;
+        o[0] = x;
+        o[1] = y;
+        o[2] = zc;
+      }
+    } else {
+      if (FIN == 0 || p.out) {
+        if (col < p.N) {
+          const int64_t row0 = tile * ROWS + rg * 32 + 4 * lh;
+#pragma unroll
+          for (int r = 0; r < 16; ++r) {
+            const int64_t row = row0 + (r & 3) + 8 * (r >> 2);
+            if (row < p.M) oz[row * p.ldc + col] = acc[r] + bv;
+          }
+        }
+      }
+    }
+    if constexpr (FIN == 1) {
+#pragma unroll
+      for (int r = 0; r < 16; ++r) s_row[(rg * 32 + 4 * lh + (r & 3) + 8 * (r >> 2)) * FIN_LD + col] = acc[r] + bv;
+      lds_barrier();
+      const int64_t g0 = (int64_t)z * p.M + tile * ROWS;
+      const int rows = (int)(p.M - tile * ROWS < ROWS ? p.M - tile * ROWS : ROWS);
+      if (wave == 0) {
+        if (lane < rows) p.opac[g0 + lane] = gaussian_row(s_row + lane * FIN_LD, s_so + lane * 17);
+      } else {
+        store_span(p.sh + g0 * 75, rows * 75, t - 64, NT - 64, [&](int i) {
+          const int rr = i / 75, e = i - rr * 75;
+          return gaussian_sh(s_row[rr * FIN_LD + 8 + e], s_mask[e % 25]);
+        });
+      }
+      lds_barrier();
+      store_span(p.scales + g0 * 3, rows * 3, t, NT, [&](int i) { return s_so[(i / 3) * 17 + i % 3]; });
+      store_span(p.rots + g0 * 4, rows * 4, t, NT, [&](int i) { return s_so[(i >> 2) * 17 + 3 + (i & 3)]; });
+      store_span(p.cov + g0 * 9, rows * 9, t, NT, [&](int i) { return s_so[(i / 9) * 17 + 7 + i % 9]; });
     }
   }
 #endif
 }
 
+}
+
+static dim3 proj_grid(int64_t M, int Z, int rows) {
+  const int64_t nt = (M + rows - 1) / rows;
+  int64_t per = 256 / Z;
+  if (per < 1) per = 1;
+  return dim3((unsigned)(nt < per ? nt : per), Z);
 }
 
 extern "C" int siu3r_proj_rows_x3(const float* x, const void* wfrag, const float* bias, float* out, int Z, int G, int64_t M, int K, int N, int ldc,
@@ -102,17 +176,11 @@
   SIU3R_CHECK(Z > 0 && G > 0 && Z % G == 0 && M > 0 && N > 0 && ldc >= N, "proj_rows_x3: bad shape (Z=%d G=%d N=%d ldc=%d)", Z, G, N, ldc);
   ProjParams p{x, (const uint4*)wfrag, bias, out, M, out_z_stride > 0 ? out_z_stride : M * ldc, Z, G, N, ldc};
   const int nb = (N + 31) / 32;
-  auto grid = [&](int rows) {
-    const int64_t nt = (M + rows - 1) / rows;
-    int64_t per = 256 / Z;
-    if (per < 1) per = 1;
-    return dim3((unsigned)(nt < per ? nt : per), Z);
-  };
   hipStream_t s = (hipStream_t)stream;
   if (K == 256 && nb == 3)
-    hipLaunchKernelGGL((proj_rows_x3_kernel<256, 3, 2>), grid(64), dim3(384), 0, s, p);
+    hipLaunchKernelGGL((proj_rows_x3_kernel<256, 3, 2, 0>), proj_grid(M, Z, 64), dim3(384), 0, s, p);
   else if (K == 128 && nb == 1)
-    hipLaunchKernelGGL((proj_rows_x3_kernel<128, 1, 4>), grid(128), dim3(256), 0, s, p);
+    hipLaunchKernelGGL((proj_rows_x3_kernel<128, 1, 4, 0>), proj_grid(M, Z, 128), dim3(256), 0, s, p);
   else {
     siu3r_set_error("proj_rows_x3: no instantiation for K=%d N=%d (K 256 with N 65..96, K 128 with N <= 32)", K, N);
     return 1;
@@ -120,3 +188,26 @@
   SIU3R_LAUNCH_CHECK("siu3r_proj_rows_x3");
   return 0;
 }
+
+extern "C" int siu3r_proj_rows_x3_gaussians(const float* x, const void* wfrag, const float* bias, float* raw_or_null, float* opacities, float* scales,
+                                            float* rotations, float* harmonics, float* covariances, int Z, int G, int64_t M, int K, int N, void* stream) {
+  SIU3R_CHECK(x && wfrag && opacities && scales && rotations && harmonics && covariances, "proj_rows_x3_gaussians: null pointer");
+  SIU3R_CHECK(Z > 0 && G > 0 && Z % G == 0 && M > 0, "proj_rows_x3_gaussians: bad shape (Z=%d G=%d M=%lld)", Z, G, (long long)M);
+  SIU3R_CHECK(K == 256 && N == 83, "proj_rows_x3_gaussians: no instantiation for K=%d N=%d (K 256 with N 83)", K, N);
+  ProjParams p{x, (const uint4*)wfrag, bias, raw_or_null, M, M * N, Z, G, N, N, opacities, scales, rotations, harmonics, covariances, {}};
+  gaussian_sh_mask(p.sh_mask);
+  hipLaunchKernelGGL((proj_rows_x3_kernel<256, 3, 2, 1>), proj_grid(M, Z, 64), dim3(384), 0, (hipStream_t)stream, p);
+  SIU3R_LAUNCH_CHECK("siu3r_proj_rows_x3_gaussians");
+  return 0;
+}
+
+extern "C" int siu3r_proj_rows_x3_pts3d(const float* x, const void* wfrag, const float* bias, float* out, int Z, int G, int64_t M, int K, int N, int ldc,
+                                        int64_t out_z_stride, void* stream) {
+  SIU3R_CHECK(x && wfrag && out, "proj_rows_x3_pts3d: null pointer");
+  SIU3R_CHECK(Z > 0 && G > 0 && Z % G == 0 && M > 0 && ldc >= 3, "proj_rows_x3_pts3d: bad shape (Z=%d G=%d M=%lld ldc=%d)", Z, G, (long long)M, ldc);
+  SIU3R_CHECK(K == 128 && N == 3, "proj_rows_x3_pts3d: no instantiation for K=%d N=%d (K 128 with N 3)", K, N);
+  ProjParams p{x, (const uint4*)wfrag, bias, out, M, out_z_stride > 0 ? out_z_stride : M * ldc, Z, G, N, ldc};
+  hipLaunchKernelGGL((proj_rows_x3_kernel<128, 1, 4, 2>), proj_grid(M, Z, 128), dim3(256), 0, (hipStream_t)stream, p);
+  SIU3R_LAUNCH_CHECK("siu3r_proj_rows_x3_pts3d");
+  return 0;
+}
diff --git a/siu3r_amd/model.py b/siu3r_amd/model.py
--- a/siu3r_amd/model.py
+++ b/siu3r_amd/model.py
@@ -509,6 +509,16 @@
     return ops.proj_rows_x3(x, wf, wb, n, out)
 
 
+_HEAD_FINISH = os.environ.get("SIU3R_NO_HEAD_FINISH", "0") != "1"
+_SKIP_ADD = _HEAD_FINISH
+
+
+def _head4_finish_ok(ctx, names, x, gs: bool) -> bool:
+    K, n = x.shape[-1], ctx.w.sd[names[0] + ".weight"].shape[0]
+    ok = ops.proj_rows_gaussians_ok if gs else ops.proj_rows_pts3d_ok
+    return bool(_HEAD_FINISH and _PROJ_KERNEL and ctx.split and x.dtype == torch.float32 and x.is_contiguous() and ok(K, n))
+
+
 _STEM_KERNEL = os.environ.get("SIU3R_NO_STEM_KERNEL", "0") != "1"
 
 
@@ -538,10 +548,10 @@
     def _stem_gemm_planes(self) -> bool:
         return self.grouped and self.ctx.split and _CONV_PLANES
 
-    def _rcu(self, q, x, extra=None):
+    def _rcu(self, q, x, extra=None, summed=False):
         ctx = self.ctx
         W = lambda name: self._w("conv", q + name)
-        skip = lambda: x if extra is None else ops.affine_add(x.flatten(0, -4), extra.flatten(0, -4), None, None).view(x.shape)
+        skip = lambda: x if extra is None else extra if summed else ops.affine_add(x.flatten(0, -4), extra.flatten(0, -4), None, None).view(x.shape)
         if self.grouped:
             W(".conv1"), W(".conv2")
             res = skip()
@@ -556,14 +566,15 @@
             res = skip()
         return ops.conv2d(o, W(".conv2"), pad=1, out_dtype=ctx.act, residual=res)
 
-    def _fusion(self, q, x0, x1, reader=None):
-        out = x0 if x1 is None else self._rcu(q + ".resConfUnit1", x1, extra=x0)
+    def _fusion(self, q, x0, x1, reader=None, skip=None, summed=False):
+        out = x0 if x1 is None else self._rcu(q + ".resConfUnit1", x1, extra=x0, summed=summed)
         out = self._rcu(q + ".resConfUnit2", out)
         lead, (hh, ww) = out.shape[:-3], out.shape[-3:-1]
         out = ops.linear(out.flatten(-3, -2), self._w("linear", q + ".out_conv"), out_dtype=self.ctx.act)
         up = torch.empty((*lead, 2 * hh, 2 * ww, out.shape[-1]), dtype=out.dtype, device=out.device)
         upp = _feeds_planes(reader[0], self.ctx, up, reader[1]) if reader is not None and _CONV_PLANES else None
-        ops.resize_bilinear(out.view(-1, hh, ww, out.shape[-1]), (2 * hh, 2 * ww), True, out=up.view(-1, 2 * hh, 2 * ww, up.shape[-1]), planes_out=upp, planes_only=True)
+        ops.resize_bilinear(out.view(-1, hh, ww, out.shape[-1]), (2 * hh, 2 * ww), True, out=up.view(-1, 2 * hh, 2 * ww, up.shape[-1]), planes_out=upp, planes_only=True,
+                            addend=None if skip is None else skip.flatten(0, -4))
         return up if reader is None else (up, upp)
 
     def trunk(self, tokens: Sequence[torch.Tensor], H, W, reader=None):
@@ -580,10 +591,12 @@
                 l = ops.conv2d(l, self._w("conv", a + ".1"), stride=2, pad=1, out_dtype=ctx.act)
             layers.append(ops.conv2d(l, self._w("conv", f".dpt.scratch.layer_rn.{i}"), pad=1, out_dtype=ctx.act))
         s = ".dpt.scratch"
-        path4 = self._fusion(s + ".refinenet4", layers[3], None)
-        path3 = self._fusion(s + ".refinenet3", path4, layers[2])
-        path2 = self._fusion(s + ".refinenet2", path3, layers[1])
-        return self._fusion(s + ".refinenet1", path2, layers[0], reader)
+        fuse = _SKIP_ADD and ctx.act == torch.float32 and all(l.dtype == torch.float32 and l.is_contiguous() for l in layers)
+        nxt = lambda i: layers[i] if fuse else None
+        path4 = self._fusion(s + ".refinenet4", layers[3], None, skip=nxt(2))
+        path3 = self._fusion(s + ".refinenet3", path4, layers[2], skip=nxt(1), summed=fuse)
+        path2 = self._fusion(s + ".refinenet2", path3, layers[1], skip=nxt(0), summed=fuse)
+        return self._fusion(s + ".refinenet1", path2, layers[0], reader, summed=fuse)
 
     def _head4_names(self):
         return tuple(q + ".dpt.head.4" for q in self.ps)
@@ -598,12 +611,17 @@
         upp = _feeds_planes("pts_resize", ctx, up, lambda t: ops.conv2d(t, w2, pad=1, act=ACT_RELU, dry_run=True)) if _CONV_PLANES else None
         ops.resize_bilinear(x.flatten(0, -4), (H, W), True, out=up.view(-1, H, W, up.shape[-1]), planes_out=upp, planes_only=True)
         x = ops.conv2d(up, w2, pad=1, out_dtype=ctx.act, act=ACT_RELU, a_planes=upp)
-        xyz = _head4(ctx, self._head4_names(), x.view(lead[0], len(self.ps), H * W, -1))
+        x4 = x.view(lead[0], len(self.ps), H * W, -1)
+        if _head4_finish_ok(ctx, self._head4_names(), x4, gs=False):
+            wf, wb, n = ctx.w.proj(self._head4_names())
+            xyz = torch.empty((*x4.shape[:3], n), dtype=torch.float32, device=x.device)
+            return ops.proj_rows_x3_pts3d(x4, wf, wb, n, xyz).view(*lead, H, W, 3)
+        xyz = _head4(ctx, self._head4_names(), x4)
         if xyz is None:
             xyz = ops.linear(x.flatten(-3, -2), self._w("linear", ".dpt.head.4"), out_dtype=torch.float32)
         return ops.pts3d_exp_(xyz).view(*lead, H, W, 3)
 
-    def forward_gs(self, tokens, img, H, W, out=None):
+    def forward_gs(self, tokens, img, H, W, out=None, fields=None, want_raw=True):
         ctx = self.ctx
         path1 = self.trunk(tokens, H, W)
         lead, G = path1.shape[:-3], len(self.ps)
@@ -633,9 +651,17 @@
         if reads:
             xp.valid = xp.only = True
         x = ops.conv2d(x, head0(), pad=1, out_dtype=ctx.act, act=ACT_RELU, a_planes=xp if reads else None)
+        x4 = x.view(B, G, H * W, -1)
+        if fields is not None and _head4_finish_ok(ctx, self._head4_names(), x4, gs=True) and (not want_raw or out is None or out.is_contiguous()):
+            wf, wb, n = ctx.w.proj(self._head4_names())
+            if want_raw and out is None:
+                out = torch.empty((*lead, H * W, n), dtype=torch.float32, device=ctx.dev)
+            ops.proj_rows_x3_gaussians(x4, wf, wb, n, raw=out.view(B, G, H * W, n) if want_raw else None, out=fields)
+            fields["done"] = True
+            return out if want_raw else None
         if out is None:
             out = torch.empty((*lead, H * W, ctx.w.sd[self.ps[0] + ".dpt.head.4.weight"].shape[0]), dtype=torch.float32, device=ctx.dev)
-        if _head4(ctx, self._head4_names(), x.view(B, G, H * W, -1), out=out if self.grouped else out.unsqueeze(1)) is None:
+        if _head4(ctx, self._head4_names(), x4, out=out if self.grouped else out.unsqueeze(1)) is None:
             ops.linear(x.flatten(-3, -2), self._w("linear", ".dpt.head.4"), out=out)
         return out
 
@@ -1088,6 +1114,7 @@
         self.img_bv = self.img8 = self.enc = self.adapter = self.dstate = self.dec = self.ms = self.seg = self.gaussians = None
         self.gs, self.pts, self.raw = [None, None], [None, None], None
         self.want_f1 = False
+        self.fresh, self.want_raw, self.fields, self.pts_all = False, False, None, None
 
 
 class SIU3RModel:
@@ -1165,7 +1192,8 @@
             st = sl["st"]
         else:
             st = _Run(images, K)
-            st.want_f1 = bool(return_intermediates)
+            st.want_f1 = st.want_raw = bool(return_intermediates)
+            st.fresh = True
         h = _PendingForward(self, st, caller, sidx, eager, replayed, enable_query_class_logit_lift, return_intermediates)
         after_seg = functools.partial(self._after_seg, h)
         if replayed:
@@ -1271,7 +1299,12 @@
         def dec_pre():
             st.dstate = bb.decode_begin(st.enc)
             B, V, _, H, W = st.images.shape
-            st.raw = torch.empty((B, V, H * W, self.raw_gs_dim), dtype=torch.float32, device=self._ctx.dev)
+            dev = self._ctx.dev
+            if self._finish_gs(st):
+                f = lambda *s_: torch.empty((B, V, H * W, *s_), dtype=torch.float32, device=dev)
+                st.fields = dict(opacities=f(), scales=f(3), rotations=f(4), harmonics=f(3, 25), covariances=f(3, 3))
+            if st.fields is None or st.want_raw:
+                st.raw = torch.empty((B, V, H * W, self.raw_gs_dim), dtype=torch.float32, device=dev)
 
         def dec_post():
             st.dec = bb.decode_end(st.dstate)
@@ -1314,6 +1347,9 @@
     def _paired_heads(self, st) -> bool:
         B, V = st.images.shape[:2]
         return _HEAD_PAIRS and V == 2 and B == 1
+
+    def _finish_gs(self, st) -> bool:
+        return bool(_HEAD_FINISH and _PROJ_KERNEL and self._ctx.split and st.fresh and self._paired_heads(st))
 
     def _merged_decoder(self, st) -> bool:
         return self._ctx.fold and st.images.shape[1] == 2
@@ -1363,19 +1399,29 @@
         head = heads[0 if side is None else 1 + side]
         if gs:
             dst = st.raw if side is None else st.raw[:, side] if (side == 0 or V == 2) else (st.raw[0, 1:] if B == 1 else None)
-            r = head.forward_gs(toks, views(st.img8.view(B, V, H, W, -1)).contiguous(), H, W, out=dst)
+            r = head.forward_gs(toks, views(st.img8.view(B, V, H, W, -1)).contiguous(), H, W, out=dst, fields=st.fields if side is None else None,
+                                want_raw=st.fields is None or st.want_raw)
         else:
             r = head.forward_pts3d(toks, H, W)
         res = st.gs if gs else st.pts
         if side is None:
-            res[:] = [r[:, 0], r[:, 1]]
+            if not gs:
+                st.pts_all = r
+            res[:] = [None, None] if r is None else [r[:, 0], r[:, 1]]
         else:
             res[side] = r
 
     def _s_tail(self, st):
         B, V, _, H, W = st.images.shape
         cat = lambda a, b_: torch.cat((a.reshape(B, 1, H * W, -1), b_.reshape(B, V - 1, H * W, -1)), dim=1)
-        raw = st.raw if (V == 2 or B == 1) else cat(st.gs[0], st.gs[1])
+        if st.fields is not None and st.fields.get("done"):
+            cur = torch.cuda.current_stream()
+            g = dict(means=st.pts_all.view(B, V, H * W, 3), **{k: v for k, v in st.fields.items() if k != "done"})
+            for v in g.values():
+                v.record_stream(cur)
+            st.gaussians = Gaussians(**g)
+            return
+        raw = st.raw if (st.raw is not None and (V == 2 or B == 1)) else cat(st.gs[0], st.gs[1])
         st.gaussians = self.gaussian_adapter.forward(cat(st.pts[0], st.pts[1]), raw)
 
     __call__ = forward
diff --git a/siu3r_amd/ops.py b/siu3r_amd/ops.py
--- a/siu3r_amd/ops.py
+++ b/siu3r_amd/ops.py
@@ -788,6 +788,49 @@
     return (K == 256 and 65 <= n <= 96) or (K == 128 and n <= 32)
 
 
+GAUSSIAN_FIELDS = dict(opacities=(), scales=(3,), rotations=(4,), harmonics=(3, 25), covariances=(3, 3))
+
+
+def proj_rows_gaussians_ok(K: int, n: int) -> bool:
+    return K == 256 and n == 83
+
+
+def proj_rows_pts3d_ok(K: int, n: int) -> bool:
+    return K == 128 and n == 3
+
+
+def proj_rows_x3_gaussians(x: torch.Tensor, wfrag: torch.Tensor, bias: Optional[torch.Tensor], n: int, raw: Optional[torch.Tensor] = None,
+                           out: Optional[dict] = None):
+    B, G, M, K = x.shape
+    if not proj_rows_gaussians_ok(K, n):
+        raise ValueError(f"proj_rows_x3_gaussians: no instantiation for K={K} N={n} (K 256 with N 83)")
+    _gpu(x, wfrag, bias, raw)
+    assert x.dtype == torch.float32 and x.is_contiguous() and wfrag.shape[0] == G and wfrag.dtype == torch.bfloat16
+    assert raw is None or (raw.shape == (B, G, M, n) and raw.dtype == torch.float32 and raw.is_contiguous())
+    tails = GAUSSIAN_FIELDS
+    if out is None:
+        out = {k: torch.empty((B, G, M, *s), dtype=torch.float32, device=x.device) for k, s in tails.items()}
+    for k, s in tails.items():
+        _gpu(out[k])
+        assert out[k].shape == (B, G, M, *s) and out[k].dtype == torch.float32 and out[k].is_contiguous(), (k, out[k].shape)
+    check(_lib.lib().siu3r_proj_rows_x3_gaussians(_p(x), _p(wfrag), _p(bias), _p(raw), _p(out["opacities"]), _p(out["scales"]), _p(out["rotations"]),
+                                                  _p(out["harmonics"]), _p(out["covariances"]), B * G, G, M, K, n, _stream()))
+    return {k: out[k] for k in tails}
+
+
+def proj_rows_x3_pts3d(x: torch.Tensor, wfrag: torch.Tensor, bias: Optional[torch.Tensor], n: int, out: torch.Tensor):
+    B, G, M, K = x.shape
+    if not proj_rows_pts3d_ok(K, n):
+        raise ValueError(f"proj_rows_x3_pts3d: no instantiation for K={K} N={n} (K 128 with N 3)")
+    _gpu(x, wfrag, bias, out)
+    assert x.dtype == torch.float32 and x.is_contiguous() and wfrag.shape[0] == G and wfrag.dtype == torch.bfloat16
+    assert out.shape == (B, G, M, n) and out.dtype == torch.float32 and out.stride(3) == 1 and out.stride(2) >= n
+    zs = out.stride(1) if G > 1 else out.stride(0)
+    assert zs >= M * out.stride(2) and (B == 1 or G == 1 or out.stride(0) == G * zs), (out.shape, out.stride())
+    check(_lib.lib().siu3r_proj_rows_x3_pts3d(_p(x), _p(wfrag), _p(bias), _p(out), B * G, G, M, K, n, out.stride(2), zs, _stream()))
+    return out
+
+
 def pack_rowchain(wo, bo, g1, b1, w1, c1, w2, c2, g2, b2) -> torch.Tensor:
     H = w1.shape[0]
     assert tuple(wo.shape) == (256, 256) and tuple(w1.shape) == (H, 256) and tuple(w2.shape) == (256, H) and H > 0 and H % 256 == 0
```
